# aukeschaap/ttcross

Hardware: AMD Instinct MI355X
Metric: fiber evals/s (neval / wall time of dtt_dmrgg), Ising C_64 n=51 r=32 piv=2 (d=63) (higher is better)
Workload: dtype f64; 1 GPU; Ising C_64 n=51 r=32 piv=2 (d=63); driver=test_crs_ising c 64 51 32 2, bond_groups=8, transport=none (single process), arith=exact, sweeps=16

## Files before the change

### profiles/trace_timeline.py

```python
import csv
import glob
import statistics
import sys

f = glob.glob(sys.argv[1] + '/**/*kernel_trace.csv', recursive=True)[0]
rows = list(csv.DictReader(open(f)))
rows.sort(key=lambda r: int(r['Start_Timestamp']))
start = sys.argv[2] if len(sys.argv) > 2 else "20"
count = int(sys.argv[3]) if len(sys.argv) > 3 else 40


def short(name):
    return name.split('(')[0].replace('void ', '')[:40]


if start == "tail":
    med = statistics.median
    sw = [i for i, r in enumerate(rows) if 'k_sweep_cluster' in r['Kernel_Name']]
    pairs = []
    for a, b in zip(sw, sw[1:]):
        mid = [r for r in rows[a + 1:b] if r['Queue_Id'] == rows[a]['Queue_Id']]
        if any(k in r['Kernel_Name'] for r in mid for k in ('k_reset', 'k_init', 'k_fin_')):
            continue
        t = int(rows[a]['End_Timestamp'])
        steps = []
        for r in mid:
            s, e = int(r['Start_Timestamp']), int(r['End_Timestamp'])
            steps.append((short(r['Kernel_Name']), (s - t) / 1e3, (e - s) / 1e3))
            t = max(t, e)
        last = (int(rows[b]['Start_Timestamp']) - t) / 1e3
        ktime = sum(x[2] for x in steps)
        e2s = (int(rows[b]['Start_Timestamp']) - int(rows[a]['End_Timestamp'])) / 1e3
        pairs.append((e2s, ktime, e2s - ktime, tuple(steps), last))
    shapes = {}
    for p in pairs:
        shapes.setdefault(tuple(x[0] for x in p[3]), []).append(p)
    sweeps = [(int(rows[i]['End_Timestamp']) - int(rows[i]['Start_Timestamp'])) / 1e3 for i in sw]
    real = [x for x in sweeps if x > 20.0]
    print(f"k_sweep_cluster: {len(real)} launches that sweep, median {med(real):.1f} us (min {min(real):.1f}, max {max(real):.1f}); "
          f"{len(sweeps) - len(real)} that exit on the stop flag")
    for names, ps in sorted(shapes.items(), key=lambda kv: -len(kv[1])):
        print(f"{len(ps)} pairs with {len(names)} launches in between: end-to-start median {med(p[0] for p in ps):.1f} us "
              f"(min {min(p[0] for p in ps):.1f}, max {max(p[0] for p in ps):.1f}) = kernels {med(p[1] for p in ps):.1f} + gaps {med(p[2] for p in ps):.1f}")
        for k, nm in enumerate(names):
            print(f"    gap {med(p[3][k][1] for p in ps):6.1f}  dur {med(p[3][k][2] for p in ps):6.1f}  {nm}")
        print(f"    gap {med(p[4] for p in ps):6.1f}  k_sweep_cluster (next)")
    sys.exit(0)
if start == "run":
    inits = [i for i, r in enumerate(rows) if 'k_init_samples' in r['Kernel_Name']]
    i0 = inits[2] - 8
else:
    idx = [i for i, r in enumerate(rows) if 'k_sweep_cluster' in r['Kernel_Name']]
    i0 = idx[int(start)]
t0 = int(rows[i0]['Start_Timestamp'])
prev_end = t0
for r in rows[i0:i0 + count]:
    s, e = int(r['Start_Timestamp']), int(r['End_Timestamp'])
    print(f"{(s - t0) / 1e3:9.1f} us  gap {(s - prev_end) / 1e3:6.1f}  dur {(e - s) / 1e3:7.1f}  {r['Kernel_Name'][:60]}")
    prev_end = max(prev_end, e)
```

### ttcross_amd/csrc/ttx_create_plan.h

```cpp
#pragma once
#include <algorithm>
#include <cmath>
#include <cstdarg>
#include <cstddef>
#include <cstdio>
#include <cstdlib>
#include <cstring>
#include <mutex>
#include <string>
#include <vector>

#include "../../include/ttx.h"
#include "ttx_dev.h"
#include "ttx_qr_plan.h"

#if defined(__HIPCC__)
#define TTX_PLAN_HD __host__ __device__ inline
#else
#define TTX_PLAN_HD inline
#endif

#define DE5_W 4
#define DE5_SEG 16
TTX_PLAN_HD size_t de5_lds_doubles(int m) { const int VS = ((m + 7) & ~7) + 8 + DE5_SEG; return (size_t)5 * VS + 128 + (size_t)DE5_W * 64; }
TTX_PLAN_HD bool de5_fits(int m) { return m >= 3; }
TTX_PLAN_HD int de_rows_stride(int m) { const int s = m + 56; return ((s + 31) & ~31) + 16; }
TTX_PLAN_HD size_t de_rows_lds_doubles(int m) { return (size_t)12 * de_rows_stride(m); }
TTX_PLAN_HD int det_vs(int m) { return ((m + 7) & ~7) + 8; }
TTX_PLAN_HD size_t det_lds_doubles(int m, int nbk) { return (size_t)4 * det_vs(m) + 256 + (det_vs(m) + 48) + (size_t)3 * nbk * 16 * 64; }

constexpr int TTX_PLAN_FB = 1024;
constexpr int TTX_PLAN_FNR = 24;
constexpr int TTX_PLAN_MVN_MAXQ = 8;

struct EnvText { bool set = false; std::string v; };
struct CreateEnv {
    EnvText arith;
    EnvText sweep;
    EnvText cl_pad;
    bool fullpiv_mfma = false;
    bool fast_persist_off = false;
    bool de_lane = false;
    bool de_tables_off = false, de_fastdiv_off = false, de_cut_off = false, de_v2_off = false, de_team_off = false;
    bool de_lot_point_set = false; int de_lot_point = 0;
    int de_team_units = 256, de_team6_units = 1024;
    int de_test_fault = 0;
    bool de_v5 = false;
    int cluster_nb = 8;
    bool cluster_coop = false;
    int cluster_test_abort = 0;
    bool dbg_waves = false;
    bool lottery_one_block = false;
    bool lottery_wave_off = false;
    bool lottery_rows2 = false;
    bool mvn_v2_off = false;
    bool tail_off = false;
    bool tail_side_off = false;
};
template <class Get>
CreateEnv create_env_from(Get get)
{
    auto text = [&](const char *name) { EnvText t; if (const char *e = get(name)) { t.set = true; t.v = e; } return t; };
    auto num = [&](const char *name, int dflt) { const char *e = get(name); return e ? atoi(e) : dflt; };
    auto off = [&](const char *name) { const char *e = get(name); return e && atoi(e) == 0; };
    CreateEnv v;
    v.arith = text("TTX_ARITH"); v.sweep = text("TTX_SWEEP"); v.cl_pad = text("TTX_CL_PAD");
    v.fullpiv_mfma = text("TTX_FULLPIV").v == "mfma";
    v.fast_persist_off = off("TTX_FAST_PERSIST");
    v.de_lane = num("TTX_DE_LANE", 0) == 1;
    v.de_tables_off = off("TTX_DE_TABLES"); v.de_fastdiv_off = off("TTX_DE_FASTDIV"); v.de_cut_off = off("TTX_DE_CUT");
    v.de_v2_off = off("TTX_DE_V2"); v.de_team_off = off("TTX_DE_TEAM");
    v.de_lot_point_set = get("TTX_DE_LOT_POINT") != nullptr; v.de_lot_point = num("TTX_DE_LOT_POINT", 0);
    v.de_team_units = num("TTX_DE_TEAM_UNITS", v.de_team_units); v.de_team6_units = num("TTX_DE_TEAM6_UNITS", v.de_team6_units);
    v.de_test_fault = num("TTX_DE_TEST_FAULT", 0);
    v.de_v5 = num("TTX_DE_V5", 0) == 1;
    v.cluster_nb = num("TTX_CLUSTER_NB", v.cluster_nb);
    v.cluster_coop = num("TTX_CLUSTER_COOP", 0) == 1;
    v.cluster_test_abort = num("TTX_CLUSTER_TEST_ABORT", 0);
    v.dbg_waves = get("TTX_DBG_WAVES") != nullptr;
    v.lottery_one_block = num("TTX_LOTTERY_NB", 0) == 1;
    v.lottery_wave_off = off("TTX_LOTTERY_WAVE");
    v.lottery_rows2 = num("TTX_LOTTERY_ROWS", 0) == 2;
    v.mvn_v2_off = off("TTX_MVN_V2");
    v.tail_off = off("TTX_TAIL"); v.tail_side_off = off("TTX_TAIL_SIDE");
    return v;
}
struct DevCaps { int ncu = 0; bool coop = false; };

enum SweepWant { SWEEP_AUTO, SWEEP_CHAIN, SWEEP_FUSED, SWEEP_CLUSTER };
enum SlotKind { SLOTS_NONE, SLOTS_HOST, SLOTS_DEVICE };

struct CdfTables { std::vector<ttx_cdfseg> tab; std::vector<int> ns; };

struct CreatePlan {
    int err = TTX_OK; std::string errtext;
    int d = 0, RM = 0, NM = 0, W = 1, wrank = 0, nproc = 1, g0 = 0, G = 0, nbmax = 0, NC = 0, mode = 0, H = 0;
    std::vector<int32_t> own;
    int ising_id = 0; bool isDE = false;
    double mvn_norm = 1.0;
    size_t SS = 0, SW = 0, CS = 0, XD = 0, IOFF = 0, MSZ = 0, QB = 0, SB = 0, VS = 0;
    int nfb = 0, nlotmax = 0;
    int nn = 0, snum = 0;
    SlotKind slots = SLOTS_NONE; size_t HS = 0;
    int cdf_kmax = -1;
    bool pfull = false, qscr = false;
    bool want_fast = false;
    bool unit_nodes = false;
    int arith = 0, FD = 0, fpersist = 0;
    bool fast_tables = false;
    int de_npair = 0;
    int de_unit = 0, de_cut = 0;
    int de_slots = 0;
    int de_v2 = 0;
    int de_team = 0, de_team_units = 256, de_team6_units = 1024;
    int de_v5 = 0;
    int de_test_fault = 0;
    int de_lot_point = 0;
    int lot_wave = 0, lot_rows = 0;
    size_t lds_de = 0, lds_det = 0, lds_det6 = 0, lds_de5 = 0, lds_der = 0;
    int mvn_v2 = 0; size_t lds_mvn = 0;
    int lot_nb = 1, bnd_wave = 0;
    bool lot_cand = false;
    int fp_mfma = 0, fp_tiles = 0;
    size_t lds_par = 0, lds_half = 0, lds_lot = 0;
    int half_vals = 0, lot_vals = 0, fast_cap = 0;
    size_t lds_fused = 0, lds_cluster = 0;
    bool fused_ok = false;
    int cluster_cand = 0;
    int cluster_var = 0;
    int cluster_ldsinv = 0, cluster_zkeep = 0, cluster_coop = 0;
    int cl_test_abort = 0; bool dbg_waves = false;
    bool sweep_tail = true;
    bool sweep_tail_side = true;
    SweepWant sweep_want = SWEEP_AUTO; int ncu = 0;
    int fused = 0;
    int cluster = 0;
};

inline void share(int first, int last, int nproc, std::vector<int32_t> &own)
{
    own.assign(nproc + 1, 0);
    own[0] = first;
    for (int p = 1; p < nproc; p++) own[p] = first + (int)((double)(last - first + 1) * (double)p / nproc);
    own[nproc] = last + 1;
}
inline double powi(double a, int b)
{
    double r = 1.0;
    for (;;) { if (b & 1) r *= a; b /= 2; if (b == 0) break; a *= a; }
    return r;
}
inline bool cdf_tables(int kmax, CdfTables &out)
{
    out.tab.assign((size_t)(kmax + 1) * TTX_TABSEG, ttx_cdfseg());
    out.ns.assign(kmax + 1, 0);
    std::vector<ttx_cdfseg> tmp(TTX_MAXSEG);
    for (int K = 1; K <= kmax; K++) {
        const int n_ = ttx_cdf_build(K, tmp.data());
        if (n_ > TTX_TABSEG) { out = CdfTables(); return false; }
        out.ns[K] = n_;
        memcpy(&out.tab[(size_t)K * TTX_TABSEG], tmp.data(), sizeof(ttx_cdfseg) * n_);
    }
    return true;
}
inline bool cdf_table_fits(int kmax)
{
    static std::mutex mu;
    static int looked = 0, first_over = -1;
    if (kmax > 16384) return false;
    std::lock_guard<std::mutex> lk(mu);
    std::vector<ttx_cdfseg> tmp(TTX_MAXSEG);
    while (looked < kmax && first_over < 0) { looked++; if (ttx_cdf_build(looked, tmp.data()) > TTX_TABSEG) first_over = looked; }
    return first_over < 0 || kmax < first_over;
}

#if defined(__GNUC__)
__attribute__((format(printf, 3, 4)))
#endif
inline CreatePlan &plan_refuse(CreatePlan &p, int code, const char *fmt, ...)
{
    char buf[512];
    va_list ap; va_start(ap, fmt); vsnprintf(buf, sizeof buf, fmt, ap); va_end(ap);
    p.err = code; p.errtext = buf;
    return p;
}

inline CreatePlan create_plan(const ttx_config &cfg, bool nofun, const CreateEnv &env, const DevCaps &caps)
{
    CreatePlan p;
    const int d = cfg.d, fun = cfg.fun_id, nproc = std::max(cfg.nproc, 1);
    p.d = d; p.RM = cfg.maxrank; p.nproc = nproc; p.ncu = caps.ncu;
    p.W = cfg.world_size < 1 ? 1 : cfg.world_size; p.wrank = cfg.world_rank;
    int NM = 1;
    for (int k = 0; k < d; k++) { if (cfg.n[k] < 1 || cfg.n[k] > 32000) return plan_refuse(p, TTX_EINVAL, "bad mode size"); NM = std::max(NM, cfg.n[k]); }
    p.NM = NM;
    if ((long long)p.RM * NM > (long long)TTX_MAXPART * TTX_BLK) return plan_refuse(p, TTX_EINVAL, "maxrank*n too large");
    if (cfg.mybonds) p.own.assign(cfg.mybonds, cfg.mybonds + nproc + 1);
    else share(1, d - 1, nproc, p.own);
    for (int g = 0; g < nproc; g++) if (p.own[g + 1] <= p.own[g]) return plan_refuse(p, TTX_EINVAL, "mybonds: empty group %d", g);
    if (p.own[0] != 1 || p.own[nproc] != d) return plan_refuse(p, TTX_EINVAL, "mybonds: must run from 1 to d = %d (got %d .. %d)", d, p.own[0], p.own[nproc]);
    p.g0 = (int)((long long)nproc * p.wrank / p.W);
    p.G = (int)((long long)nproc * (p.wrank + 1) / p.W) - p.g0;
    for (int g = 0; g < nproc; g++) p.nbmax = std::max(p.nbmax, p.own[g + 1] - p.own[g]);
    p.NC = p.nbmax + 1;
    p.mode = (cfg.pivoting == 0) ? 1 : (cfg.pivoting < 0) ? 2 : 0;
    p.H = (cfg.pivoting <= 0) ? 2 : 2 * cfg.pivoting;
    p.ising_id = (fun == TTX_FUN_ISING) ? (int)cfg.par[2 * cfg.n[0]] : 0;
    p.isDE = fun == TTX_FUN_ISING && p.ising_id != 1;
    if (fun == TTX_FUN_MVN) {
        if (cfg.naux < d + d * d + 1) return plan_refuse(p, TTX_EINVAL, "mvn: aux too short");
        p.mvn_norm = std::sqrt(powi(2.0 * 3.141592653589793, d) * cfg.aux[d + (size_t)d * d]);
        if (!(p.mvn_norm > 0.0) || !std::isfinite(p.mvn_norm))
            return plan_refuse(p, TTX_EINVAL, "ttx_create: mvn normalisation sqrt((2 pi)^d det) = %g is not a positive finite number (det = %g under- or overflows at d = %d)",
                               p.mvn_norm, cfg.aux[d + (size_t)d * d], d);
    }
    const size_t RM = p.RM;
    const size_t VS = ((d + 7) & ~7) + 8;
    const int nlotmax = 2 * p.RM + 2 * NM;
    p.VS = VS; p.nlotmax = nlotmax;
    p.SS = RM * NM; p.SW = (size_t)NM * RM; p.CS = RM * NM * RM;
    p.nfb = (int)((RM * NM + TTX_BLK - 1) / TTX_BLK);
    p.XD = RM * NM + RM * RM;
    p.IOFF = (sizeof(int) * (XH + d + 2) + 15) & ~(size_t)15;
    p.MSZ = (p.IOFF + sizeof(double) * p.XD + 15) & ~(size_t)15;
    p.QB = (size_t)nproc * RM * RM + 2 * nproc;
    p.SB = SUM_HDR + nproc + 5 * (size_t)(d + 1);
    p.qscr = 2 * sizeof(double) * (RM * RM + 2) > TTX_LDS_WORK;
    p.nn = cfg.n[0];
    for (int k = 1; k < d; k++) p.nn = std::min(p.nn, cfg.n[k]);
    p.snum = std::max(8, nproc);

    bool want = cfg.arith == TTX_ARITH_FAST;
    if (cfg.arith != TTX_ARITH_EXACT && cfg.arith != TTX_ARITH_FAST) return plan_refuse(p, TTX_EINVAL, "ttx_create: arith must be TTX_ARITH_EXACT or TTX_ARITH_FAST (got %d)", cfg.arith);
    if (env.arith.set) {
        if (env.arith.v == "fast") want = true;
        else if (env.arith.v != "exact") return plan_refuse(p, TTX_EINVAL, "TTX_ARITH must be exact or fast (got %s)", env.arith.v.c_str());
    }
    p.want_fast = want && !nofun;
    bool unit = fun == TTX_FUN_ISING;
    for (int j = 0; unit && j < std::min(NM, (int)cfg.npar); j++) unit = cfg.par[j] >= 0.0 && cfg.par[j] <= 1.0;
    p.unit_nodes = unit;
    p.arith = (p.want_fast && ((p.isDE && unit) || fun == TTX_FUN_MVN)) ? 1 : 0;
    if (p.arith) {
        p.fast_tables = true;
        p.FD = d + 1;
        p.fpersist = (fun == TTX_FUN_MVN && env.fast_persist_off) ? 0 : 1;
    }
    if (p.isDE && !p.arith && env.de_lane) p.de_unit = unit;
    if (p.isDE && !p.arith && !env.de_lane && !env.de_tables_off) {
        p.de_npair = d * (d + 1) / 2;
        p.de_unit = unit && !env.de_fastdiv_off;
        p.de_cut = (p.de_unit && !env.de_cut_off) ? 1 : 0;
        p.de_lot_point = (env.de_lot_point_set ? env.de_lot_point : (int)(d <= 160)) != 0;
        p.de_slots = (int)RM * ((NM + 63) / 64);
        p.lds_de = sizeof(double) * (5 * VS + 256) + (p.de_cut ? sizeof(int) * VS : 0);
        p.de_v2 = cfg.pivoting >= 0 && p.de_slots <= TTX_MAXPART && p.lds_de <= TTX_LDS_WORK && !env.de_v2_off;
        p.lds_det = sizeof(double) * det_lds_doubles(d, 3);
        p.lds_det6 = sizeof(double) * det_lds_doubles(d, 1);
        p.de_team = p.de_v2 && !p.de_cut && p.lds_det <= TTX_LDS_WORK && !env.de_team_off;
        p.de_team_units = env.de_team_units;
        p.de_team6_units = env.de_team6_units;
        p.de_test_fault = env.de_test_fault;
        p.lds_de5 = sizeof(double) * de5_lds_doubles(d);
        p.de_v5 = p.de_v2 && !p.de_cut && de5_fits(d) && p.lds_de5 <= TTX_LDS_WORK && env.de_v5;
    }
    p.pfull = cfg.pivoting < 0;
    if (cfg.pivoting < 0 && env.fullpiv_mfma && RM <= 64 && (long long)(RM * NM) * (long long)(RM * NM) < (1LL << 31)) {
        const size_t side = RM * NM;
        p.fp_mfma = 1; p.fp_tiles = (int)(((side + 63) / 64) * ((side + 63) / 64));
    }
    if (cdf_table_fits(p.RM * NM)) p.cdf_kmax = p.RM * NM;

    p.lds_par = sizeof(double) * (cfg.npar + 2);
    {
        const size_t base = sizeof(double) * (cfg.npar + RM + 4);
        const size_t idx_bytes = sizeof(short) * ((RM + 1) * VS + 16), val_bytes = sizeof(double) * ((RM + 1) * 2 * VS + 4);
        p.half_vals = (fun == TTX_FUN_ISING && p.ising_id == 1 && base + val_bytes <= TTX_LDS_VALUES) ? 1 : 0;
        p.lds_half = base + (p.half_vals ? val_bytes : idx_bytes);
        const size_t dif_bytes = sizeof(double) * ((RM + 1) * VS + 4);
        if (fun == TTX_FUN_MVN && base + dif_bytes <= TTX_LDS_HALF_DIFF) { p.half_vals = 1; p.lds_half = base + dif_bytes; }
        if (p.arith) p.lds_half = std::max(p.lds_half, base + sizeof(double) * ((size_t)std::max(p.FD, TTX_PLAN_FNR) + 4 + RM + 2));
    }
    const size_t lot_hdr = sizeof(double) * (cfg.npar + 4) + sizeof(int) * 4 * (nlotmax + 4);
    {
        p.lds_lot = lot_hdr + sizeof(short) * (2 * RM * VS + 16);
        const size_t lot_dif = lot_hdr + sizeof(double) * (2 * RM * VS + 4);
        if (fun == TTX_FUN_MVN && lot_dif <= TTX_LDS_LOTTERY) { p.lot_vals = 1; p.lds_lot = lot_dif; }
        if (p.arith && fun == TTX_FUN_ISING) {
            const size_t hdr = lot_hdr + 32;
            const size_t rowb = 2 * sizeof(double) * RM;
            p.fast_cap = (int)std::min<size_t>(std::min<size_t>(40, (size_t)d + 1), hdr < TTX_LDS_VALUES ? (TTX_LDS_VALUES - hdr) / rowb : 0);
            p.lds_lot = std::max(p.lds_lot, hdr + rowb * p.fast_cap);
        }
    }
    {
        const bool fastc = fun == TTX_FUN_ISING && p.ising_id == 1 && cfg.pivoting >= 0 && p.cdf_kmax >= 0;
        p.lds_fused = sizeof(double) * (cfg.npar + 4 + 4 * RM * VS + 2 * RM * NM + RM + 4) + sizeof(int) * 4 * (nlotmax + 4);
        p.fused_ok = fastc && p.RM <= 64 && nlotmax <= TTX_PLAN_FB && p.lds_fused <= TTX_LDS_WORK;
        int NB = std::max(1, std::min(env.cluster_nb, TTX_CLMAX));
        while (NB > 1 && p.G * NB > caps.ncu / 2) NB--;
        const size_t SL = RM * ((NM + NB - 1) / NB + 1);
        p.lds_cluster = sizeof(double) * (cfg.npar + 4 + 2 * RM * (2 * VS + 2) + 4 * SL + 2 * RM + 8) + sizeof(int) * 4 * (nlotmax + 4);
        if (p.lds_cluster + sizeof(double) * 2 * RM * RM <= TTX_LDS_WORK) { p.cluster_ldsinv = 1; p.lds_cluster += sizeof(double) * 2 * RM * RM; }
        const size_t zk = sizeof(int) * ((size_t)p.nbmax * 2 * RM + 2 * p.nbmax + 4);
        if (p.lds_cluster + zk <= TTX_LDS_WORK) { p.cluster_zkeep = 1; p.lds_cluster += zk; }
        const bool cfastc = p.want_fast && fun == TTX_FUN_ISING && p.ising_id == 1;
        if (env.cl_pad.set && env.cl_pad.v != "0" && env.cl_pad.v != "1") return plan_refuse(p, TTX_EINVAL, "TTX_CL_PAD must be 0 or 1 (got %s)", env.cl_pad.v.c_str());
        p.cluster_var = cfastc ? 2 : (unit && !(env.cl_pad.set && env.cl_pad.v == "0")) ? 1 : 0;
        if (fastc && p.RM <= 64 && NB >= 2 && p.G * NB <= caps.ncu && p.lds_cluster <= TTX_LDS_WORK) {
            p.cluster_cand = NB;
            p.cluster_coop = caps.coop && env.cluster_coop;
        }
        p.cl_test_abort = env.cluster_test_abort; p.dbg_waves = env.dbg_waves;
        p.sweep_tail = !env.tail_off; p.sweep_tail_side = !env.tail_side_off;
        const std::string want_sweep = env.sweep.set ? env.sweep.v : "auto";
        if (want_sweep == "cluster") p.sweep_want = SWEEP_CLUSTER;
        else if (want_sweep == "fused") p.sweep_want = SWEEP_FUSED;
        else if (want_sweep == "auto") p.sweep_want = SWEEP_AUTO;
        else if (want_sweep == "chain") p.sweep_want = SWEEP_CHAIN;
        else return plan_refuse(p, TTX_EINVAL, "TTX_SWEEP must be auto, chain, fused or cluster (got %s)", want_sweep.c_str());
    }
    if (!nofun && (p.lds_half > TTX_LDS_DEVICE || p.lds_lot > TTX_LDS_LOTTERY)) return plan_refuse(p, TTX_EINVAL, "problem too large for LDS staging (d*maxrank)");
    {
        const bool heavy = p.isDE || fun == TTX_FUN_MVN;
        if (heavy && !env.lottery_one_block) p.lot_nb = std::min((nlotmax + 63) / 64, 64);
        if (p.lot_nb > 1 && (nlotmax + p.lot_nb - 1) / p.lot_nb > 64) p.lot_nb = 1;
        if (fun == TTX_FUN_MVN && d <= 64 * TTX_PLAN_MVN_MAXQ && cfg.pivoting >= 0 && (int)RM * ((NM + 63) / 64) <= TTX_MAXPART && !env.mvn_v2_off) {
            p.lot_cand = true;
            p.mvn_v2 = 1; p.de_slots = (int)RM * ((NM + 63) / 64);
            p.bnd_wave = 1;
            p.lds_mvn = sizeof(double) * (3 * (size_t)d + 8);
        }
        if (p.isDE && p.arith) p.bnd_wave = 1;
        if (p.isDE && p.de_npair) {
            p.lot_cand = true;
            p.lds_der = sizeof(double) * de_rows_lds_doubles(d);
            p.lot_wave = p.de_v2 && !p.de_cut && p.lds_der <= TTX_LDS_WORK && !env.lottery_wave_off;
            p.bnd_wave = p.lot_wave || (p.de_cut && p.de_v2 && p.lds_der <= TTX_LDS_WORK);
            p.lot_rows = p.lot_wave ? (env.lottery_rows2 ? 2 : 1) : 0;
        }
    }
    if (fun == TTX_FUN_HOST || fun == TTX_FUN_COSCOEFF || fun == TTX_FUN_DEVICE || fun == TTX_FUN_TRAINS) {
        p.HS = std::max<size_t>({RM * NM, (size_t)p.nn * p.snum, (size_t)p.NC * NM, (size_t)nlotmax, (size_t)2 * NM, (size_t)256});
        p.slots = fun == TTX_FUN_HOST ? SLOTS_HOST : SLOTS_DEVICE;
    }
    return p;
}

inline void create_admit(CreatePlan &p, int occ)
{
    bool cluster_ok = p.cluster_cand != 0;
    if (cluster_ok) {
        const long long cap = (long long)occ * p.ncu;
        const long long grid = 8LL * p.cluster_cand * ((p.G + 7) / 8);
        if (grid * 2 > cap) cluster_ok = false;
    }
    if (p.sweep_want == SWEEP_CLUSTER) { if (cluster_ok) p.cluster = p.cluster_cand; }
    else if (p.sweep_want == SWEEP_FUSED) { if (p.fused_ok) p.fused = 1; }
    else if (p.sweep_want == SWEEP_AUTO) { if (cluster_ok) p.cluster = p.cluster_cand; else if (p.fused_ok && p.G == 1) p.fused = 1; }
    if (p.cluster && p.cluster_var == 2) p.arith = 1;
}
```

### ttcross_amd/csrc/ttx_engine.hip

```cpp
#include <hip/hip_runtime.h>

#include <chrono>
#include <cmath>
#include <cstdarg>
#include <cstdio>
#include <cstdlib>
#include <cstring>
#include <map>
#include <memory>
#include <string>
#include <thread>
#include <type_traits>
#include <vector>

#include <atomic>
#include <dlfcn.h>
#include <rccl/rccl.h>

#include "../../include/ttx.h"
#include "../../include/ttx_device_fun.h"
#include "ttx_lds.h"
#include "ttx_qr_plan.h"
#include "ttx_create_plan.h"
#include "ttx_loop_plan.h"
// ... 21 lines not shown
#include "ttx_roundsum.h"
#include "ttx_sample.h"
#include "ttx_sample_real.h"
#include "ttx_topk.h"
#include "ttx_sample_sq.h"
#include "ttx_trainfun.h"

static thread_local std::string g_err;
static int fail(int code, const char *fmt, ...)
{
    char buf[512];
    va_list ap; va_start(ap, fmt); vsnprintf(buf, sizeof buf, fmt, ap); va_end(ap);
    g_err = buf;
    return code;
}
#define HIPCHECK(x) do { hipError_t e_ = (x); if (e_ != hipSuccess) return fail(TTX_EHIP, "%s failed: %s (%s:%d)", #x, hipGetErrorString(e_), __FILE__, __LINE__); } while (0)


static int env_int(const char *name, int dflt) { const char *e = getenv(name); return e ? atoi(e) : dflt; }
static bool env_off(const char *name) { const char *e = getenv(name); return e && atoi(e) == 0; }

static int ensure_lds(int device, const void *fn, size_t need)
{
    return ttx_lds_raise(device, fn, need, [](const void *fn, size_t need) -> int {
        HIPCHECK(hipFuncSetAttribute(fn, hipFuncAttributeMaxDynamicSharedMemorySize, (int)need));
        return TTX_OK;
    });
}

extern "C" const char *ttx_last_error(void) { return g_err.c_str(); }
extern "C" int ttx_version(void) { return 3; }


struct RcclApi {
    void *lib = nullptr;
    ncclResult_t (*GetUniqueId)(ncclUniqueId *) = nullptr;
    ncclResult_t (*CommInitRank)(ncclComm_t *, int, ncclUniqueId, int) = nullptr;
    ncclResult_t (*CommDestroy)(ncclComm_t) = nullptr;
    ncclResult_t (*Send)(const void *, size_t, ncclDataType_t, int, ncclComm_t, hipStream_t) = nullptr;
    ncclResult_t (*Recv)(void *, size_t, ncclDataType_t, int, ncclComm_t, hipStream_t) = nullptr;
    ncclResult_t (*AllReduce)(const void *, void *, size_t, ncclDataType_t, ncclRedOp_t, ncclComm_t, hipStream_t) = nullptr;
    ncclResult_t (*GroupStart)() = nullptr;
    ncclResult_t (*GroupEnd)() = nullptr;
    const char *(*GetErrorString)(ncclResult_t) = nullptr;
};
static RcclApi g_rccl;
static int rccl_load()
{
    if (g_rccl.lib) return TTX_OK;
    void *L = dlopen("librccl.so", RTLD_NOW | RTLD_GLOBAL);
    if (!L) L = dlopen("/opt/rocm/lib/librccl.so", RTLD_NOW | RTLD_GLOBAL);
    if (!L) return fail(TTX_EHIP, "cannot load librccl.so: %s", dlerror());
#define SYM_(f, name) *(void **)(&g_rccl.f) = dlsym(L, name); if (!g_rccl.f) return fail(TTX_EHIP, "librccl.so lacks %s", name);
    SYM_(GetUniqueId, "ncclGetUniqueId") SYM_(CommInitRank, "ncclCommInitRank") SYM_(CommDestroy, "ncclCommDestroy")
    SYM_(Send, "ncclSend") SYM_(Recv, "ncclRecv") SYM_(AllReduce, "ncclAllReduce") SYM_(GroupStart, "ncclGroupStart")
    SYM_(GroupEnd, "ncclGroupEnd") SYM_(GetErrorString, "ncclGetErrorString")
#undef SYM_
    g_rccl.lib = L;
    return TTX_OK;
}
#define NCCLCHECK(x) do { ncclResult_t e_ = (x); if (e_ != ncclSuccess) return fail(TTX_EHIP, "%s failed: %s", #x, g_rccl.GetErrorString(e_)); } while (0)

enum {
    SC_TRAIN,
    SC_META,
    SC_IND, SC_OUT, SC_X,
    SC_FLAG, SC_LQ,
    SC_XA, SC_XB, SC_SORT,
    SC_W, SC_M, SC_P, SC_SCR, SC_VEC,
    SC_H, SC_ROW, SC_CNT,
    SC_SRX,
    SC_TFUN, SC_TVAL,
    SC_MAT,
    SC_KP, SC_KW, SC_KS, SC_KX,
    SC_KREC, SC_KSEL, SC_KOUT,
    SC_RSO, SC_RSW, SC_RSYA, SC_RSYB,
    SC_RSM, SC_RSTAB,
    SC_QH, SC_QF, SC_QS, SC_QX,
    SC_BTAB,
    SC_NBUF
};
struct EvBuf { void *p = nullptr; size_t bytes = 0; };
struct OpTimer {
    hipEvent_t ev[2] = {nullptr, nullptr};
    int start(hipStream_t s) { for (auto &e : ev) if (!e) HIPCHECK(hipEventCreate(&e)); HIPCHECK(hipEventRecord(ev[0], s)); return TTX_OK; }
    int stop(hipStream_t s) { HIPCHECK(hipEventRecord(ev[1], s)); return TTX_OK; }
    int ms(double *out) { float t = 0.f; HIPCHECK(hipEventElapsedTime(&t, ev[0], ev[1])); *out = t; return TTX_OK; }
};
enum { TM_MODESUM, TM_ALG, TM_HEAD, TM_DRAW, TM_APPLY,
       TM_GRAM, TM_SCORE, TM_SELECT,
       TM_RS_SKETCH, TM_N };

struct DevFun;
struct TrainFun;
struct ttx_engine {
    ttx_config cfg;
    std::vector<int32_t> n1;
    std::vector<double> par, aux, quadw;
    std::vector<int32_t> own;
    int d = 0, RM = 0, NM = 0, G = 0, NC = 0, nbmax = 0, H = 0, mode = 0;
    int g0 = 0;
    int W = 1, wrank = 0;
    DevProb P{};
    hipStream_t stream = nullptr;
    std::vector<void *> allocs;
    size_t SB = 0, QB = 0;
    double *h_sum = nullptr;
    char *h_msg = nullptr;
    double *h_tmp = nullptr;
    char *recvL = nullptr, *recvR = nullptr;
    ncclComm_t comm = nullptr;
    ttx_transport cb{};
    bool have_cb = false;
    int cb_error = 0;
    struct RedJob { ttx_engine *h; double *buf; size_t count; int op; };
    static const int NRED = 16;
    RedJob red[NRED];
    double *red_mem = nullptr; size_t red_cap = 0; int red_next = 0;
    RedJob *red_slot(size_t count, int op)
    {
        if (!red_mem || count > red_cap) return nullptr;
        RedJob *j = &red[red_next];
        j->h = this; j->buf = red_mem + (size_t)red_next * red_cap; j->count = count; j->op = op;
        red_next = (red_next + 1) % NRED;
        return j;
    }
    ShmTransport *shm = nullptr;
    std::vector<ttx_sweep_rec> recs;
    std::vector<int32_t> tapes;
    std::vector<int32_t> rfinal;
    std::vector<std::vector<uint8_t>> updhist;
    int64_t neval = 0;
    double seconds = 0.0;
    bool ran = false;
    bool profile = false;
    struct Ev { int kind, n; hipEvent_t a, b; };
    std::vector<Ev> evs;
    std::vector<hipEvent_t> evpool;
    int64_t k_launches[TTX_K_NKINDS] = {0};
    double k_ms[TTX_K_NKINDS] = {0}, k_bytes[TTX_K_NKINDS] = {0};
    double *Wa = nullptr, *Wb = nullptr, *Wc = nullptr, *Wd = nullptr, *Sm = nullptr, *bak = nullptr;
    int *Si = nullptr;
    CreatePlan sel;
    struct Retired { bool cluster = false, de_team = false, de_v5 = false; } retired;
    int cluster_nb() const { return retired.cluster ? 0 : sel.cluster; }
    bool de_team() const { return sel.de_team && !retired.de_team; }
    bool de_v5() const { return sel.de_v5 && !retired.de_v5; }
    int arith() const { return P.arith; }
    int cluster_fallbacks = 0;
    int det_fallbacks = 0, de5_fallbacks = 0;
    bool cluster_aborted = false;
    double *h_svd = nullptr; double svd_seq = 0.0;
    hipStream_t qstream = nullptr;
    hipEvent_t ev_sum[2] = {nullptr, nullptr}, ev_val[2] = {nullptr, nullptr}, ev_tail[2] = {nullptr, nullptr};
    double *h_sum_base = nullptr;
    double *h_val = nullptr;
    int *h_abort = nullptr;
    ttx_host_fun hfun = nullptr;
    const double *hfun_par = nullptr;
    std::shared_ptr<DevFun> dfun;
    std::shared_ptr<TrainFun> tfun;
    TfOps tf_ops{};
    std::vector<char> tf_host;
    std::vector<std::pair<hipEvent_t, hipEvent_t>> tf_evs;
    bool tf_figures = false;
    int64_t tf_launches = 0, tf_elements = 0;
    double tf_ms = 0.0;
    int64_t host_calls = 0;
    int64_t n_resid = 0;
    EvBuf scratch[SC_NBUF];
    std::vector<char> train_host, meta_host;
    OpTimer timer[TM_N];
    int ncu = 0;
    int ev_last_mode = -1;
    double ct_ms = 0.0, ct_bytes = 0.0;
    double alg_ms = 0.0, alg_rd = 0.0, alg_wr = 0.0;
    double sm_ms_head = 0.0, sm_bytes = 0.0, sm_ms_draw = 0.0;
    int64_t sm_failed = 0;
    double sr_ms_head = 0.0, sr_bytes = 0.0, sr_ms_draw = 0.0;
    int64_t sr_failed = 0;
    double ma_ms = 0.0, ma_rd = 0.0, ma_wr = 0.0, ma_flops = 0.0;
    int ma_mode = -1;
    double tk_ms_gram = 0.0, tk_ms_score = 0.0, tk_ms_select = 0.0, tk_flops = 0.0;
    int tk_mode = -1;
    double sq_ms_head = 0.0, sq_ms_rows = 0.0, sq_ms_pick = 0.0, sq_flops = 0.0;
    int64_t sq_failed = 0;
    int sq_mode = -1;
    double rs_ms[4] = {0.0, 0.0, 0.0, 0.0}, rs_flops = 0.0;
    std::vector<int32_t> rs_l;
    int rs_mode = -1;
    std::vector<hipEvent_t> rs_ev;
    double bs_ms_tab = 0.0, bs_ms_chain = 0.0, bs_flops = 0.0;
    int bs_mode = -1;
    std::vector<hipEvent_t> bs_ev;
};

static HostPool &host_pool()
{
    static HostPool p(host_pool_threads(getenv("TTX_HOST_THREADS"), getenv("OMP_NUM_THREADS"), std::thread::hardware_concurrency()));
    return p;
}

static int host_eval(ttx_engine *h)
{
    HIPCHECK(hipStreamSynchronize(h->stream));
    HIPCHECK(hipGetLastError());
    DevProb &P = h->P;
    const size_t nslot = (size_t)h->G * h->sel.HS;
    std::vector<uint32_t> todo;
    for (size_t s = 0; s < nslot; s++) if (P.hreq[s]) { todo.push_back((uint32_t)s); P.hreq[s] = 0; }
    const int32_t d = h->d;
    const int32_t *nn = h->n1.data() + 1;
    host_pool().run(todo.size(), [&](size_t i) {
        int32_t ind[2048];
        const short *row = P.hidx + (size_t)todo[i] * d;
        for (int k = 0; k < d; k++) ind[k] = row[k];
        P.hval[todo[i]] = h->hfun(&d, ind, nn, h->hfun_par);
    });
    h->host_calls += (int64_t)todo.size();
    return TTX_OK;
}

struct DevFun {
    int device = 0;
    hipModule_t mod = nullptr;
    hipFunction_t slots = nullptr, list = nullptr;
    ttx_devfun_info info{};
    double *par = nullptr;
    std::string name;
    std::vector<unsigned char> image;
    ~DevFun()
    {
        (void)hipSetDevice(device);
        if (par) (void)hipFree(par);
        else (void)hipDeviceSynchronize();
        if (mod) (void)hipModuleUnload(mod);
    }
};
#define DEVFUN_LAUNCHCHECK(x) do { hipError_t e_ = (x); if (e_ != hipSuccess) return fail(TTX_EHIP, "%s failed: %s (%s:%d)", #x, hipGetErrorString(e_), __FILE__, __LINE__); } while (0)
static int devfun_slots(ttx_engine *h)
{
    DevFun &f = *h->dfun;
    DevProb &P = h->P;
    int d = P.d;
    long long nslot = (long long)h->G * h->sel.HS;
    const int *n = P.n + 1;
    const double *par = f.par;
    const short *hidx = P.hidx; unsigned char *hreq = P.hreq; double *hval = P.hval;
    const int waves = f.info.block / 64;
    const long long want = f.info.kind == TTX_DEVFUN_KIND_WAVE ? (nslot + waves - 1) / waves : (nslot + f.info.block - 1) / f.info.block;
    const unsigned grid = (unsigned)std::max<long long>(1, std::min<long long>(want, 4096));
    void *args[] = {&d, &n, &par, &nslot, &hidx, &hreq, &hval};
    DEVFUN_LAUNCHCHECK(hipModuleLaunchKernel(f.slots, grid, 1, 1, (unsigned)f.info.block, 1, 1, (unsigned)(f.info.lds_per_wave * waves), h->stream, args, nullptr));
    return TTX_OK;
}

struct TrainFun {
    std::vector<ttx_engine *> x;
    int op = 0;
    std::shared_ptr<DevFun> comb;
};
static int tf_grid(ttx_engine *h, long long items);
static int tf_prepare(ttx_engine *h, const char *who, bool figures);
static int tf_finish(ttx_engine *h);
static int tf_eval_list(ttx_engine *h, int64_t npts, const int32_t *ind, double *out);
struct TfScope {
    ttx_engine *h; hipEvent_t a = nullptr, b = nullptr;
    bool on;
    explicit TfScope(ttx_engine *h_) : h(h_), on(h_->profile && h_->tf_figures) { if (on) { (void)hipEventCreate(&a); (void)hipEventCreate(&b); (void)hipEventRecord(a, h->stream); } }
    ~TfScope() { if (on) { (void)hipEventRecord(b, h->stream); h->tf_evs.push_back({a, b}); } }
};
static int tf_slots(ttx_engine *h)
{
    const TrainFun &f = *h->tfun;
    DevProb &P = h->P;
    long long nslot = (long long)h->G * h->sel.HS;
    const TfOps &O = h->tf_ops;
    const size_t lds = sizeof(double) * TTX_TF_WAVES * tf_lds_doubles(O.ldx, O.d);
    const dim3 grid(tf_grid(h, nslot)), block(64 * TTX_TF_WAVES);
    const short *hidx = P.hidx; unsigned char *hreq = P.hreq; double *hval = P.hval;
    double *tval = (double *)h->scratch[SC_TVAL].p;
    unsigned long long *cnt = (unsigned long long *)h->scratch[SC_CNT].p;
    if (h->tf_figures) h->tf_launches++;
    TfScope timed(h);
    switch (f.op) {
        case TTX_TOP_PRODUCT: hipLaunchKernelGGL(k_tf_slots<TF_PRODUCT>, grid, block, lds, h->stream, O, nslot, hidx, hreq, hval, tval, cnt); break;
        case TTX_TOP_RATIO: hipLaunchKernelGGL(k_tf_slots<TF_RATIO>, grid, block, lds, h->stream, O, nslot, hidx, hreq, hval, tval, cnt); break;
        case TTX_TOP_SQRTABS: hipLaunchKernelGGL(k_tf_slots<TF_SQRTABS>, grid, block, lds, h->stream, O, nslot, hidx, hreq, hval, tval, cnt); break;
        default: {
            hipLaunchKernelGGL(k_tf_slots<TF_DEVICE>, grid, block, lds, h->stream, O, nslot, hidx, hreq, hval, tval, cnt);
            DevFun &c = *f.comb;
            int m = O.m, d = O.d;
            const int *n = P.n + 1;
            const double *par = c.par, *tv = tval;
            const unsigned cg = (unsigned)std::max<long long>(1, std::min<long long>((nslot + c.info.block - 1) / c.info.block, 4096));
            void *args[] = {&m, &d, &n, &par, &nslot, &hidx, &hreq, &tv, &hval};
            DEVFUN_LAUNCHCHECK(hipModuleLaunchKernel(c.slots, cg, 1, 1, (unsigned)c.info.block, 1, 1, 0, h->stream, args, nullptr));
        }
    }
    return TTX_OK;
}

static int slot_eval(ttx_engine *h)
{
    DevProb &P = h->P;
    if (!P.slot_dev) return host_eval(h);
    if (h->cfg.fun_id == TTX_FUN_DEVICE) return devfun_slots(h);
// ... 66 lines not shown
    P.ising_id = s.ising_id;
    P.has_quad = cfg.quadw != nullptr;
    P.small_element = 10 * 2.220446049250313e-16; P.small_pivot = 1.e-5;
    P.mvn_norm = s.mvn_norm;
    P.SS = s.SS; P.SW = s.SW; P.CS = s.CS;
    P.arith = s.arith; P.FD = s.FD; P.fpersist = s.fpersist;
    P.de_npair = s.de_npair; P.de_unit = s.de_unit; P.de_cut = s.de_cut;
    P.nfb = s.nfb; P.fp_mfma = s.fp_mfma; P.fp_tiles = s.fp_tiles;
    P.XD = s.XD; P.IOFF = s.IOFF; P.MSZ = s.MSZ;
    P.accuracy = cfg.accuracy; P.maxrank = cfg.maxrank;
    P.lot_nb = s.lot_nb; P.lot_max = s.nlotmax; P.bnd_wave = s.bnd_wave;
    h->n1.assign(d + 2, 1);
    for (int k = 1; k <= d; k++) h->n1[k] = cfg.n[k - 1];
    if (cfg.npar > 0) h->par.assign(cfg.par, cfg.par + cfg.npar);
    if (cfg.aux && cfg.naux > 0) h->aux.assign(cfg.aux, cfg.aux + cfg.naux);
    int *dn; double *dpar, *daux = nullptr, *dq = nullptr;
    A_(dev_upload(h, &dn, h->n1.data(), (size_t)d + 2));
    A_(dev_alloc(h, &dpar, cfg.npar + 1));
    if (cfg.npar > 0) HIPCHECK(hipMemcpy(dpar, h->par.data(), sizeof(double) * cfg.npar, hipMemcpyHostToDevice));
    if (!h->aux.empty()) A_(dev_upload(h, &daux, h->aux.data(), h->aux.size()));
    if (cfg.quadw) {
        h->quadw.assign((size_t)(d + 1) * NM, 0.0);
        size_t off = 0;
        for (int k = 1; k <= d; k++) { for (int j = 0; j < h->n1[k]; j++) h->quadw[(size_t)k * NM + j] = cfg.quadw[off + j]; off += h->n1[k]; }
        A_(dev_upload(h, &dq, h->quadw.data(), h->quadw.size()));
    }
    P.n = dn; P.par = dpar; P.aux = daux; P.quadw = dq;
    return TTX_OK;
}
static int create_integrand_tables(ttx_engine *h)
{
    const CreatePlan &s = h->sel;
    DevProb &P = h->P;
    const int d = s.d;
    const size_t G = s.G, NC = s.NC, RM = s.RM;
    const bool mvn = h->cfg.fun_id == TTX_FUN_MVN;
    if (s.fast_tables) {
        const size_t slots = s.fpersist ? G * NC : G;
        for (int sd = 0; sd < 2; sd++) {
            A_(dev_alloc(h, &P.fNear[sd], slots * (size_t)s.FD * RM));
            A_(dev_alloc(h, &P.fPiv[sd], slots * (size_t)TTX_FS * RM));
            if (mvn) A_(dev_alloc(h, &P.fDv[sd], slots * (size_t)s.FD * RM));
        }
        if (mvn) {
            std::vector<double> sy((size_t)d * d);
            const double *ic = h->aux.data() + d;
            for (int i = 0; i < d; i++) for (int j = 0; j < d; j++) sy[i + (size_t)d * j] = 0.5 * (ic[i + (size_t)d * j] + ic[j + (size_t)d * i]);
            double *ds;
            A_(dev_upload(h, &ds, sy.data(), sy.size()));
            P.auxS = ds;
        }
    }
    if (s.de_npair) {
        A_(dev_alloc(h, &P.deTL, G * (size_t)s.de_npair * RM)); A_(dev_alloc(h, &P.deTR, G * (size_t)s.de_npair * RM));
        A_(dev_alloc(h, &P.deUL, G * (size_t)(d + 1) * RM));
        if (s.de_cut) { A_(dev_alloc(h, &P.deCL, G * (size_t)(d + 1) * RM)); A_(dev_alloc(h, &P.deCR, G * (size_t)(d + 1) * RM)); }
    }
    if (mvn) {
        std::vector<double> t((size_t)d * d);
        for (int i = 0; i < d; i++) for (int j = 0; j < d; j++) t[j + (size_t)d * i] = h->aux[d + i + (size_t)d * j];
        double *dt;
        A_(dev_upload(h, &dt, t.data(), t.size()));
        P.auxT = dt;
    }
    return TTX_OK;
}
static int create_cores(ttx_engine *h)
{
    const CreatePlan &s = h->sel;
    DevProb &P = h->P;
    const size_t d = s.d, G = s.G, NC = s.NC, RM = s.RM, NM = s.NM;
    A_(dev_alloc(h, &P.arg, G * NC * P.CS)); A_(dev_alloc(h, &P.col, G * NC * P.CS)); A_(dev_alloc(h, &P.row, G * NC * P.CS));
    A_(dev_alloc(h, &P.inv, G * NC * RM * RM)); A_(dev_alloc(h, &P.vip, G * NC * 4 * RM));
    A_(dev_alloc(h, &P.L, G * NC * d * RM)); A_(dev_alloc(h, &P.R, G * NC * d * RM));
    A_(dev_alloc(h, &P.r, G * (d + 2))); A_(dev_alloc(h, &P.rr, G * (d + 2))); A_(dev_alloc(h, &P.upd, G * (d + 2))); A_(dev_alloc(h, &P.tape, G * (d + 2) * 4));
    A_(dev_alloc(h, &P.acol, G * RM * NM)); A_(dev_alloc(h, &P.arow, G * RM * NM));
    A_(dev_alloc(h, &P.Tq, G * NC * RM * RM));
    A_(dev_alloc(h, &P.ind0, d + 2)); A_(dev_alloc(h, &P.gs, G));
    for (size_t g = 0; g < G; g++) {
        GroupState g0s{};
        g0s.first = h->own[h->g0 + g]; g0s.last = h->own[h->g0 + g + 1] - 1; g0s.gglobal = h->g0 + (int)g;
        const hipError_t e = hipMemcpy(P.gs + g, &g0s, offsetof(GroupState, S), hipMemcpyHostToDevice);
        if (e != hipSuccess) return fail(TTX_EHIP, "ttx_create: %s", hipGetErrorString(e));
    }
    if (s.pfull) A_(dev_alloc(h, &P.pfull, G * NM * RM * (size_t)s.nfb));
    if (s.fp_mfma) { A_(dev_alloc(h, &P.sb, G * (RM * NM) * (RM * NM))); A_(dev_alloc(h, &P.pfull2, G * (size_t)s.fp_tiles)); }
    if (s.cdf_kmax >= 0) {
        CdfTables t;
        if (!cdf_tables(s.cdf_kmax, t)) return fail(TTX_EINVAL, "ttx_create: no CDF tables up to K = %d", s.cdf_kmax);
        ttx_cdfseg *dt; int *dn_;
        A_(dev_upload(h, &dt, t.tab.data(), t.tab.size()));
        A_(dev_upload(h, &dn_, t.ns.data(), t.ns.size()));
        P.cdf_tab = dt; P.cdf_ns = dn_; P.cdf_kmax = s.cdf_kmax;
    }
    LotPart *lp; unsigned *lc;
    A_(dev_alloc(h, &lp, G * s.lot_nb));
    A_(dev_alloc(h, &lc, G));
    P.lotp = lp; P.lot_ctr = lc;
    if (s.lot_cand) { A_(dev_alloc(h, &P.lotc, G * s.nlotmax * 4)); A_(dev_alloc(h, &P.lotf, G * s.nlotmax)); }
    if (s.cluster) {
        unsigned *ctr; ClPart *cp;
        A_(dev_alloc(h, &ctr, G));
        A_(dev_alloc(h, &cp, 2 * G * TTX_CLREC));
        P.cl_ctr = ctr; P.cl_part = cp;
#ifdef TTX_STAMPS
        if (s.dbg_waves) { long long *dbg; A_(dev_alloc(h, &dbg, (size_t)8 * 64 * 8)); P.dbg = dbg; }
#endif
        HIPCHECK(hipHostMalloc((void **)&h->h_abort, sizeof(int)));
        *h->h_abort = 0;
        P.cl_abort = h->h_abort;
        P.cl_test_abort = s.cl_test_abort;
    }
    return TTX_OK;
}
static int create_exchange(ttx_engine *h)
{
    const CreatePlan &s = h->sel;
    DevProb &P = h->P;
    const size_t G = s.G, RM = s.RM, d = s.d;
    const int nproc = s.nproc;
    A_(dev_alloc(h, &P.msgR, G * P.MSZ)); A_(dev_alloc(h, &P.msgL, G * P.MSZ));
    A_(dev_alloc(h, &h->recvL, P.MSZ)); A_(dev_alloc(h, &h->recvR, P.MSZ));
    A_(dev_alloc(h, &P.inL, G)); A_(dev_alloc(h, &P.inR, G));
    A_(dev_alloc(h, &P.red, G * 4)); A_(dev_alloc(h, &P.redsend, 4));
    A_(dev_alloc(h, &P.qsend, h->QB)); A_(dev_alloc(h, &P.qwork, ((size_t)nproc + 2) * RM * RM)); A_(dev_alloc(h, &P.sumsend, h->SB));
    P.qscr = nullptr;
    if (s.qscr) A_(dev_alloc(h, &P.qscr, G * 2 * RM * RM));
    if (s.W > 1) { A_(dev_alloc(h, &P.redrecv, 4)); A_(dev_alloc(h, &P.qall, h->QB)); A_(dev_alloc(h, &P.sumrecv, h->SB)); }
    else { P.redrecv = P.redsend; P.qall = P.qsend; P.sumrecv = P.sumsend; }
    {
        std::vector<char *> il(G, nullptr), ir(G, nullptr);
        for (size_t g = 0; g < G; g++) {
            if (g > 0) il[g] = P.msgR + (g - 1) * P.MSZ; else if (h->g0 > 0) il[g] = h->recvL;
            if (g + 1 < G) ir[g] = P.msgL + (g + 1) * P.MSZ; else if (h->g0 + (int)G < nproc) ir[g] = h->recvR;
        }
        HIPCHECK(hipMemcpy(P.inL, il.data(), sizeof(char *) * G, hipMemcpyHostToDevice));
        HIPCHECK(hipMemcpy(P.inR, ir.data(), sizeof(char *) * G, hipMemcpyHostToDevice));
    }
    int *ctl, *rq;
    A_(dev_alloc(h, &ctl, (size_t)4));
    A_(dev_alloc(h, &rq, G * (d + 2)));
    P.ctl = ctl; P.rq = rq;
    P.tail_side = 0;
    A_(dev_alloc(h, &P.tailrec, 2 * G)); A_(dev_alloc(h, &P.tail_tape, 2 * G * (d + 2) * 4)); A_(dev_alloc(h, &P.strk, (size_t)2));
    return TTX_OK;
}
static int create_staging(ttx_engine *h)
{
    HIPCHECK(hipHostMalloc((void **)&h->h_sum_base, sizeof(double) * 2 * h->SB));
    h->h_sum = h->h_sum_base;
    memset(h->h_sum_base, 0, sizeof(double) * 2 * h->SB);
    HIPCHECK(hipHostMalloc((void **)&h->h_val, sizeof(double) * 2));
    HIPCHECK(hipStreamCreateWithFlags(&h->qstream, hipStreamNonBlocking));
    for (int x = 0; x < 2; x++) { HIPCHECK(hipEventCreateWithFlags(&h->ev_sum[x], hipEventDisableTiming)); HIPCHECK(hipEventCreateWithFlags(&h->ev_val[x], hipEventDisableTiming)); HIPCHECK(hipEventCreateWithFlags(&h->ev_tail[x], hipEventDisableTiming)); }
    HIPCHECK(hipHostMalloc((void **)&h->h_msg, 4 * h->P.MSZ));
    HIPCHECK(hipHostMalloc((void **)&h->h_tmp, sizeof(double) * std::max(h->QB, h->SB)));
    if (h->W > 1) {
        h->red_cap = std::max<size_t>(std::max(h->QB, h->SB), 8);
        HIPCHECK(hipHostMalloc((void **)&h->red_mem, sizeof(double) * h->red_cap * ttx_engine::NRED));
    }
    return TTX_OK;
}
static int create_slots(ttx_engine *h)
{
    const CreatePlan &s = h->sel;
    DevProb &P = h->P;
    if (s.slots == SLOTS_NONE) return TTX_OK;
    const size_t nslot = (size_t)s.G * s.HS, d = s.d;
    if (s.slots == SLOTS_DEVICE) {
        P.slot_dev = 1;
        A_(dev_alloc(h, &P.hidx, nslot * d)); A_(dev_alloc(h, &P.hval, nslot)); A_(dev_alloc(h, &P.hreq, nslot));
    } else {
        HIPCHECK(hipHostMalloc((void **)&P.hidx, sizeof(short) * nslot * d));
        HIPCHECK(hipHostMalloc((void **)&P.hval, sizeof(double) * nslot));
        HIPCHECK(hipHostMalloc((void **)&P.hreq, nslot));
        memset(P.hreq, 0, nslot); memset(P.hval, 0, sizeof(double) * nslot);
    }
    P.HS = (int)s.HS; P.hostpass = 0;
    return TTX_OK;
}
#undef A_

static int create_impl(ttx_engine **out, const ttx_config *cfg, bool nofun)
{
    if (!out || !cfg) return fail(TTX_EINVAL, "ttx_create: null argument");
    *out = nullptr;
    if (!cfg->n) return fail(TTX_EINVAL, "ttx_create: mode sizes missing");
    if (cfg->d < 2) return fail(TTX_EINVAL, "dtt_dmrgg: l,m: 1 %d", cfg->d);
    if (cfg->maxrank < 1 || cfg->maxrank > 128) return fail(TTX_EINVAL, "ttx_create: maxrank must be in 1..128 (got %d)", cfg->maxrank);
    if (cfg->pivoting < -1) return fail(TTX_EINVAL, "dtt_dmrgg: unknown pivoting: %d", cfg->pivoting);
    if (2 * cfg->pivoting + 2 > TTX_MAXH) return fail(TTX_EINVAL, "dtt_dmrgg: pivoting %d too large", cfg->pivoting);
    if (!(nofun && cfg->fun_id == 0) && (cfg->fun_id < 1 || cfg->fun_id > TTX_FUN_TRAINS)) return fail(TTX_EINVAL, "ttx_create: unknown fun_id %d", cfg->fun_id);
    if (cfg->npar < 0 || (cfg->npar > 0 && !cfg->par)) return fail(TTX_EINVAL, "ttx_create: par missing");
    if (cfg->fun_id == TTX_FUN_ISING && (cfg->npar < 2 * cfg->n[0] + 1)) return fail(TTX_EINVAL, "ttx_create: the Ising integrand needs par(1:2n+1) (nodes, weights, id)");
    if ((cfg->fun_id == TTX_FUN_STDNORM || cfg->fun_id == TTX_FUN_MVN) && cfg->npar < cfg->n[0]) return fail(TTX_EINVAL, "ttx_create: the integrand needs the nodes par(1:n)");
    if (cfg->fun_id != TTX_FUN_HOST && cfg->fun_id != TTX_FUN_COSCOEFF && cfg->fun_id != TTX_FUN_DEVICE && cfg->fun_id != TTX_FUN_TRAINS && cfg->fun_id != 0)
        for (int k = 1; k < cfg->d; k++)
            if (cfg->n[k] > cfg->n[0]) return fail(TTX_EINVAL, "ttx_create: mode %d has %d points, more than the first mode (%d): the built-in integrands index par by n(1)", k + 1, cfg->n[k], cfg->n[0]);
    if (cfg->fun_id == TTX_FUN_HOST && cfg->d > 2048) return fail(TTX_EINVAL, "ttx_create: host integrand: at most 2048 dimensions (tt_size)");
    if (cfg->fun_id == TTX_FUN_DEVICE && cfg->d > 2048) return fail(TTX_EINVAL, "ttx_create: device integrand: at most 2048 dimensions (tt_size)");
    if (cfg->fun_id == TTX_FUN_TRAINS && cfg->d > 2048) return fail(TTX_EINVAL, "ttx_create: integrand of trains: at most 2048 dimensions (tt_size)");
    if (cfg->fun_id == TTX_FUN_COSCOEFF) { if (int rc0 = coscoeff_check("ttx_create", cfg->d, cfg->n, cfg->aux, cfg->naux)) return rc0; }
    const int W = cfg->world_size < 1 ? 1 : cfg->world_size;
    if (cfg->fun_id == TTX_FUN_TRAINS && W > 1) return fail(TTX_EINVAL, "ttx_create: an integrand of trains (TTX_FUN_TRAINS) runs in one process: bond groups (nproc) work, world_size %d does not", W);
    const int nproc = std::max(cfg->nproc < 1 ? 1 : cfg->nproc, 1);
    if (nproc >= cfg->d) return fail(TTX_EINVAL, "nproc exceeds or equal dimension, cannot proceed");
    if (nproc < W) return fail(TTX_EINVAL, "ttx_create: %d bond groups cannot be spread over %d GPUs", nproc, W);
    if (nproc > 256) return fail(TTX_EINVAL, "ttx_create: at most 256 bond groups");
    if (cfg->world_rank < 0 || cfg->world_rank >= W) return fail(TTX_EINVAL, "ttx_create: world_rank out of range");
    int ndev = 0;
    if (hipGetDeviceCount(&ndev) != hipSuccess || ndev <= 0) return fail(TTX_ENODEV, "ttx_create: no HIP device (the engine has no CPU path)");
    if (cfg->device < 0 || cfg->device >= ndev) return fail(TTX_ENODEV, "ttx_create: device %d not present", cfg->device);
    HIPCHECK(hipSetDevice(cfg->device));
    DevCaps caps;
    {
        hipDeviceProp_t prop;
        HIPCHECK(hipGetDeviceProperties(&prop, cfg->device));
        int coop = 0;
        HIPCHECK(hipDeviceGetAttribute(&coop, hipDeviceAttributeCooperativeLaunch, cfg->device));
        caps.ncu = prop.multiProcessorCount; caps.coop = coop != 0;
    }

    ttx_config c = *cfg;
    c.nproc = nproc;
    CreatePlan plan = create_plan(c, nofun, create_env(), caps);
    if (plan.err) return fail(plan.err, "%s", plan.errtext.c_str());
    if (plan.cluster_cand) {
        const void *fn = reinterpret_cast<const void *>(cluster_kernel(plan.cluster_var));
        if (int rc = ensure_lds(cfg->device, fn, plan.lds_cluster)) return rc;
        int occ = 0;
        HIPCHECK(hipOccupancyMaxActiveBlocksPerMultiprocessor(&occ, cluster_kernel(plan.cluster_var), CB, plan.lds_cluster));
        create_admit(plan, occ);
    } else create_admit(plan, 0);

    ttx_engine *h = new ttx_engine();
    struct Guard { ttx_engine *h; ~Guard() { if (h) destroy_keep_error(h); } } guard{h};
    h->cfg = c;
    h->sel = std::move(plan);
    const CreatePlan &s = h->sel;
    h->W = s.W; h->wrank = s.wrank; h->d = s.d; h->RM = s.RM; h->NM = s.NM; h->own = s.own;
    h->g0 = s.g0; h->G = s.G; h->nbmax = s.nbmax; h->NC = s.NC; h->mode = s.mode; h->H = s.H;
    h->QB = s.QB; h->SB = s.SB;
    HIPCHECK(hipStreamCreateWithFlags(&h->stream, hipStreamNonBlocking));
    int rc;
    if ((rc = create_problem(h)) || (rc = create_integrand_tables(h)) || (rc = create_cores(h)) || (rc = create_exchange(h)) ||
        (rc = create_staging(h)) || (rc = create_slots(h))) return rc;
    guard.h = nullptr;
    *out = h;
    return TTX_OK;
}
extern "C" int ttx_create(ttx_engine **out, const ttx_config *cfg) { return create_impl(out, cfg, false); }

extern "C" void ttx_destroy(ttx_engine *h)
{
    if (!h) return;
    if (h->dfun) { (void)hipSetDevice(h->cfg.device); if (h->stream) (void)hipStreamSynchronize(h->stream); h->dfun.reset(); }
    if (h->tfun) { (void)hipSetDevice(h->cfg.device); if (h->stream) (void)hipStreamSynchronize(h->stream); h->tfun.reset(); }
    if (h->comm && g_rccl.CommDestroy) (void)g_rccl.CommDestroy(h->comm);
    for (void *p : h->allocs) (void)hipFree(p);
    for (auto &b : h->scratch) if (b.p) (void)hipFree(b.p);
    for (auto &t : h->timer) for (auto &e : t.ev) if (e) (void)hipEventDestroy(e);
    for (auto &e : h->tf_evs) { (void)hipEventDestroy(e.first); (void)hipEventDestroy(e.second); }
    if (h->h_sum_base) (void)hipHostFree(h->h_sum_base);
    if (h->h_val) (void)hipHostFree(h->h_val);
    if (h->h_svd) (void)hipHostFree(h->h_svd);
    if (h->qstream) (void)hipStreamDestroy(h->qstream);
    for (int x = 0; x < 2; x++) { if (h->ev_sum[x]) (void)hipEventDestroy(h->ev_sum[x]); if (h->ev_val[x]) (void)hipEventDestroy(h->ev_val[x]); if (h->ev_tail[x]) (void)hipEventDestroy(h->ev_tail[x]); }
    if (h->h_msg) (void)hipHostFree(h->h_msg);
    if (h->h_tmp) (void)hipHostFree(h->h_tmp);
    if (h->red_mem) (void)hipHostFree(h->red_mem);
    if (h->shm) { shm_close(h->shm); delete h->shm; }
    if (h->h_abort) (void)hipHostFree(h->h_abort);
    if (!h->P.slot_dev) {
        if (h->P.hidx) (void)hipHostFree(h->P.hidx);
        if (h->P.hval) (void)hipHostFree(h->P.hval);
        if (h->P.hreq) (void)hipHostFree(h->P.hreq);
    }
    for (auto &e : h->evpool) (void)hipEventDestroy(e);
    for (auto &e : h->rs_ev) (void)hipEventDestroy(e);
    for (auto &e : h->bs_ev) (void)hipEventDestroy(e);
    if (h->stream) (void)hipStreamDestroy(h->stream);
    delete h;
}

extern "C" int ttx_comm_unique_id(uint8_t id[128])
{
    int rc = rccl_load();
    if (rc) return rc;
    ncclUniqueId u;
    NCCLCHECK(g_rccl.GetUniqueId(&u));
    memcpy(id, u.internal, 128);
    return TTX_OK;
}
extern "C" int ttx_comm_init(ttx_engine *h, const uint8_t id[128])
{
    if (!h) return fail(TTX_EINVAL, "ttx_comm_init: null handle");
    if (h->cfg.fun_id == TTX_FUN_TRAINS) return fail(TTX_ESTATE, "ttx_comm_init: an engine with an integrand of trains (TTX_FUN_TRAINS) runs in one process");
    if (h->W == 1) return TTX_OK;
    int rc = rccl_load();
    if (rc) return rc;
    HIPCHECK(hipSetDevice(h->cfg.device));
    ncclUniqueId u;
    memcpy(u.internal, id, 128);
    NCCLCHECK(g_rccl.CommInitRank(&h->comm, h->W, u, h->wrank));
    return TTX_OK;
}
extern "C" int ttx_k_rccl_selftest(int32_t device, int64_t msg_bytes, int32_t nsum)
{
    if (msg_bytes < 1 || nsum < 1) return fail(TTX_EINVAL, "ttx_k_rccl_selftest: bad sizes");
    int ndev = 0;
    if (hipGetDeviceCount(&ndev) != hipSuccess || ndev <= 0) return fail(TTX_ENODEV, "no HIP device");
    HIPCHECK(hipSetDevice(device));
    int rc = rccl_load();
    if (rc) return rc;
    ncclUniqueId u;
    NCCLCHECK(g_rccl.GetUniqueId(&u));
    ncclComm_t comm = nullptr;
    NCCLCHECK(g_rccl.CommInitRank(&comm, 1, u, 0));
    hipStream_t st = nullptr;
    char *dsend = nullptr, *drecv = nullptr; double *dred = nullptr, *dout = nullptr;
    std::vector<char> hs((size_t)msg_bytes), hr((size_t)msg_bytes);
    std::vector<double> hd((size_t)nsum + 4), ho((size_t)nsum + 4);
    for (int64_t i = 0; i < msg_bytes; i++) hs[(size_t)i] = (char)((i * 131 + 7) & 0xff);
    for (size_t i = 0; i < hd.size(); i++) hd[i] = 1.0 / (double)(i + 3) - 0.25 * (double)(i % 5);
    int bad = 0;
    auto body = [&]() -> int {
        HIPCHECK(hipStreamCreateWithFlags(&st, hipStreamNonBlocking));
        HIPCHECK(hipMalloc((void **)&dsend, (size_t)msg_bytes)); HIPCHECK(hipMalloc((void **)&drecv, (size_t)msg_bytes));
        HIPCHECK(hipMalloc((void **)&dred, sizeof(double) * hd.size())); HIPCHECK(hipMalloc((void **)&dout, sizeof(double) * hd.size()));
        HIPCHECK(hipMemcpyAsync(dsend, hs.data(), (size_t)msg_bytes, hipMemcpyHostToDevice, st));
        HIPCHECK(hipMemsetAsync(drecv, 0, (size_t)msg_bytes, st));
        HIPCHECK(hipMemcpyAsync(dred, hd.data(), sizeof(double) * hd.size(), hipMemcpyHostToDevice, st));
        HIPCHECK(hipMemsetAsync(dout, 0, sizeof(double) * hd.size(), st));
        NCCLCHECK(g_rccl.GroupStart());
        NCCLCHECK(g_rccl.Send(dsend, (size_t)msg_bytes, ncclChar, 0, comm, st));
        NCCLCHECK(g_rccl.Recv(drecv, (size_t)msg_bytes, ncclChar, 0, comm, st));
        NCCLCHECK(g_rccl.GroupEnd());
        NCCLCHECK(g_rccl.AllReduce(dred, dout, 4, ncclDouble, ncclMax, comm, st));
        NCCLCHECK(g_rccl.AllReduce(dred + 4, dout + 4, (size_t)nsum, ncclDouble, ncclSum, comm, st));
        HIPCHECK(hipMemcpyAsync(hr.data(), drecv, (size_t)msg_bytes, hipMemcpyDeviceToHost, st));
        HIPCHECK(hipMemcpyAsync(ho.data(), dout, sizeof(double) * ho.size(), hipMemcpyDeviceToHost, st));
        HIPCHECK(hipStreamSynchronize(st));
        if (memcmp(hs.data(), hr.data(), (size_t)msg_bytes) != 0) bad |= 1;
        if (memcmp(hd.data(), ho.data(), sizeof(double) * hd.size()) != 0) bad |= 2;
        return TTX_OK;
    };
    rc = body();
    if (dsend) (void)hipFree(dsend); if (drecv) (void)hipFree(drecv); if (dred) (void)hipFree(dred); if (dout) (void)hipFree(dout);
    if (st) (void)hipStreamDestroy(st);
    (void)g_rccl.CommDestroy(comm);
    if (rc) return rc;
    if (bad) return fail(TTX_EHIP, "ttx_k_rccl_selftest: %s came back different", bad == 1 ? "the point-to-point message" : bad == 2 ? "an all-reduce" : "message and all-reduce");
    return TTX_OK;
}

extern "C" int ttx_comm_init_shm(ttx_engine *h, const char *name)
{
    if (!h || !name || !*name) return fail(TTX_EINVAL, "ttx_comm_init_shm: null argument");
    if (h->cfg.fun_id == TTX_FUN_TRAINS) return fail(TTX_ESTATE, "ttx_comm_init_shm: an engine with an integrand of trains (TTX_FUN_TRAINS) runs in one process");
    if (h->W == 1) return TTX_OK;
    if (h->shm) return fail(TTX_ESTATE, "ttx_comm_init_shm: already initialised");
    ShmTransport *T = new ShmTransport();
    std::string text;
    if (int rc = shm_attach(name, h->wrank, h->W, (h->P.MSZ + 63) & ~(size_t)63, std::max<size_t>(std::max(h->QB, h->SB), 8), T, &text)) {
        delete T;
        return fail(rc, "%s", text.c_str());
    }
    h->shm = T;
    h->cb.ctx = T; h->cb.sendrecv = shm_sendrecv; h->cb.allreduce = shm_allreduce; h->have_cb = true;
    if (shm_barrier(T)) return fail(TTX_EHIP, "ttx_comm_init_shm: not all %d ranks attached", T->W);
    return TTX_OK;
}

extern "C" int ttx_set_transport(ttx_engine *h, const ttx_transport *t)
{
    if (!h || !t || !t->sendrecv || !t->allreduce) return fail(TTX_EINVAL, "ttx_set_transport: null argument");
    if (h->cfg.fun_id == TTX_FUN_TRAINS) return fail(TTX_ESTATE, "ttx_set_transport: an engine with an integrand of trains (TTX_FUN_TRAINS) runs in one process");
    h->cb = *t; h->have_cb = true;
    return TTX_OK;
}

extern "C" int ttx_set_integrand_host(ttx_engine *h, ttx_host_fun fun, const double *par)
{
    if (!h || !fun) return fail(TTX_EINVAL, "ttx_set_integrand_host: null argument");
    if (h->cfg.fun_id != TTX_FUN_HOST) return fail(TTX_ESTATE, "ttx_set_integrand_host: the engine was not created with fun_id = TTX_FUN_HOST");
    h->hfun = fun; h->hfun_par = par;
    return TTX_OK;
}
extern "C" int64_t ttx_host_calls(const ttx_engine *h) { return h ? h->host_calls : 0; }

static int devfun_load(const char *who, const char *prefix, const char *macro, const char *what, ttx_engine *h, const void *image, int64_t nbytes, const char *name,
                       const double *par, int32_t npar, std::shared_ptr<DevFun> *out)
{
    if (!image || nbytes <= 0) return fail(TTX_EINVAL, "%s: empty code object image", who);
    if (!name || !*name || strlen(name) > 200) return fail(TTX_EINVAL, "%s: integrand name missing (or longer than 200 characters)", who);
    if (npar < 0 || (npar > 0 && !par)) return fail(TTX_EINVAL, "%s: par missing (npar = %d)", who, npar);
    if (!devfun_image_plausible((const unsigned char *)image, (size_t)nbytes))
        return fail(TTX_EINVAL, "%s: the image is neither a complete code object (ELF) nor a complete offload bundle of hipcc --genco", who);
    HIPCHECK(hipSetDevice(h->cfg.device));
    auto f = std::make_shared<DevFun>();
    f->device = h->cfg.device; f->name = name;
    f->image.assign((const unsigned char *)image, (const unsigned char *)image + nbytes);
    f->image.push_back(0);
    hipError_t e = hipModuleLoadData(&f->mod, f->image.data());
    if (e != hipSuccess) {
        (void)hipGetLastError(); f->mod = nullptr;
        return fail(TTX_EINVAL, "%s: the runtime refused the code object (%s): is it built for this GPU (--offload-arch=gfx950)?", who, hipGetErrorString(e));
    }
    const std::string sn = std::string(prefix) + "slots_" + name, ln = std::string(prefix) + "list_" + name, in = std::string(prefix) + "info_" + name;
    hipDeviceptr_t ip = nullptr; size_t ib = 0;
    if ((e = hipModuleGetGlobal(&ip, &ib, f->mod, in.c_str())) != hipSuccess || hipModuleGetFunction(&f->slots, f->mod, sn.c_str()) != hipSuccess ||
        hipModuleGetFunction(&f->list, f->mod, ln.c_str()) != hipSuccess) {
        (void)hipGetLastError();
        return fail(TTX_EINVAL, "%s: the code object has no %s '%s' (symbols %s, %s, %s: see %s in ttx_device_fun.h)",
                    who, what, name, in.c_str(), sn.c_str(), ln.c_str(), macro);
    }
    if (ib < sizeof(int)) return fail(TTX_EINVAL, "%s: %s is not a ttx_devfun_info", who, in.c_str());
    HIPCHECK(hipMemcpy(&f->info, (const void *)ip, std::min(ib, sizeof(f->info)), hipMemcpyDeviceToHost));
    if (f->info.abi != TTX_DEVFUN_ABI || ib != sizeof(f->info))
        return fail(TTX_EINVAL, "%s: integrand '%s' was compiled against slot ABI version %d, this engine speaks version %d: recompile it with this engine's ttx_device_fun.h",
// ... 31 lines not shown
{
    if (!h) return fail(TTX_EINVAL, "ttx_eval_device: null handle");
    if (h->cfg.fun_id == TTX_FUN_TRAINS) return tf_eval_list(h, npts, ind, out);
    if (h->cfg.fun_id != TTX_FUN_DEVICE) return fail(TTX_ESTATE, "ttx_eval_device: the engine was not created with fun_id = TTX_FUN_DEVICE");
    if (!h->dfun) return fail(TTX_ESTATE, "ttx_eval_device: call ttx_set_integrand_device first");
    if (npts < 0 || (npts > 0 && (!ind || !out))) return fail(TTX_EINVAL, "ttx_eval_device: null argument");
    if (npts == 0) return TTX_OK;
    int d = h->d;
    for (int64_t p = 0; p < npts; p++)
        for (int k = 0; k < d; k++)
            if (ind[p * d + k] < 1 || ind[p * d + k] > h->n1[k + 1])
                return fail(TTX_EINVAL, "ttx_eval_device: point %lld: index %d of mode %d is outside 1..%d", (long long)p, ind[p * d + k], k + 1, h->n1[k + 1]);
    HIPCHECK(hipSetDevice(h->cfg.device));
    DevFun &f = *h->dfun;
    int *dind = nullptr; double *dout = nullptr;
    HIPCHECK(hipMalloc((void **)&dind, sizeof(int) * (size_t)npts * d));
    if (hipMalloc((void **)&dout, sizeof(double) * (size_t)npts) != hipSuccess) { (void)hipFree(dind); return fail(TTX_EHIP, "ttx_eval_device: out of device memory"); }
    int rc = TTX_OK;
    long long np = npts;
    const int *n = h->P.n + 1;
    const double *par = f.par;
    const int waves = f.info.block / 64;
    const long long want = f.info.kind == TTX_DEVFUN_KIND_WAVE ? (np + waves - 1) / waves : (np + f.info.block - 1) / f.info.block;
    const unsigned grid = (unsigned)std::max<long long>(1, std::min<long long>(want, 4096));
    void *args[] = {&d, &n, &par, &np, &dind, &dout};
    hipError_t e = hipMemcpyAsync(dind, ind, sizeof(int) * (size_t)npts * d, hipMemcpyHostToDevice, h->stream);
    if (e == hipSuccess) e = hipModuleLaunchKernel(f.list, grid, 1, 1, (unsigned)f.info.block, 1, 1, (unsigned)(f.info.lds_per_wave * waves), h->stream, args, nullptr);
    if (e == hipSuccess) e = hipMemcpyAsync(out, dout, sizeof(double) * (size_t)npts, hipMemcpyDeviceToHost, h->stream);
    if (e == hipSuccess) e = hipStreamSynchronize(h->stream);
    if (e != hipSuccess) rc = fail(TTX_EHIP, "ttx_eval_device: %s", hipGetErrorString(e));
    (void)hipFree(dind); (void)hipFree(dout);
    return rc;
}

static void hostfn_xfer(void *ud)
{
    ttx_engine *h = (ttx_engine *)ud;
    const DevProb &P = h->P;
    const int left = (h->g0 > 0) ? h->wrank - 1 : -1, right = (h->g0 + h->G < h->cfg.nproc) ? h->wrank + 1 : -1;
    char *sR = h->h_msg, *sL = h->h_msg + P.MSZ, *rL = h->h_msg + 2 * P.MSZ, *rR = h->h_msg + 3 * P.MSZ;
    if (h->cb.sendrecv(h->cb.ctx, right, sR, (int64_t)P.MSZ, left, rL, (int64_t)P.MSZ)) h->cb_error = 1;
    if (h->cb.sendrecv(h->cb.ctx, left, sL, (int64_t)P.MSZ, right, rR, (int64_t)P.MSZ)) h->cb_error = 1;
}
static void hostfn_allreduce(void *ud)
{
    ttx_engine::RedJob *j = (ttx_engine::RedJob *)ud;
    if (j->h->cb.allreduce(j->h->cb.ctx, j->buf, (int64_t)j->count, j->op)) j->h->cb_error = 1;
}

static int xfer_neighbours(ttx_engine *h)
{
    if (h->W == 1) return TTX_OK;
    DevProb &P = h->P;
    const int left = (h->g0 > 0) ? h->wrank - 1 : -1, right = (h->g0 + h->G < h->cfg.nproc) ? h->wrank + 1 : -1;
    char *outR = P.msgR + (size_t)(h->G - 1) * P.MSZ, *outL = P.msgL;
    if (h->comm) {
        NCCLCHECK(g_rccl.GroupStart());
        if (right >= 0) { NCCLCHECK(g_rccl.Send(outR, P.MSZ, ncclChar, right, h->comm, h->stream)); NCCLCHECK(g_rccl.Recv(h->recvR, P.MSZ, ncclChar, right, h->comm, h->stream)); }
        if (left >= 0) { NCCLCHECK(g_rccl.Send(outL, P.MSZ, ncclChar, left, h->comm, h->stream)); NCCLCHECK(g_rccl.Recv(h->recvL, P.MSZ, ncclChar, left, h->comm, h->stream)); }
        NCCLCHECK(g_rccl.GroupEnd());
        return TTX_OK;
    }
    if (!h->have_cb) return fail(TTX_ESTATE, "world_size > 1 but neither ttx_comm_init nor ttx_set_transport was called");
    char *sR = h->h_msg, *sL = h->h_msg + P.MSZ;
    if (right >= 0) HIPCHECK(hipMemcpyAsync(sR, outR, P.MSZ, hipMemcpyDeviceToHost, h->stream));
    if (left >= 0) HIPCHECK(hipMemcpyAsync(sL, outL, P.MSZ, hipMemcpyDeviceToHost, h->stream));
    HIPCHECK(hipLaunchHostFunc(h->stream, hostfn_xfer, h));
    if (left >= 0) HIPCHECK(hipMemcpyAsync(h->recvL, h->h_msg + 2 * P.MSZ, P.MSZ, hipMemcpyHostToDevice, h->stream));
    if (right >= 0) HIPCHECK(hipMemcpyAsync(h->recvR, h->h_msg + 3 * P.MSZ, P.MSZ, hipMemcpyHostToDevice, h->stream));
    return TTX_OK;
}
static int allreduce_dev(ttx_engine *h, const double *src, double *dst, size_t count, int op)
{
    if (h->W == 1) return TTX_OK;
    if (h->comm) { NCCLCHECK(g_rccl.AllReduce(src, dst, count, ncclDouble, op ? ncclMax : ncclSum, h->comm, h->stream)); return TTX_OK; }
    if (!h->have_cb) return fail(TTX_ESTATE, "world_size > 1 but neither ttx_comm_init nor ttx_set_transport was called");
    ttx_engine::RedJob *job = h->red_slot(count, op);
    if (!job) return fail(TTX_EHIP, "allreduce staging exhausted");
    HIPCHECK(hipMemcpyAsync(job->buf, src, sizeof(double) * count, hipMemcpyDeviceToHost, h->stream));
    HIPCHECK(hipLaunchHostFunc(h->stream, hostfn_allreduce, job));
    HIPCHECK(hipMemcpyAsync(dst, job->buf, sizeof(double) * count, hipMemcpyHostToDevice, h->stream));
    return TTX_OK;
}

static hipEvent_t ev_get(ttx_engine *h)
{
    if (!h->evpool.empty()) { hipEvent_t e = h->evpool.back(); h->evpool.pop_back(); return e; }
    hipEvent_t e; (void)hipEventCreate(&e); return e;
}
struct KScope {
    ttx_engine *h; int kind, n; hipEvent_t a = nullptr, b = nullptr;
    KScope(ttx_engine *h_, int kind_, int n_ = 1) : h(h_), kind(kind_), n(n_) { if (h->profile) { a = ev_get(h); b = ev_get(h); (void)hipEventRecord(a, h->stream); } }
    ~KScope() { if (h->profile) { (void)hipEventRecord(b, h->stream); h->evs.push_back({kind, n, a, b}); } else h->k_launches[kind] += n; }
};
static void ev_collect(ttx_engine *h)
{
    for (auto &e : h->evs) {
        float ms = 0.f;
        (void)hipEventElapsedTime(&ms, e.a, e.b);
        h->k_ms[e.kind] += ms; h->k_launches[e.kind] += e.n;
        h->evpool.push_back(e.a); h->evpool.push_back(e.b);
    }
    h->evs.clear();
}

static double erank_host(const ttx_engine *h, const int32_t *r)
{
    const int l = 1, m = h->d, d = m;
    if (d == 1) return 0.0;
    double s = 0.0;
    for (int i = l; i <= m; i++) s = s + r[i - 1] * h->n1[i] * r[i];
    if (s == 0.0) return s;
    int b = r[l - 1] * h->n1[l] + h->n1[m] * r[m];
    if (d == 2) return s / b;
    int a = 0;
    for (int i = l + 1; i <= m - 1; i++) a += h->n1[i];
    return (std::sqrt(b * b + 4.0 * a * s) - b) / (2.0 * a);
}

static std::string fmt_e(int w, int dgt, double v)
{
    char tmp[64], body[64];
    if (v != 0.0 && std::isfinite(v)) {
        snprintf(tmp, sizeof tmp, "%.*e", dgt - 1, v);
        char *e = strchr(tmp, 'e');
        int ex = atoi(e + 1) + 1;
        *e = 0;
        std::string digs;
        for (char *c = tmp; *c; c++) if (*c >= '0' && *c <= '9') digs.push_back(*c);
        snprintf(body, sizeof body, ".%sE%c%02d", digs.c_str(), ex < 0 ? '-' : '+', abs(ex));
    } else snprintf(body, sizeof body, ".%sE+00", std::string(dgt, '0').c_str());
    std::string s = body;
    const bool neg = std::signbit(v) && v != 0.0;
    if ((int)s.size() + 1 + (neg ? 1 : 0) <= w) s = "0" + s;
    if (neg) s = "-" + s;
    if ((int)s.size() < w) s = std::string(w - s.size(), ' ') + s;
    return s;
}

static void print_line(const ttx_engine *h, const ttx_sweep_rec &r, double val_prev)
{
    if (h->wrank != 0) return;
    const char *sd = r.dir == 0 ? "::" : r.dir == 1 ? ">>" : "<<";
    printf("%3d%2s rank%5.1f time: %s n_evals: %10lld", r.it, sd, r.erank, fmt_e(9, 3, r.seconds).c_str(), (long long)r.neval);
    if (h->P.has_quad) {
        if (r.it == 0) printf(" val %s", fmt_e(20, 14, r.val).c_str());
        else if (h->cfg.has_tru) printf(" err %s val %s", fmt_e(8, 3, std::fabs(1.0 - r.val / h->cfg.tru)).c_str(), fmt_e(20, 14, r.val).c_str());
        else printf(" cnv %s val %s", fmt_e(8, 3, std::fabs(1.0 - r.val / val_prev)).c_str(), fmt_e(20, 14, r.val).c_str());
    }
    printf("\n");
    fflush(stdout);
}

static int readback(ttx_engine *h)
{
    hipLaunchKernelGGL(k_collect, dim3(1), dim3(256), 0, h->stream, h->P);
    {
        int rc = allreduce_dev(h, h->P.sumsend, h->P.sumrecv, h->SB, 0);
        if (rc) return rc;
        HIPCHECK(hipMemcpyAsync(h->h_sum, h->P.sumrecv, sizeof(double) * h->SB, hipMemcpyDeviceToHost, h->stream));
        HIPCHECK(hipStreamSynchronize(h->stream));
        if (h->cb_error) return fail(TTX_EHIP, "host transport: a sendrecv / allreduce callback failed");
    }
    if (h->profile) ev_collect(h);
    return TTX_OK;
}
static inline const double *sum_bond(const ttx_engine *h, int p) { return h->h_sum + SUM_HDR + h->cfg.nproc + 5 * (size_t)p; }

static std::vector<int32_t> global_ranks(const ttx_engine *h)
{
    std::vector<int32_t> r(h->d + 1, 1);
    for (int p = 1; p < h->d; p++) r[p] = (int32_t)sum_bond(h, p)[0];
    return r;
}
static std::vector<int32_t> rank0_view(ttx_engine *h, int it)
{
    const int d = h->d;
    if (it == 0) { h->updhist.clear(); return std::vector<int32_t>(d + 1, 1); }
    std::vector<uint8_t> u(d + 1, 0);
    for (int p = 1; p < d; p++) u[p] = sum_bond(h, p)[1] > 0.0;
    h->updhist.push_back(u);
    std::vector<int32_t> r(d + 1, 1);
    for (int g = 0; g < h->cfg.nproc; g++) {
        int lag = std::max(0, g - 1), upto = it - lag;
        for (int p = h->own[g]; p < h->own[g + 1]; p++)
            for (int t = 1; t <= upto; t++) r[p] += h->updhist[t - 1][p];
    }
    return r;
}

static inline size_t lds_fpersist(const DevProb &P) { return (P.arith && P.fpersist) ? sizeof(double) * 4 * (P.d + 8) : 0; }

static int launch_quad(ttx_engine *h, hipStream_t sq, const DevProb &Q, int mode, const double *w)
{
    const size_t lds_q = sizeof(double) * ((size_t)h->RM * h->RM + 2);
    hipLaunchKernelGGL(k_quad_build, dim3(h->NC, h->G), dim3(256), lds_q, sq, Q, mode, w);
    hipLaunchKernelGGL(k_quad_chain, dim3(h->G), dim3(256), Q.qscr ? 0 : 2 * lds_q, sq, Q);
    if (h->cfg.nproc > 1) {
        int rc = allreduce_dev(h, Q.qsend, Q.qall, h->QB, 0);
        if (rc) return rc;
        hipLaunchKernelGGL(k_quad_tree, dim3(1), dim3(256), 0, sq, Q);
    }
    return TTX_OK;
}

struct KLaunch {
    const void *fn = nullptr; const char *name = "-"; dim3 grid, block; size_t lds = 0; bool raise = false;
    explicit operator bool() const { return fn != nullptr; }
};
template <class F>
static KLaunch kl(F *fn, const char *name, dim3 grid, dim3 block, size_t lds, bool raise = false)
{
    KLaunch k; k.fn = reinterpret_cast<const void *>(fn); k.name = name; k.grid = grid; k.block = block; k.lds = lds; k.raise = raise;
    return k;
}
template <class... A>
static void launch(hipStream_t st, const KLaunch &k, const A &...a)
{
    static_assert(((std::is_same<A, DevProb>::value || std::is_same<A, int>::value) && ...), "the chain kernels take a DevProb and ints");
    void *args[] = {(void *)&a...};
    (void)hipLaunchKernel(k.fn, k.grid, k.block, args, k.lds, st);
}
struct ChainPlan {
    KLaunch tables;
    KLaunch lottery, lot_eval;
    int lot_vals = 0;
    struct Tier { KLaunch k; int upto = 0; };
    Tier half[3]; int ntier = 0;
    int half_vals = -1;
    KLaunch base; int base_vals = 0;
    enum { FP_PLAIN, FP_MFMA, FP_COLUMNS } fullpiv = FP_PLAIN;
    KLaunch accept, init_samples, init_fibers, exch_boundary, fin_luar, fin_lual;
    KLaunch exch_tail;
    int nfb = 0, srows = 0, fl = 0;
    std::vector<const KLaunch *> all() const
    {
        std::vector<const KLaunch *> v = {&tables, &lottery, &lot_eval, &base, &accept, &init_samples, &init_fibers, &exch_boundary, &exch_tail, &fin_luar, &fin_lual};
        for (int t = 0; t < ntier; t++) v.push_back(&half[t].k);
        return v;
    }
};
#define KFUN_(k) (FUN == FUN_ISING ? #k "<ISING>" : FUN == FUN_STDNORM ? #k "<STDNORM>" : FUN == FUN_MVN ? #k "<MVN>" : #k "<HOST>")
#define KUNIT_(k, ...) (P.de_unit ? kl(k<true>, #k "<true>", __VA_ARGS__) : kl(k<false>, #k "<false>", __VA_ARGS__))
#define KUNIT2_(k, x, ...) (P.de_unit ? kl(k<true, x>, #k "<true," #x ">", __VA_ARGS__) : kl(k<false, x>, #k "<false," #x ">", __VA_ARGS__))
template <int FUN>
static ChainPlan chain_plan(const ttx_engine *h)
{
    const DevProb &P = h->P;
    const CreatePlan &s = h->sel;
    const int d = h->d, G = h->G, RM = h->RM, NM = h->NM, nproc = h->cfg.nproc;
    const bool fastk = P.arith && (FUN == FUN_MVN || s.isDE);
    const size_t VS = s.VS;
    ChainPlan p;
    p.nfb = s.nfb;
    p.base = kl(k_halfstep<FUN>, KFUN_(k_halfstep), dim3(p.nfb, G), dim3(TTX_BLK), s.lds_half, true);
    p.base_vals = fastk ? 0 : s.half_vals;
    p.lottery = kl(k_lottery<FUN>, "k_lottery", dim3(P.lot_nb, G), dim3(P.lot_nb == 1 ? 512 : 256), s.lds_lot, true);
    p.lot_vals = fastk ? s.fast_cap : s.lot_vals;
    const dim3 slots(s.de_slots, G), cand(P.lot_max, G), cand4((P.lot_max + 3) / 4, G);
    const KLaunch de = KUNIT_(k_halfstep_de, slots, dim3(64), s.lds_de, true);
    const KLaunch det3 = KUNIT2_(k_halfstep_det, 3, dim3(1, G), dim3(64 * 14), s.lds_det, true);
    const KLaunch det1 = KUNIT2_(k_halfstep_det, 1, dim3(1, G), dim3(64 * 6), s.lds_det6, true);
    const KLaunch de5 = KUNIT_(k_halfstep_de5, slots, dim3(64 * DE5_W), s.lds_de5, true);
    const KLaunch rows = KUNIT2_(k_lottery_eval_de_rows, false, cand4, dim3(64), s.lds_der, true);
    const KLaunch rows_tab = KUNIT2_(k_lottery_eval_de_rows, true, cand4, dim3(64), s.lds_der, true);
    if (fastk) p.lot_eval = KLaunch();
    else if (FUN == FUN_MVN && s.mvn_v2) p.lot_eval = kl(k_lottery_eval_mvn, "k_lottery_eval_mvn", cand, dim3(64), s.lds_mvn);
    else if (FUN == FUN_ISING && P.de_cut && s.de_v2 && s.lot_cand)
        p.lot_eval = s.de_lot_point ? kl(k_lottery_eval_decp, "k_lottery_eval_decp", cand, dim3(64), sizeof(double) * (2 * (size_t)(d + 64) + 2048), true)
                                    : kl(k_lottery_eval_dec, "k_lottery_eval_dec", cand, dim3(64), s.lds_de, true);
    else if (FUN == FUN_ISING && s.lot_wave) p.lot_eval = s.lot_rows == 2 ? rows_tab : rows;
    if (p.lot_eval) { p.lottery.grid = dim3(1, G); p.lottery.block = dim3(512); }
    if (fastk) { p.half[p.ntier++].k = p.base; p.half_vals = 0; }
    else if (FUN == FUN_MVN && s.mvn_v2) p.half[p.ntier++].k = kl(k_halfstep_mvn, "k_halfstep_mvn", slots, dim3(64), s.lds_mvn);
    else if (FUN == FUN_ISING && s.de_v2) {
        if (h->de_team() && !h->de_v5()) { p.half[p.ntier++] = {det3, s.de_team_units}; p.half[p.ntier++] = {det1, s.de_team6_units}; }
        p.half[p.ntier++].k = h->de_v5() ? de5 : P.de_cut ? kl(k_halfstep_dec, "k_halfstep_dec", slots, dim3(64), s.lds_de, true) : de;
    } else { p.half[p.ntier++].k = p.base; p.half_vals = s.half_vals; }
    p.fullpiv = FUN == FUN_HOST ? ChainPlan::FP_COLUMNS : P.fp_mfma ? ChainPlan::FP_MFMA : ChainPlan::FP_PLAIN;
    p.accept = kl(k_accept, "k_accept", dim3(2 * p.nfb + 2 * NM + 1, G), dim3(TTX_BLK), sizeof(double) * std::max<size_t>(RM + 2, (size_t)std::min<int>(RM, 64) * std::min<int>(RM, 64)));
    {
        const size_t lds_s = s.lds_par + 16 + sizeof(short) * 256 * VS;
        p.srows = lds_s <= TTX_LDS_WORK ? 1 : 0;
        p.init_samples = kl(k_init_samples<FUN>, KFUN_(k_init_samples), dim3(G), dim3(256), p.srows ? lds_s : s.lds_par, p.srows != 0);
        p.init_fibers = kl(k_init_fibers<FUN>, KFUN_(k_init_fibers), dim3(h->NC, G), dim3(256), s.lds_par);
    }
    if (s.de_npair) p.tables = P.de_cut ? kl(k_de_ctables, "k_de_ctables", dim3(2 * RM, G), dim3(256), sizeof(double) * (size_t)(d + 2))
                                    : kl(k_de_tables, "k_de_tables", dim3((2 * (d + 1) * RM + 255) / 256, G), dim3(256), 0);
    else if (fastk && !P.fpersist) p.tables = kl(k_fast_tables<FUN>, KFUN_(k_fast_tables), dim3(2 * RM, G), dim3(64), sizeof(double) * 2 * (d + 8));
    if (nproc > 1) {
        const size_t lds_b = s.lds_par + 16 + sizeof(short) * 2 * VS + sizeof(double) * (64 * 64 + 4) +
                             (P.bnd_wave ? sizeof(double) * (std::max<size_t>(2 * (size_t)de_rows_stride(d), 3 * (size_t)d + 2) + 8 + (P.de_cut ? 64 * 32 : 0)) : 0);
        p.exch_boundary = kl(k_exch_boundary<FUN>, KFUN_(k_exch_boundary), dim3(2 * NM, G), dim3(TTX_BLK), lds_b, true);
        if constexpr (FUN != FUN_HOST) p.exch_tail = kl(k_exch_tail<FUN>, KFUN_(k_exch_tail), dim3(2 * NM + 1, G), dim3(TTX_BLK), std::max(lds_b, lds_fpersist(P)), true);
    }
    {
        int ft = 256;
        while (ft > 64 && sizeof(double) * ((size_t)RM * RM + (size_t)ft * RM) > TTX_LDS_FIN) ft >>= 1;
        const size_t lds_f = sizeof(double) * ((size_t)RM * RM + (size_t)ft * RM);
        p.fl = lds_f <= TTX_LDS_WORK ? 1 : 0;
        const dim3 gr(h->NC, G, std::max(1, std::min(64, (NM * RM + ft - 1) / ft)));
        p.fin_luar = kl(k_fin_luar, "k_fin_luar", gr, dim3(ft), p.fl ? lds_f : 0, p.fl != 0);
        p.fin_lual = kl(k_fin_lual, "k_fin_lual", gr, dim3(ft), p.fl ? lds_f : 0, p.fl != 0);
    }
    return p;
}
#undef KFUN_
#undef KUNIT_
#undef KUNIT2_

#ifdef TTX_STAMPS
static int dump_stamps(ttx_engine *h)
{
    const DevProb &P = h->P;
    if (P.dbg) {
        std::vector<long long> hb(8 * 64 * 8);
        HIPCHECK(hipMemcpy(hb.data(), P.dbg, sizeof(long long) * hb.size(), hipMemcpyDeviceToHost));
        long long t0 = 0;
        for (long long v : hb) if (v && (!t0 || v < t0)) t0 = v;
        for (int hh = 0; hh < 8; hh++) {
            bool any = false;
            for (int w = 0; w < 64; w++) if (hb[((size_t)hh * 64 + w) * 8]) any = true;
            if (!any) continue;
            fprintf(stderr, "half-step %d (cycles since the first stamp; per wave: start eval-done reduced published polled reduced2)\n", hh);
            for (int w = 0; w < 64; w++) {
                const long long *e = &hb[((size_t)hh * 64 + w) * 8];
                if (!e[0]) continue;
                fprintf(stderr, "  blk %d wave %d: %7lld %7lld %7lld %7lld %7lld %7lld\n", w / 4, w % 4, e[0] - t0, e[1] - t0, e[2] - t0, e[3] - t0, e[4] - t0, e[5] - t0);
            }
        }
    }
    GroupState g0s;
    HIPCHECK(hipMemcpy(&g0s, P.gs, sizeof(GroupState), hipMemcpyDeviceToHost));
    for (int k = 0; k < 2; k++) {
        fprintf(stderr, "stamps kernel %d (n=%lld):", k, g0s.nstamp[k]);
        for (int x = 0; x < 16; x++) fprintf(stderr, " %.2fus", g0s.nstamp[k] ? 0.01 * (double)g0s.stamp[k][x] / (double)g0s.nstamp[k] : 0.0);
        fprintf(stderr, "\n");
    }
    return TTX_OK;
}
#endif

template <int FUN>
struct SweepRun {
    using clk = std::chrono::steady_clock;
    ttx_engine *const h; DevProb &P; const hipStream_t st;
    const int d, G, nproc, cluster, fused;
    const clk::time_point t0 = clk::now();
    LoopPlan L; ChainPlan plan;
    DevProb Pq;
    double val = 1.0, val_prev = 1.0;
    int strike = 0; bool ready = false, fin_enqueued = false;
    explicit SweepRun(ttx_engine *h_) : h(h_), P(h_->P), st(h_->stream), d(h_->d), G(h_->G), nproc(h_->cfg.nproc), cluster(h_->cluster_nb()), fused(h_->sel.fused) {}
    double since() const { return std::chrono::duration<double>(clk::now() - t0).count(); }
    template <class... A>
    int EV(const KLaunch &k, A... a)
    {
        if (FUN != FUN_HOST) { launch(st, k, P, a...); return TTX_OK; }
        DevProb Q = P;
        Q.hostpass = 1; launch(st, k, Q, a...);
        if (int rc = slot_eval(h)) return rc;
        Q.hostpass = 2; launch(st, k, Q, a...);
        return TTX_OK;
    }
    int prepare()
    {
        LoopIn in;
        in.whole = cluster || fused; in.cluster = cluster != 0; in.profile = h->profile; in.pipeline_off = env_off("TTX_PIPELINE");
        in.W = h->W; in.nproc = nproc; in.has_quad = P.has_quad; in.host_pass = FUN == FUN_HOST;
        in.sweep_tail = h->sel.sweep_tail; in.sweep_tail_side = h->sel.sweep_tail_side; in.maxrank = h->cfg.maxrank;
        L = loop_plan(in);
        P.tail_side = L.side ? 1 : 0;
        h->recs.clear(); h->tapes.clear();
        plan = chain_plan<FUN>(h);
        for (const KLaunch *k : plan.all()) if (k->raise) if (int rc = ensure_lds(h, k->fn, k->lds)) return rc;
        if (fused) if (int rc = ensure_lds(h, reinterpret_cast<const void *>(k_sweep_fused), h->sel.lds_fused)) return rc;
        if (cluster) { if (int rc = ensure_lds_cluster(h)) return rc; *h->h_abort = 0; }
        Pq = P;
        if (L.pipe) Pq.r = P.rq;
        hipLaunchKernelGGL(k_reset, dim3(64), dim3(256), 0, st, P, h->SB, h->QB);
        {
            KScope ks(h, TTX_K_OTHER, 4);
            if (int rc = EV(plan.init_samples, h->sel.snum, h->sel.nn, FUN == FUN_HOST ? 0 : plan.srows, 0)) return rc;
            if (int rc = EV(plan.init_fibers)) return rc;
            hipLaunchKernelGGL(k_init_factors, dim3(h->NC, G), dim3(256), lds_fpersist(P), st, P);
            hipLaunchKernelGGL(k_init_final, dim3(G), dim3(256), 0, st, P);
        }
        if (L.head) {
            hipLaunchKernelGGL(k_collect, dim3(1), dim3(256), 0, st, P);
            h->h_sum = h->h_sum_base;
            HIPCHECK(hipMemcpyAsync(h->h_sum, P.sumrecv, sizeof(double) * h->SB, hipMemcpyDeviceToHost, st));
            HIPCHECK(hipEventRecord(h->ev_sum[0], st));
            if (int rc = launch_sweep_kernel(1)) return rc;
            HIPCHECK(hipEventSynchronize(h->ev_sum[0]));
        } else if (int rc = readback(h)) return rc;
        HIPCHECK(hipGetLastError());
        for (int g = 0; g < nproc; g++) val = (g == 0) ? h->h_sum[SUM_HDR + g] : val * h->h_sum[SUM_HDR + g];
        if (!P.has_quad) val = 0.0;
        val_prev = val;
        record(0, 0);
        ready = (1 >= h->cfg.maxrank);
        return TTX_OK;
    }
    int launch_sweep_kernel(int it_)
    {
        const CreatePlan &s = h->sel;
        int dir = 2 - it_ % 2, epoch = it_, nsteps = h->nbmax, NB = s.cluster, ldsinv = s.cluster_ldsinv, zkeep = s.cluster_zkeep;
        const dim3 grid(8 * NB * ((G + 7) / 8)), block(CB);
        KScope ks(h, TTX_K_HALFSTEP, 1);
        if (!cluster) hipLaunchKernelGGL(k_sweep_fused, dim3(G), dim3(FB), s.lds_fused, st, P, dir, nsteps);
        else if (s.cluster_coop) {
            void *args[] = {&P, &dir, &nsteps, &NB, &ldsinv, &epoch, &zkeep};
            HIPCHECK(hipLaunchCooperativeKernel(reinterpret_cast<const void *>(cluster_kernel(s.cluster_var)), grid, block, args, (unsigned)s.lds_cluster, st));
        } else hipLaunchKernelGGL(cluster_kernel(s.cluster_var), grid, block, s.lds_cluster, st, P, dir, nsteps, NB, ldsinv, epoch, zkeep);
        return TTX_OK;
    }
    int enqueue_chain_sweep(int it_)
    {
        const int dir = 2 - it_ % 2;
        const int rb = std::min((int)h->RM, it_ + 1);
        const int units = (h->sel.de_test_fault && it_ == h->sel.de_test_fault) ? 1 : rb * ((h->NM + 63) / 64);
        KLaunch half = plan.half[plan.ntier - 1].k;
        for (int t = plan.ntier - 2; t >= 0; t--) if (units * G <= plan.half[t].upto) { half = plan.half[t].k; half.grid.x = units; }
        for (int pp = 1; pp <= h->nbmax; pp++) {
            if (plan.tables) { KScope ks(h, TTX_K_OTHER); launch(st, plan.tables, P, dir, pp); }
            if (h->cfg.pivoting < 0) { if (int rc = enqueue_full_pivoting(dir, pp, rb)) return rc; }
            else {
                if (plan.lot_eval) {
                    KScope ks(h, TTX_K_LOTTERY, 3);
                    launch(st, plan.lottery, P, dir, pp, plan.lot_vals, 1);
                    launch(st, plan.lot_eval, P);
                    launch(st, plan.lottery, P, dir, pp, plan.lot_vals, 2);
                } else { KScope ks(h, TTX_K_LOTTERY); if (int rc = EV(plan.lottery, dir, pp, plan.lot_vals, 0)) return rc; }
                KScope ks(h, TTX_K_HALFSTEP, h->H);
                for (int hh = 0; hh < h->H; hh++) {
                    if (plan.half_vals < 0) launch(st, half, P, hh, dir, h->mode);
                    else if (int rc = EV(half, hh, dir, h->mode, plan.half_vals)) return rc;
                }
            }
            { KScope ks(h, TTX_K_ACCEPT); launch(st, plan.accept, P, h->H, plan.nfb); }
        }
        return TTX_OK;
    }
    int enqueue_full_pivoting(int dir, int pp, int rb)
    {
        KScope ks(h, TTX_K_HALFSTEP, 5);
        KLaunch cols = plan.base;
        cols.grid.z = h->NM * h->RM;
        hipLaunchKernelGGL(k_bond_begin, dim3(G), dim3(64), 0, st, P, dir, pp);
        if (plan.fullpiv == ChainPlan::FP_MFMA) {
            const int side = h->RM * h->NM, gx = (side + 63) / 64;
            launch(st, cols, P, 0, dir, 4, plan.base_vals);
            hipLaunchKernelGGL(k_full_gemm_argmax, dim3(gx, gx, G), dim3(256), 0, st, P);
            hipLaunchKernelGGL(k_full_resolve2, dim3(G), dim3(256), 0, st, P, gx, gx);
        } else if (plan.fullpiv == ChainPlan::FP_COLUMNS) {
            for (int z = 0; z < h->NM * rb; z++) {
                DevProb Q = P;
                Q.zbase = z;
                Q.hostpass = 1; launch(st, plan.base, Q, 0, dir, 3, 0);
                if (int rc = slot_eval(h)) return rc;
                Q.hostpass = 2; launch(st, plan.base, Q, 0, dir, 3, 0);
            }
            hipLaunchKernelGGL(k_full_resolve, dim3(G), dim3(256), 0, st, P);
        } else {
            launch(st, cols, P, 0, dir, 3, plan.base_vals);
            hipLaunchKernelGGL(k_full_resolve, dim3(G), dim3(256), 0, st, P);
        }
        if (int rc = EV(plan.base, 0, dir, 2, plan.base_vals)) return rc;
        return EV(plan.base, 1, dir, 2, plan.base_vals);
    }
    int enqueue_sweep_end(int it_)
    {
        const int slot = it_ & 1;
        if (L.side) return end_side(it_);
        if (L.forkq) HIPCHECK(hipStreamWaitEvent(st, h->ev_val[slot ^ 1], 0));
        if (int rc = L.tail ? end_tail(it_) : end_classic(it_)) return rc;
        if (L.pipe) HIPCHECK(hipEventRecord(h->ev_sum[slot], st));
        if (!P.has_quad) return TTX_OK;
        if (L.forkq) HIPCHECK(hipStreamWaitEvent(h->qstream, h->ev_sum[slot], 0));
        return enqueue_quadrature(it_, L.forkq ? h->qstream : st);
    }
    int end_side(int it_)
    {
        const int slot = it_ & 1;
        HIPCHECK(hipStreamWaitEvent(st, h->ev_val[slot ^ 1], 0));
        KScope ks(h, TTX_K_EXCHANGE, 1);
        launch(st, plan.exch_tail, P, it_);
        HIPCHECK(hipEventRecord(h->ev_tail[slot], st));
        return TTX_OK;
    }
    int end_tail(int it_)
    {
        { KScope ks(h, TTX_K_EXCHANGE, 1); launch(st, plan.exch_tail, P, it_); }
        hipLaunchKernelGGL(k_sweep_end, dim3(1), dim3(256), 0, st, P, it_, h->h_sum_base + (size_t)(it_ & 1) * h->SB, 1);
        return TTX_OK;
    }
    int end_classic(int it_)
    {
        {
            KScope ks(h, TTX_K_EXCHANGE, (h->W > 1 ? 4 : 2) + (nproc > 1 ? 1 : 0));
            if (!cluster) hipLaunchKernelGGL(k_exch_pack, dim3(G), dim3(256), 0, st, P);
            if (h->W > 1) {
                hipLaunchKernelGGL(k_exch_localmax, dim3(1), dim3(64), 0, st, P);
                if (int rc = xfer_neighbours(h)) return rc;
                if (int rc = allreduce_dev(h, P.redsend, P.redrecv, 4, 1)) return rc;
            }
            hipLaunchKernelGGL(k_exch_max_apply, dim3(G), dim3(256), lds_fpersist(P), st, P, h->W > 1 ? 1 : 0, nproc > 1 ? 1 : 0);
            if (nproc > 1) { if (int rc = EV(plan.exch_boundary)) return rc; }
        }
        double *const pinned = h->h_sum_base + (size_t)(it_ & 1) * h->SB;
        if (L.pipe) hipLaunchKernelGGL(k_sweep_end, dim3(1), dim3(256), 0, st, P, it_, h->W > 1 ? P.sumsend : pinned, 0);
        if (L.pipe && h->W > 1) {
            if (int rc = allreduce_dev(h, P.sumsend, P.sumrecv, h->SB, 0)) return rc;
            HIPCHECK(hipMemcpyAsync(pinned, P.sumrecv, sizeof(double) * h->SB, hipMemcpyDeviceToHost, st));
        }
        return TTX_OK;
    }
    int enqueue_quadrature(int it_, hipStream_t sq)
    {
        const int slot = it_ & 1;
        KScope ks(h, TTX_K_QUAD, nproc > 1 ? 3 : 2);
        if (int rc = launch_quad(h, sq, L.pipe ? Pq : P, 0, P.quadw)) return rc;
        if (L.pipe) {
            HIPCHECK(hipMemcpyAsync(h->h_val + slot, &P.gs[0].val, sizeof(double), hipMemcpyDeviceToHost, sq));
            HIPCHECK(hipEventRecord(h->ev_val[slot], sq));
        }
        return h->cb_error ? fail(TTX_EHIP, "host transport: a sendrecv / allreduce callback failed") : TTX_OK;
    }
    int enqueue_side(int it_)
    {
        const int slot = it_ & 1;
        hipStream_t sq = h->qstream;
        HIPCHECK(hipStreamWaitEvent(sq, h->ev_tail[slot], 0));
        hipLaunchKernelGGL(k_sweep_summary, dim3(1), dim3(256), 0, sq, P, it_, h->h_sum_base + (size_t)slot * h->SB);
        HIPCHECK(hipEventRecord(h->ev_sum[slot], sq));
        return enqueue_quadrature(it_, sq);
    }
    int enqueue_final(int after_val)
    {
        if (fin_enqueued) return TTX_OK;
        fin_enqueued = true;
        if (after_val >= 0) HIPCHECK(hipStreamWaitEvent(st, h->ev_val[after_val], 0));
        HIPCHECK(hipMemsetAsync(P.ctl, 0, sizeof(int) * 3, st));
        KScope ks(h, TTX_K_OTHER, 2);
        if (nproc > 1) {
            hipLaunchKernelGGL(k_exch_pack, dim3(G), dim3(256), 0, st, P);
            if (int rc = xfer_neighbours(h)) return rc;
            hipLaunchKernelGGL(k_exch_apply, dim3(G), dim3(256), lds_fpersist(P), st, P);
        }
        launch(st, plan.fin_luar, P, plan.fl);
        launch(st, plan.fin_lual, P, plan.fl);
        return TTX_OK;
    }
    void record(int it_, int dir)
    {
        ttx_sweep_rec r{};
        r.it = it_; r.dir = dir; r.erank = erank_host(h, rank0_view(h, it_).data()); r.neval = (int64_t)h->h_sum[SUM_NEVAL]; r.val = val;
        r.amax = h->h_sum[SUM_AMAX]; r.pivotmax = it_ ? h->h_sum[SUM_PMAX] : -1; r.pivotmin = it_ ? h->h_sum[SUM_PMIN] : -1; r.seconds = since();
        h->recs.push_back(r);
        if (h->cfg.verbose) print_line(h, r, val_prev);
    }
    int process_sweep(int it_)
    {
        const int slot = it_ & 1;
        if (L.pipe) {
            HIPCHECK(hipEventSynchronize(h->ev_sum[slot]));
            h->h_sum = h->h_sum_base + (size_t)slot * h->SB;
        } else if (int rc = readback(h)) return rc;
        const StopRule sr = stop_rule(it_, h->cfg.maxrank, h->cfg.accuracy, h->h_sum[SUM_PMAX], h->h_sum[SUM_AMAX], strike);
        if (L.pipe && sr.ready) if (int rc = enqueue_final(P.has_quad ? slot : -1)) return rc;
        if (P.has_quad) {
            if (L.pipe) { HIPCHECK(hipEventSynchronize(h->ev_val[slot])); val = h->h_val[slot]; }
            else val = h->h_sum[SUM_VAL];
        }
        HIPCHECK(hipGetLastError());
        if (cluster && *(volatile int *)h->h_abort) { h->cluster_aborted = true; return fail(TTX_EHIP, "cluster sweep kernel: barrier timed out (workgroups of a bond group were not co-resident)"); }
        record(it_, 2 - it_ % 2);
        const size_t o = h->tapes.size();
        h->tapes.resize(o + (size_t)(d + 1) * 4, -1);
        for (int p = 1; p < d; p++) for (int x = 0; x < 4; x++) h->tapes[o + (size_t)p * 4 + x] = (int32_t)sum_bond(h, p)[1 + x];
        val_prev = val;
        strike = sr.strikes;
        ready = ready || sr.ready;
        return TTX_OK;
    }
    int run()
    {
        if (int rc = prepare()) return rc;
        if (!L.pipe) {
            for (int it = 1; !ready; it++) {
                if (int rc = (cluster || fused) ? launch_sweep_kernel(it) : enqueue_chain_sweep(it)) return rc;
                if (int rc = enqueue_sweep_end(it)) return rc;
                if (int rc = process_sweep(it)) return rc;
            }
        } else if (!ready) {
            if (L.forkq) { HIPCHECK(hipEventRecord(h->ev_val[0], h->qstream)); HIPCHECK(hipEventRecord(h->ev_val[1], h->qstream)); }
            if (!L.head) if (int rc = launch_sweep_kernel(1)) return rc;
            for (int it = 1; !ready; it++) {
                if (int rc = enqueue_sweep_end(it)) return rc;
                if (it + 1 < h->cfg.maxrank) if (int rc = launch_sweep_kernel(it + 1)) return rc;
                if (L.side) if (int rc = enqueue_side(it)) return rc;
                if (int rc = process_sweep(it)) return rc;
            }
        }
        if (int rc = enqueue_final(-1)) return rc;
        if (int rc = readback(h)) return rc;
        HIPCHECK(hipGetLastError());
#ifdef TTX_STAMPS
        if (int rc = dump_stamps(h)) return rc;
#endif
        h->neval = (int64_t)h->h_sum[SUM_NEVAL];
        h->k_bytes[TTX_K_HALFSTEP] += h->h_sum[SUM_BYTES];
        h->n_resid = (int64_t)h->h_sum[SUM_NRESID];
        h->rfinal = global_ranks(h);
        h->seconds = since();
        h->ran = true;
        return TTX_OK;
    }
};
template <int FUN>
static int run_impl(ttx_engine *h) { return SweepRun<FUN>(h).run(); }

template <class F>
static int with_fun(const ttx_engine *h, const char *who, F f)
{
    switch (h->cfg.fun_id) {
        case TTX_FUN_ISING: return f(std::integral_constant<int, FUN_ISING>());
        case TTX_FUN_STDNORM: return f(std::integral_constant<int, FUN_STDNORM>());
        case TTX_FUN_HOST:
            if (who && !h->hfun) return fail(TTX_ESTATE, "%s: call ttx_set_integrand_host first", who);
            return f(std::integral_constant<int, FUN_HOST>());
        case TTX_FUN_COSCOEFF: return f(std::integral_constant<int, FUN_HOST>());
        case TTX_FUN_DEVICE:
            if (who && !h->dfun) return fail(TTX_ESTATE, "%s: call ttx_set_integrand_device first", who);
            return f(std::integral_constant<int, FUN_HOST>());
        case TTX_FUN_TRAINS:
            if (who && !h->tfun) return fail(TTX_ESTATE, "%s: call ttx_set_integrand_trains first", who);
            return f(std::integral_constant<int, FUN_HOST>());
        default: return f(std::integral_constant<int, FUN_MVN>());
    }
}

static void reset_kernel_stats(ttx_engine *h)
{
    for (int k = 0; k < TTX_K_NKINDS; k++) { h->k_launches[k] = 0; h->k_ms[k] = 0; h->k_bytes[k] = 0; }
}
static void drain(ttx_engine *h) { (void)hipStreamSynchronize(h->stream); (void)hipStreamSynchronize(h->qstream); }
static int read_fault_counter(ttx_engine *h)
{
    int faults = 0;
    drain(h);
    if (hipMemcpy(&faults, h->P.ctl + 3, sizeof(int), hipMemcpyDeviceToHost) != hipSuccess) faults = 0;
    return faults;
}
static int replay(ttx_engine *h, void (*retire)(ttx_engine *))
{
    drain(h);
    (void)hipGetLastError();
    retire(h);
    reset_kernel_stats(h);
    return run_impl<FUN_ISING>(h);
}

extern "C" int ttx_run(ttx_engine *h)
{
    if (!h) return fail(TTX_EINVAL, "ttx_run: null handle");
    HIPCHECK(hipSetDevice(h->cfg.device));
    if (h->cfg.fun_id == 0) return fail(TTX_ESTATE, "ttx_run: this engine holds a loaded tensor train and has no integrand");
    reset_kernel_stats(h);
    if (h->cfg.fun_id == TTX_FUN_TRAINS) {
        if (int rc = tf_prepare(h, "ttx_run", true)) return rc;
        if (int rc = run_impl<FUN_HOST>(h)) return rc;
        return tf_finish(h);
    }
    if (h->cfg.fun_id != TTX_FUN_ISING)
        return with_fun(h, "ttx_run", [&](auto fun) { h->host_calls = 0; return run_impl<decltype(fun)::value>(h); });
    h->cluster_aborted = false;
    int rc = run_impl<FUN_ISING>(h);
    if (rc && h->cluster_aborted)
        rc = replay(h, [](ttx_engine *e) {
            *e->h_abort = 0;
            e->retired.cluster = true; e->cluster_aborted = false; e->cluster_fallbacks++;
            if (e->P.ising_id == 1) e->P.arith = 0;
        });
    if (h->de_team() && !h->de_v5() && read_fault_counter(h)) {
        (void)hipGetLastError();
        if (h->W > 1) return fail(TTX_EHIP, "ttx_run: k_halfstep_det met a rank above the host's bound; set TTX_DE_TEAM=0");
        rc = replay(h, [](ttx_engine *e) { e->retired.de_team = true; e->det_fallbacks++; });
    }
    if (h->de_v5()) if (const int faults = read_fault_counter(h)) {
        (void)hipGetLastError();
        if (h->W > 1) return fail(TTX_EHIP, "ttx_run: the wave relay of k_halfstep_de5 broke (%d hand-overs); set TTX_DE_V5=0", faults);
        rc = replay(h, [](ttx_engine *e) { e->retired.de_v5 = true; e->de5_fallbacks++; });
    }
    return rc;
}

extern "C" int ttx_plan_describe(const ttx_engine *h, char *buf, int64_t cap)
{
    if (!h || !buf || cap < 1) return fail(TTX_EINVAL, "ttx_plan_describe: null argument");
    if (h->cfg.fun_id == 0) return fail(TTX_ESTATE, "ttx_plan_describe: this engine holds a loaded tensor train and has no integrand");
    return with_fun(h, nullptr, [&](auto fun) {
        const ChainPlan p = chain_plan<decltype(fun)::value>(h);
        std::string s = std::string("path: ") + (h->cluster_nb() ? "cluster" : h->sel.fused ? "fused" : "chain") + "\ntables: " + p.tables.name + "\nlottery: ";
        if (h->cfg.pivoting < 0) s += "-";
        else s += p.lot_eval ? std::string(p.lottery.name) + " + " + p.lot_eval.name + " + " + p.lottery.name : std::string(p.lottery.name);
        s += "\nhalfstep: ";
        for (int t = 0; t < p.ntier; t++) s += std::string(t ? ", " : "") + p.half[t].k.name + (t + 1 < p.ntier ? "[<=" + std::to_string(p.half[t].upto) + "]" : "");
        if (h->cfg.pivoting < 0) s += std::string("\nfullpiv: ") + (p.fullpiv == ChainPlan::FP_MFMA ? "mfma" : p.fullpiv == ChainPlan::FP_COLUMNS ? "columns" : "plain");
        s += "\n";
        if ((int64_t)s.size() + 1 > cap) return fail(TTX_EINVAL, "ttx_plan_describe: the text needs %zu bytes", s.size() + 1);
        memcpy(buf, s.c_str(), s.size() + 1);
        return (int)TTX_OK;
    });
}

extern "C" int ttx_num_sweeps(const ttx_engine *h) { return h ? (int)h->recs.size() : 0; }
extern "C" int ttx_get_sweeps(const ttx_engine *h, ttx_sweep_rec *out, int cap)
{
    if (!h || !out) return fail(TTX_EINVAL, "ttx_get_sweeps: null argument");
    int n = std::min(cap, (int)h->recs.size());
    memcpy(out, h->recs.data(), sizeof(ttx_sweep_rec) * n);
    return TTX_OK;
}
extern "C" int ttx_get_tapes(const ttx_engine *h, int32_t *out, int64_t cap)
{
    if (!h || !out) return fail(TTX_EINVAL, "ttx_get_tapes: null argument");
    int64_t n = std::min<int64_t>(cap, (int64_t)h->tapes.size());
    memcpy(out, h->tapes.data(), sizeof(int32_t) * n);
    return TTX_OK;
}
extern "C" int64_t ttx_neval(const ttx_engine *h) { return h ? h->neval : 0; }
extern "C" double ttx_seconds(const ttx_engine *h) { return h ? h->seconds : 0.0; }
extern "C" int ttx_get_ranks(const ttx_engine *h, int32_t *r)
{
    if (!h || !r || !h->ran) return fail(TTX_ESTATE, "ttx_get_ranks: run first");
    memcpy(r, h->rfinal.data(), sizeof(int32_t) * (h->d + 1));
    return TTX_OK;
}
static int owner_of_core(const ttx_engine *h, int k)
{
    for (int g = 0; g < h->G; g++) {
        int first = h->own[h->g0 + g], last = h->own[h->g0 + g + 1] - 1;
        bool lastg = (h->g0 + g == h->cfg.nproc - 1);
        if (k >= first && (k <= last || (lastg && k == h->d))) return g;
    }
    return -1;
}
static double *core_dev(const ttx_engine *h, int k)
{
    const int g = owner_of_core(h, k), first = h->own[h->g0 + g];
    return h->P.arg + ((size_t)g * h->NC + (k - first)) * h->P.CS;
}
static void push_ranks(ttx_engine *h)
{
    std::vector<int32_t> rr((size_t)h->G * (h->d + 2), 1);
    for (int g = 0; g < h->G; g++) for (int p = 0; p <= h->d; p++) rr[(size_t)g * (h->d + 2) + p] = h->rfinal[p];
    (void)hipMemcpyAsync(h->P.r, rr.data(), sizeof(int32_t) * rr.size(), hipMemcpyHostToDevice, h->stream);
    (void)hipStreamSynchronize(h->stream);
// ... 2889 lines not shown
```

### ttcross_amd/csrc/ttx_kernels.h

```cpp
#pragma once
#include <hip/hip_runtime.h>
#include <limits.h>
#include <math.h>
#include "ttx_cdf.h"
#include "ttx_dev.h"
#include "ttx_exp.h"

#ifdef TTX_STAMPS
#define STAMP_DECL const bool t_me = (threadIdx.x == 0 && blockIdx.x == 0 && blockIdx.y == 0); long long t_prev = wall_clock64(); int t_slot = 0
#define STAMP(gs, k) do { __syncthreads(); if (t_me) { long long t_now = wall_clock64(); (gs).stamp[k][t_slot++] += t_now - t_prev; t_prev = t_now; } } while (0)
#define STAMP_END(gs, k) do { if (t_me) (gs).nstamp[k]++; } while (0)
#else
#define STAMP_DECL
#define STAMP(gs, k)
#define STAMP_END(gs, k)
#endif
#define FUN_ISING 1
#define FUN_STDNORM 2
#define FUN_MVN 3
#define FUN_HOST 4

__device__ __forceinline__ double *core_ptr(const DevProb &P, double *base, int g, int p, int first)
{ return base + ((size_t)g * P.NC + (p - first)) * P.CS; }
__device__ __forceinline__ double *inv_ptr(const DevProb &P, int g, int s, int first)
// ... 533 lines not shown
    if (ch < nfull) {
        if (!DESC && rem) ld8d(p + 8 * nfull, x);
#pragma unroll
        for (int k = 0; k < 8; k++) step(y[DESC ? 7 - k : k]);
        if (!DESC && rem) {
#pragma unroll
            for (int k = 0; k < 8; k++) if (k < rem) step(x[k]);
        }
    } else if (!DESC && rem) {
        if (nfull == 0) ld8d(p, y);
#pragma unroll
        for (int k = 0; k < 8; k++) if (k < rem) step(y[k]);
    }
}
__device__ __forceinline__ double f_ising_c3v(int m, int A, const double *an, const double *aw, double sn, double sw,
                                              const double *bn, const double *bw)
{
    const int nb = m - A - 1;
    double v = 1.0, w = 1.0, vk = 1.0, wk = 1.0;
    auto vstep = [&](double xv) { vk = vk * xv; v = v + vk; };
    auto wstep = [&](double xv) { wk = wk * xv; w = w + wk; };
    chain8v<true>(bn, nb, vstep);
    vstep(sn);
    chain8v<true>(an, A, vstep);
    chain8v<false>(an, A, wstep);
    wstep(sn);
    chain8v<false>(bn, nb, wstep);
    double b = 1.0 / (v * w);
    double f = 2 * b;
    auto fstep = [&](double xv) { f = f * xv; };
    chain8v<false>(aw, A, fstep);
    fstep(sw);
    chain8v<false>(bw, nb, fstep);
    return f;
}

template <int FUN, bool ALIGNED>
__device__ __forceinline__ double eval_src3(const DevProb &P, const double *par, const Src3 &S, long slot = -1)
{
    if (ALIGNED && FUN == FUN_ISING && P.ising_id == 1) return f_ising_c3(P.d, P.n[1], par, S);
    if (ALIGNED && FUN == FUN_ISING && P.arith) return f_ising_fast(P.ising_id, P.d, P.n[1], par, S);
    if (ALIGNED && FUN == FUN_ISING) return f_ising_de<1>(P.ising_id, P.d, P.n[1], par, S.pa, S.A, S.self, 0, S.pb, P.de_unit != 0);
    return eval_fun<FUN>(P, par, S, slot);
}

template <int CTRL, int ROWMASK>
__device__ __forceinline__ int dpp_i(int x) { return __builtin_amdgcn_update_dpp(x, x, CTRL, ROWMASK, 0xf, false); }
template <int CTRL, int ROWMASK>
__device__ __forceinline__ double dpp_d(double x)
{
    const long long b = __double_as_longlong(x);
    const int lo = dpp_i<CTRL, ROWMASK>((int)b), hi = dpp_i<CTRL, ROWMASK>((int)(b >> 32));
    return __longlong_as_double(((long long)hi << 32) | (unsigned int)lo);
}
__device__ __forceinline__ double readlane63(double x)
{
    const long long b = __double_as_longlong(x);
    const int lo = __builtin_amdgcn_readlane((int)b, 63), hi = __builtin_amdgcn_readlane((int)(b >> 32), 63);
    return __longlong_as_double(((long long)hi << 32) | (unsigned int)lo);
}
__device__ __forceinline__ double wave_max(double v)
{
    v = fmax(v, dpp_d<0xb1, 0xf>(v));
    v = fmax(v, dpp_d<0x4e, 0xf>(v));
    v = fmax(v, dpp_d<0x124, 0xf>(v));
    v = fmax(v, dpp_d<0x128, 0xf>(v));
    v = fmax(v, dpp_d<0x142, 0xa>(v));
    v = fmax(v, dpp_d<0x143, 0xc>(v));
    return readlane63(v);
}
template <int CTRL, int ROWMASK>
__device__ __forceinline__ void argmax_step(double &a, double &v, int &idx)
{
    const double a2 = dpp_d<CTRL, ROWMASK>(a), v2 = dpp_d<CTRL, ROWMASK>(v);
    const int i2 = dpp_i<CTRL, ROWMASK>(idx);
    if (a2 > a || (a2 == a && i2 < idx)) { a = a2; v = v2; idx = i2; }
}
__device__ __forceinline__ void wave_argmax(double &a, double &v, int &idx)
{
    argmax_step<0xb1, 0xf>(a, v, idx);
    argmax_step<0x4e, 0xf>(a, v, idx);
    argmax_step<0x124, 0xf>(a, v, idx);
    argmax_step<0x128, 0xf>(a, v, idx);
    argmax_step<0x142, 0xa>(a, v, idx);
    argmax_step<0x143, 0xc>(a, v, idx);
    a = readlane63(a); v = readlane63(v); idx = __builtin_amdgcn_readlane(idx, 63);
}
__device__ __forceinline__ double block_max(double v, double *sh)
{
    v = wave_max(v);
    int w = threadIdx.x >> 6, nw = (blockDim.x + 63) >> 6;
    __syncthreads();
    if ((threadIdx.x & 63) == 0) sh[w] = v;
    __syncthreads();
    double r = sh[0];
    for (int x = 1; x < nw; x++) r = fmax(r, sh[x]);
    return r;
}
__device__ __forceinline__ void block_argmax(double &a, double &v, int &idx, double *sha, double *shv, int *shi)
{
    wave_argmax(a, v, idx);
    int w = threadIdx.x >> 6, nw = (blockDim.x + 63) >> 6;
    __syncthreads();
    if ((threadIdx.x & 63) == 0) { sha[w] = a; shv[w] = v; shi[w] = idx; }
    __syncthreads();
    if (threadIdx.x == 0)
        for (int x = 1; x < nw; x++)
            if (sha[x] > a || (sha[x] == a && shi[x] < idx)) { a = sha[x]; v = shv[x]; idx = shi[x]; }
}

__device__ __forceinline__ void atomic_max_pos(double *addr, double v)
{
    atomicMax((unsigned long long *)addr, (unsigned long long)__double_as_longlong(v));
}
__device__ __forceinline__ double max_pos(double a, double b)
{ return ((unsigned long long)__double_as_longlong(b) > (unsigned long long)__double_as_longlong(a)) ? b : a; }

__device__ inline void resolve_state(StepState &c, const Partial *pt)
{
    if (!c.active || !c.pending) return;
    const int nb = c.npart;
    double ba = -1.0, bv = 0.0; int bi = INT_MAX;
    for (int b = 0; b < nb; b++) {
        double a = pt[b].absmax; int ix = pt[b].idx;
        if (a > ba || (a == ba && ix < bi)) { ba = a; bv = pt[b].val; bi = ix; }
    }
    c.done = take_pivot(c.pending == 1, bi, c.r0, c.n2, c.havecol, c.haverow, c.ii, c.jj, c.kk, c.qq);
    c.pivot = bv;
    c.pending = 0;
}

__device__ inline void resolve_state_wave(StepState &c, const StepState &src, const Partial *pt, int lane)
{
    double ba = -1.0, bv = 0.0; int bi = INT_MAX;
    const bool pend = src.active && src.pending;
    if (pend)
        for (int b = lane; b < src.npart; b += 64) {
            const double a = pt[b].absmax; const int ix = pt[b].idx;
            if (a > ba || (a == ba && ix < bi)) { ba = a; bv = pt[b].val; bi = ix; }
        }
    wave_argmax(ba, bv, bi);
    if (lane != 0) return;
    c = src;
    if (!pend) return;
    c.done = take_pivot(c.pending == 1, bi, c.r0, c.n2, c.havecol, c.haverow, c.ii, c.jj, c.kk, c.qq);
    c.pivot = bv;
    c.pending = 0;
}

struct DiagIdx { const int *n; int k, s; __device__ __forceinline__ int operator()(int p) const { return (k - 1 + s * (p - 1)) % n[p] + 1; } };
struct FixIdx { const int *ind; int self, selfval; __device__ __forceinline__ int operator()(int s) const { return s == self ? selfval : ind[s]; } };

template <int FUN>
__global__ __launch_bounds__(256) void k_init_samples(DevProb P, int snum, int nn, int ldsrows, int shift_hi)
{
    extern __shared__ __align__(16) double dyn[];
    double *par = dyn;
    __shared__ double sha[4], shv[4]; __shared__ int shi[4];
    const int g = blockIdx.x, tid = threadIdx.x;
    GroupState &gs = P.gs[g];
    for (int x = tid; x < P.npar; x += blockDim.x) par[x] = P.par[x];
    __syncthreads();
    double ba = -1.0, bv = 0.0; int bi = INT_MAX;
    const int m = P.d, VSr = ((m + 7) & ~7) + 8;
    short *rows = (short *)(((size_t)(dyn + P.npar) + 15) & ~(size_t)15);
    short *row = rows + (size_t)tid * VSr;
    if (FUN == FUN_ISING && P.arith && P.ising_id != 1 && ldsrows) {
        const int lane = tid & 63, wv = tid >> 6, nw = blockDim.x >> 6, n1m = P.n[1];
        double *xv = (double *)rows + (size_t)wv * 2 * (m + 64), *wvv = xv + (m + 64);
        int *nl = (int *)((double *)rows + (size_t)nw * 2 * (m + 64));
        for (int x = tid; x < m; x += blockDim.x) nl[x] = P.n[x + 1];
        __syncthreads();
        for (int il = wv; il < nn * snum; il += nw) {
            const int k = il % nn + 1, sft = il / nn;
            __builtin_amdgcn_wave_barrier();
            for (int x = lane; x < m; x += 64) { const int ix = (k - 1 + sft * x) % nl[x]; xv[x] = par[ix]; wvv[x] = par[n1m + ix]; }
            __builtin_amdgcn_wave_barrier();
            const double f = de_fast_point_wave(P.ising_id, m, xv, wvv, lane);
            const double a = fabs(f);
            if (lane == 0 && (a > ba || (a == ba && il < bi))) { ba = a; bv = f; bi = il; }
        }
    } else
    if (!ldsrows)
        for (int il = tid; il < nn * snum; il += blockDim.x) {
            DiagIdx ix{P.n, il % nn + 1, il / nn};
            double f = eval_fun<FUN>(P, par, ix, (long)g * P.HS + il);
            double a = fabs(f);
            if (a > ba || (a == ba && il < bi)) { ba = a; bv = f; bi = il; }
        }
    else
    for (int il = tid; il < nn * snum; il += blockDim.x) {
        const int k = il % nn + 1, sft = il / nn;
        for (int p = 1; p <= m; p++) row[p - 1] = (short)((k - 1 + sft * (p - 1)) % P.n[p] + 1);
        for (int x = m; x < VSr; x++) row[x] = 1;
        row[m - 1 + 0] = row[m - 1];
        const int self = row[m - 1];
        row[m - 1] = 1;
        Src3 sx{row, m - 1, self, row + m};
        double f = eval_src3<FUN, true>(P, par, sx, (long)g * P.HS + il);
        double a = fabs(f);
        if (a > ba || (a == ba && il < bi)) { ba = a; bv = f; bi = il; }
    }
    if (HOST_PASS1(FUN, P)) return;
    block_argmax(ba, bv, bi, sha, shv, shi);
    if (tid == 0) {
        gs.amax = ba;
        int gg = gs.gglobal;
        int lo = (int)((double)snum * (double)gg / P.nprocs);
        int hi = (gg + 1 == P.nprocs) ? snum : (int)((double)snum * (double)(gg + 1) / P.nprocs);
        gs.neval = (long long)nn * (hi - lo);
        if (g == 0) {
            if (bi == INT_MAX) bi = 0;
            int s = bi / nn, k = bi % nn + 1;
            for (int p = 1; p <= P.d; p++) P.ind0[p] = (k - 1 + s * (p - 1)) % P.n[p] + 1;
            P.ind0[P.d + 1] = 1;
        }
    }
}

template <int FUN>
__global__ __launch_bounds__(256) void k_init_fibers(DevProb P)
{
    extern __shared__ __align__(16) double dyn[];
    double *par = dyn;
    __shared__ double shm[4];
    const int g = blockIdx.y, tid = threadIdx.x;
    GroupState &gs = P.gs[g];
    const int p = gs.first + blockIdx.x;
    if (p > gs.last + 1) return;
    for (int x = tid; x < P.npar; x += blockDim.x) par[x] = P.par[x];
    __syncthreads();
    double *A = core_ptr(P, P.arg, g, p, gs.first);
    double mx = 0.0;
    for (int j = tid; j < P.n[p]; j += blockDim.x) {
        FixIdx ix{P.ind0, p, j + 1};
        double f = eval_fun<FUN>(P, par, ix, (long)g * P.HS + (long)blockIdx.x * P.NM + j);
        A[(size_t)P.RM * j] = f;
        mx = fmax(mx, fabs(f));
    }
    if (HOST_PASS1(FUN, P)) return;
    mx = block_max(mx, shm);
    if (tid == 0) { atomic_max_pos(&gs.amax, mx); atomicAdd((unsigned long long *)&gs.neval, (unsigned long long)P.n[p]); }
}

__global__ __launch_bounds__(256) void k_init_factors(DevProb P)
{
    const int g = blockIdx.y, tid = threadIdx.x;
    GroupState &gs = P.gs[g];
    const int first = gs.first, p = first + blockIdx.x, m = P.d;
    if (p > gs.last + 1) return;
    const double *A = core_ptr(P, P.arg, g, p, first);
    if (p <= gs.last) {
        double piv = A[(size_t)P.RM * (P.ind0[p] - 1)];
        double rp = 1.0 / piv;
        double *C = core_ptr(P, P.col, g, p, first);
        for (int j = tid; j < P.n[p]; j += blockDim.x) C[(size_t)P.RM * j] = rp * A[(size_t)P.RM * j];
        if (tid == 0) {
            inv_ptr(P, g, p, first)[0] = piv;
            int *v = vip_ptr(P, g, p, first);
            v[0] = 1; v[1] = P.ind0[p]; v[2] = P.ind0[p + 1]; v[3] = 1;
        }
    }
    if (p >= first + 1) {
        double *W = core_ptr(P, P.row, g, p, first);
        for (int k = tid; k < P.n[p]; k += blockDim.x) W[k] = A[(size_t)P.RM * k];
    }
    {
        int s = first - 1 + blockIdx.x;
        short *Lt = L_ptr(P, g, s, first);
        for (int x = tid; x < s; x += blockDim.x) Lt[(size_t)x * P.RM] = (short)P.ind0[x + 1];
        int s2 = first + blockIdx.x;
        short *Rt = R_ptr(P, g, s2, first);
        for (int x = tid; x < m - s2; x += blockDim.x) Rt[(size_t)x * P.RM] = (short)P.ind0[s2 + 1 + x];
        if (tid == 0 && blockIdx.x == 0) inv_ptr(P, g, first - 1, first)[0] = 1.0;
        if (P.arith && P.fpersist) {
            extern __shared__ __align__(16) double dyn_i[];
            const int wv_ = tid >> 6, lane_ = tid & 63;
            if (wv_ < 2) {
                double *xs = dyn_i + (size_t)wv_ * 2 * (m + 8), *ws = xs + m + 8;
                const int len = wv_ == 0 ? s : m - s2, o0 = wv_ == 0 ? 1 : s2 + 1, bnd = wv_ == 0 ? s : s2;
                if (P.fun_id == FUN_MVN) {
                    for (int k = lane_; k < len; k += 64) xs[k] = P.par[P.ind0[o0 + k] - 1] - P.aux[o0 - 1 + k];
                    __builtin_amdgcn_wave_barrier();
                    mvn_entry_scratch(P, xs, len, o0 - 1, fast_dv(P, wv_, g, bnd, first), fast_near(P, wv_, g, bnd, first), fast_piv(P, wv_, g, bnd, first), lane_);
                } else {
                for (int k = lane_; k < len; k += 64) { const int ix = P.ind0[o0 + k]; xs[k] = P.par[ix - 1]; ws[k] = P.par[P.n[1] + ix - 1]; }
                __builtin_amdgcn_wave_barrier();
                fast_entry_scratch(xs, ws, len, wv_, fast_near(P, wv_, g, bnd, first), fast_piv(P, wv_, g, bnd, first), P.RM, lane_);
                }
            }
        }
    }
}

__global__ __launch_bounds__(256) void k_init_final(DevProb P)
{
    __shared__ double dots[256];
    const int g = blockIdx.x, tid = threadIdx.x;
    GroupState &gs = P.gs[g];
    const bool lastgroup = (gs.last + 1 == P.d && gs.gglobal == P.nprocs - 1);
    const int ncore = gs.last - gs.first + 1 + (lastgroup ? 1 : 0);
    double val = 1.0;
    if (P.has_quad) {
        for (int c0 = 0; c0 < ncore; c0 += 256) {
            const int c = c0 + tid;
            if (c < ncore) {
                const int p = gs.first + c;
                const double *A = core_ptr(P, P.arg, g, p, gs.first), *w = P.quadw + (size_t)p * P.NM;
                double t = 0.0;
                for (int j = 0; j < P.n[p]; j++) t = t + A[(size_t)P.RM * j] * w[j];
                dots[tid] = t;
            }
            __syncthreads();
            if (tid == 0)
                for (int c2 = c0; c2 < min(ncore, c0 + 256); c2++) {
                    const int p = gs.first + c2;
                    if (p <= gs.last) val = val * dots[c2 - c0] / inv_ptr(P, g, p, gs.first)[0];
                    else val = val * dots[c2 - c0];
                }
            __syncthreads();
        }
    }
    if (tid == 0) { gs.pivotmax_prev = gs.amax; gs.pivotmax = -1.0; gs.pivotmin = -1.0; gs.initval = val; }
}

__global__ __launch_bounds__(256) void k_reset(DevProb P, size_t SB, size_t QB)
{
    const size_t t0 = (size_t)blockIdx.x * blockDim.x + threadIdx.x, nt = (size_t)gridDim.x * blockDim.x;
    const size_t nr = (size_t)P.G * (P.d + 2);
    for (size_t x = t0; x < nr; x += nt) { P.r[x] = 1; P.rr[x] = 1; P.upd[x] = 0; }
    for (size_t x = t0; x < 4 * nr; x += nt) P.tape[x] = -1;
    for (size_t x = t0; x < SB; x += nt) P.sumsend[x] = 0.0;
    for (size_t x = t0; x < QB; x += nt) P.qsend[x] = 0.0;
    if (t0 < 4) P.ctl[t0] = 0;
    if (t0 < 2) P.strk[t0] = 0;
    if (P.lot_ctr) for (size_t x = t0; x < (size_t)P.G; x += nt) P.lot_ctr[x] = 0u;
    if (P.cl_ctr) {
        for (size_t x = t0; x < (size_t)P.G; x += nt) P.cl_ctr[x] = 0u;
        ClPart z; z.ab = 0.0; z.bb = 0.0; z.mx = 0.0; z.ix = 0; z.pad = 0;
        for (size_t x = t0; x < (size_t)2 * P.G * TTX_CLREC; x += nt) P.cl_part[x] = z;
    }
    for (size_t g = t0; g < (size_t)P.G; g += nt) {
        GroupState &gs = P.gs[g];
        gs.amax = 0.0; gs.pivotmax = -1.0; gs.pivotmin = -1.0; gs.pivotmax_prev = 0.0;
        gs.neval = 0; gs.rngpos = 0; gs.val = 0.0; gs.initval = 0.0; gs.bytes_half = 0.0; gs.n_resid = 0;
        gs.amax_bnd[0] = 0.0; gs.amax_bnd[1] = 0.0;
#ifdef TTX_STAMPS
        for (int a = 0; a < 2; a++) { gs.nstamp[a] = 0; for (int b = 0; b < 16; b++) gs.stamp[a][b] = 0; }
#endif
    }
}

__device__ inline void bond_state(const DevProb &P, int g, int dir, int pp, StepState &st)
{
    GroupState &gs = P.gs[g];
    const int m = P.d;
    int *r = P.r + (size_t)g * (m + 2);
    if (pp == 1) sweep_start(P, g);
    int nb = gs.last - gs.first + 1;
    st.active = (pp <= nb);
    st.done = 0; st.havecol = 0; st.haverow = 0; st.crs = 0; st.pending = 0; st.npart = 0; st.pivot = 0.0;
    st.ii = st.jj = st.kk = st.qq = 0;
    if (st.active) {
        int p = (dir == 1) ? gs.first + pp - 1 : gs.last + 1 - pp;
        st.p = p; st.r0 = r[p - 1]; st.r1 = r[p]; st.r2 = r[p + 1]; st.n1 = P.n[p]; st.n2 = P.n[p + 1];
    } else { st.p = 0; st.r0 = st.r1 = st.r2 = st.n1 = st.n2 = 0; st.done = 1; }
}

__global__ void k_bond_begin(DevProb P, int dir, int pp)
{
    if (threadIdx.x != 0) return;
    StepState st;
    bond_state(P, blockIdx.x, dir, pp, st);
    P.gs[blockIdx.x].S[0] = st;
}
__global__ __launch_bounds__(256) void k_full_resolve(DevProb P)
{
    __shared__ double sha[4], shv[4]; __shared__ int shi[4];
    const int g = blockIdx.x, tid = threadIdx.x;
    GroupState &gs = P.gs[g];
    StepState st = gs.S[0];
    if (!st.active) return;
    const int nf = st.r0 * st.n1, nb = (nf + TTX_BLK - 1) / TTX_BLK, ncol = st.n2 * st.r2;
    double ba = -1.0, bv = 0.0; int bi = INT_MAX;
    for (int x = tid; x < ncol * nb; x += blockDim.x) {
        const Partial pr = P.pfull[((size_t)g * P.NM * P.RM + x / nb) * P.nfb + x % nb];
        if (pr.absmax > ba || (pr.absmax == ba && pr.idx < bi)) { ba = pr.absmax; bv = pr.val; bi = pr.idx; }
    }
    block_argmax(ba, bv, bi, sha, shv, shi);
    if (tid == 0) {
        int x = (bi == INT_MAX) ? 0 : bi;
        st.qq = x / (nf * st.n2) + 1; x %= nf * st.n2;
        st.kk = x / nf + 1; x %= nf;
        st.jj = x / st.r0 + 1; st.ii = x % st.r0 + 1;
        st.pivot = bv;
        gs.S[0] = st;
    }
}

typedef double dbl4_ __attribute__((ext_vector_type(4)));
__global__ __launch_bounds__(256) void k_full_gemm_argmax(DevProb P)
{
    __shared__ double Bt[64 * 65];
    __shared__ double sha[4], shv[4]; __shared__ int shi[4];
    const int g = blockIdx.z, tid = threadIdx.x, wave = tid >> 6, l = tid & 63;
    const GroupState &gs = P.gs[g];
    const StepState &st = gs.S[0];
    if (!st.active) return;
    const int p = st.p, r0 = st.r0, r1 = st.r1, r2 = st.r2, n1 = st.n1, n2 = st.n2, first = gs.first;
    const int nf = r0 * n1, nc = n2 * r2;
    const int tm = blockIdx.x * 64, tn = blockIdx.y * 64;
    if (tm >= nf || tn >= nc) return;
    const double *Cp = core_ptr(P, P.col, g, p, first), *Wq = core_ptr(P, P.row, g, p + 1, first);
    const double *sb = P.sb + (size_t)g * ((size_t)P.RM * P.NM) * ((size_t)P.RM * P.NM);
    for (int x = tid; x < r1 * 64; x += 256) {
        const int k = x >> 6, c = x & 63, col = tn + c;
        double v = 0.0;
        if (col < nc) { const int kk = col % n2, qq = col / n2; v = Wq[kk + (size_t)P.NM * qq + P.SW * k]; }
        Bt[k * 65 + c] = v;
    }
    __syncthreads();
    const int ar = tm + 16 * wave + (l & 15), kq = l >> 4;
    const bool arok = ar < nf;
    const size_t aoff = arok ? (size_t)(ar % r0) + (size_t)P.RM * (ar / r0) : 0;
    dbl4_ acc[4];
#pragma unroll
    for (int nt = 0; nt < 4; nt++) acc[nt] = dbl4_{0.0, 0.0, 0.0, 0.0};
    for (int k0 = 0; k0 < r1; k0 += 4) {
        const int k = k0 + kq;
        const double a = (arok && k < r1) ? Cp[aoff + P.SS * k] : 0.0;
#pragma unroll
        for (int nt = 0; nt < 4; nt++) {
            const double b = (k < r1) ? Bt[k * 65 + 16 * nt + (l & 15)] : 0.0;
            acc[nt] = __builtin_amdgcn_mfma_f64_16x16x4f64(a, b, acc[nt], 0, 0, 0);
        }
    }
    double ab = -1.0, bv = 0.0; int bi = INT_MAX;
#pragma unroll
    for (int nt = 0; nt < 4; nt++)
#pragma unroll
        for (int reg = 0; reg < 4; reg++) {
            const int row = tm + 16 * wave + (l >> 4) + 4 * reg, col = tn + 16 * nt + (l & 15);
            if (row < nf && col < nc) {
                const size_t ix = (size_t)row + (size_t)nf * col;
                const double b = sb[ix] - acc[nt][reg];
                const double a_ = fabs(b);
                if (a_ > ab || (a_ == ab && (int)ix < bi)) { ab = a_; bv = b; bi = (int)ix; }
            }
        }
    block_argmax(ab, bv, bi, sha, shv, shi);
    if (tid == 0) { Partial pr; pr.absmax = ab; pr.val = bv; pr.idx = bi; pr.pad = 0; P.pfull2[(size_t)g * P.fp_tiles + blockIdx.y * gridDim.x + blockIdx.x] = pr; }
}
__global__ __launch_bounds__(256) void k_full_resolve2(DevProb P, int gx, int gy)
{
    __shared__ double sha[4], shv[4]; __shared__ int shi[4];
    const int g = blockIdx.x, tid = threadIdx.x;
    GroupState &gs = P.gs[g];
    StepState st = gs.S[0];
    if (!st.active) return;
    const int nf = st.r0 * st.n1, nc = st.n2 * st.r2;
    const int ux = (nf + 63) / 64, uy = (nc + 63) / 64;
    double ba = -1.0, bv = 0.0; int bi = INT_MAX;
    for (int x = tid; x < ux * uy; x += blockDim.x) {
        const Partial pr = P.pfull2[(size_t)g * P.fp_tiles + (x / ux) * gx + (x % ux)];
        if (pr.absmax > ba || (pr.absmax == ba && pr.idx < bi)) { ba = pr.absmax; bv = pr.val; bi = pr.idx; }
    }
    block_argmax(ba, bv, bi, sha, shv, shi);
    if (tid == 0) {
        int x = (bi == INT_MAX) ? 0 : bi;
        st.qq = x / (nf * st.n2) + 1; x %= nf * st.n2;
        st.kk = x / nf + 1; x %= nf;
        st.jj = x / st.r0 + 1; st.ii = x % st.r0 + 1;
        st.pivot = bv;
        gs.S[0] = st;
    }
}
// ... 732 lines not shown
    }
}

struct ListIdx { const int *ind; __device__ __forceinline__ int operator()(int s) const { return ind[s - 1]; } };
template <int FUN>
__global__ void k_eval_list(DevProb P, long long npts, const int *ind, double *out)
{
    extern __shared__ __align__(16) double dyn[];
    for (int x = threadIdx.x; x < P.npar; x += blockDim.x) dyn[x] = P.par[x];
    __syncthreads();
    long long t = (long long)blockIdx.x * blockDim.x + threadIdx.x;
    if (t >= npts) return;
    ListIdx ix{ind + t * P.d};
    out[t] = eval_fun<FUN>(P, dyn, ix);
}

__global__ __launch_bounds__(TTX_BLK) void k_resid_argmax(int m, int r, size_t ld, const double *a, const double *F, const double *x,
                                                          double *b_out, Partial *parts)
{
    __shared__ double xs[256];
    __shared__ double sha[4], shv[4]; __shared__ int shi[4];
    for (int s = threadIdx.x; s < r; s += TTX_BLK) xs[s] = x[s];
    __syncthreads();
    int t = blockIdx.x * TTX_BLK + threadIdx.x;
    double b = 0.0, ab = -1.0; int bi = INT_MAX;
    if (t < m) {
        b = a[t];
#pragma unroll 8
        for (int s = 0; s < r; s++) b = b + (-xs[s]) * F[t + ld * s];
        b_out[t] = b; ab = fabs(b); bi = t;
    }
    block_argmax(ab, b, bi, sha, shv, shi);
    if (threadIdx.x == 0) { Partial pr; pr.absmax = ab; pr.val = b; pr.idx = bi; pr.pad = 0; parts[blockIdx.x] = pr; }
}

__global__ void k_lottery_only(int npnt, int m, int n, int nz, const int *zcol, const int *zrow, unsigned long long rngpos, int *points)
{
    __shared__ ttx_cdfseg segc[TTX_MAXSEG], segr[TTX_MAXSEG];
    __shared__ int nsc, nsr;
    if (threadIdx.x == 0) nsc = ttx_cdf_build(m - nz, segc);
    if (threadIdx.x == 64) nsr = ttx_cdf_build(n - nz, segr);
    __syncthreads();
    for (int il = threadIdx.x; il < npnt; il += blockDim.x) {
        double d1 = ttx_flang_draw(rngpos + il), d2 = ttx_flang_draw(rngpos + npnt + il);
        points[il] = ttx_lottery_index(segc, nsc, m - nz, m, zcol, nz, d1);
        points[npnt + il] = ttx_lottery_index(segr, nsr, n - nz, n, zrow, nz, d2);
    }
}

__device__ __forceinline__ void exch_pack_group(const DevProb &P, int g)
{
    const int tid = threadIdx.x, m = P.d;
    GroupState &gs = P.gs[g];
    const int first = gs.first, last = gs.last;
    const int *r = P.r + (size_t)g * (m + 2), *rr = P.rr + (size_t)g * (m + 2), *upd = P.upd + (size_t)g * (m + 2);
    if (tid == 0) {
        double *red = P.red + (size_t)g * 4;
        red[0] = gs.amax; red[1] = gs.pivotmax; red[2] = (gs.pivotmin > 0.0) ? -gs.pivotmin : -999e9;
    }
    {
        const int q = last, u = upd[q];
        char *base = P.msgR + (size_t)g * P.MSZ;
        int *hh = (int *)base; int *ix = hh + XH; double *dd = (double *)(base + P.IOFF);
        if (tid == 0) { hh[0] = u; hh[1] = r[q]; }
        const int rq = r[q];
        const double *gI = inv_ptr(P, g, q, first);
        for (int x = tid; x < rq * rq; x += blockDim.x) dd[(size_t)P.RM * P.NM + x] = gI[x];
        if (u) {
            const short *Lt = L_ptr(P, g, q, first);
            for (int x = tid; x < q; x += blockDim.x) ix[x] = Lt[(size_t)x * P.RM + (rq - 1)];
            const double *A = core_ptr(P, P.arg, g, q + 1, first);
            const int n2 = P.n[q + 1], rrq1 = rr[q + 1];
            for (int x = tid; x < n2 * rrq1; x += blockDim.x) dd[x] = A[(rq - 1) + (size_t)P.RM * (x % n2) + P.SS * (x / n2)];
        }
    }
    {
        const int q = first, u = upd[q];
        char *base = P.msgL + (size_t)g * P.MSZ;
        int *hh = (int *)base; int *ix = hh + XH; double *dd = (double *)(base + P.IOFF);
        if (tid == 0) { hh[0] = u; hh[1] = r[q]; }
        if (u) {
            const int rq = r[q];
            const short *Rt = R_ptr(P, g, q, first);
            for (int x = tid; x < m - q; x += blockDim.x) ix[x] = Rt[(size_t)x * P.RM + (rq - 1)];
            const double *A = core_ptr(P, P.arg, g, q, first);
            const int n1 = P.n[q], rr0 = rr[q - 1];
            for (int x = tid; x < rr0 * n1; x += blockDim.x) dd[x] = A[(x % rr0) + (size_t)P.RM * (x / rr0) + P.SS * (rq - 1)];
        }
    }
}

__device__ __forceinline__ void exch_pack_group(const DevProb &P, int g);
__device__ __forceinline__ void exch_apply_group(const DevProb &P, int g);

__global__ void k_exch_localmax(DevProb P)
{
    if (P.ctl[0]) return;
    if (threadIdx.x != 0 || blockIdx.x != 0) return;
    double a = -1e300, b = -1e300, c = -1e300;
    for (int g = 0; g < P.G; g++) { a = fmax(a, P.red[4 * g]); b = fmax(b, P.red[4 * g + 1]); c = fmax(c, P.red[4 * g + 2]); }
    P.redsend[0] = a; P.redsend[1] = b; P.redsend[2] = c; P.redsend[3] = 0.0;
}
__device__ __forceinline__ void exch_apply_group(const DevProb &P, int g)
{
    const int tid = threadIdx.x, m = P.d;
    GroupState &gs = P.gs[g];
    const int first = gs.first, last = gs.last;
    int *r = P.r + (size_t)g * (m + 2), *upd = P.upd + (size_t)g * (m + 2);
    if (P.inL[g]) {
        const int bl = first - 1;
        const int *hh = (const int *)P.inL[g], *ix = hh + XH; const double *dd = (const double *)(P.inL[g] + P.IOFF);
        const int u = hh[0], rnew = hh[1];
        if (u) { short *Lt = L_ptr(P, g, bl, first); for (int x = tid; x < bl; x += blockDim.x) Lt[(size_t)x * P.RM + (rnew - 1)] = (short)ix[x]; }
        double *gI = inv_ptr(P, g, bl, first);
        for (int x = tid; x < rnew * rnew; x += blockDim.x) gI[x] = dd[(size_t)P.RM * P.NM + x];
        if (tid == 0) { upd[bl] = u; r[bl] = rnew; }
        if (u && P.arith && P.fpersist && tid < 64) {
            extern __shared__ __align__(16) double dyn_x[];
            double *xs = dyn_x, *ws = xs + m + 8;
            if (P.fun_id == FUN_MVN) {
                for (int k = tid; k < bl; k += 64) xs[k] = P.par[ix[k] - 1] - P.aux[k];
                __builtin_amdgcn_wave_barrier();
                mvn_entry_scratch(P, xs, bl, 0, fast_dv(P, 0, g, bl, first) + (rnew - 1), fast_near(P, 0, g, bl, first) + (rnew - 1), fast_piv(P, 0, g, bl, first) + (rnew - 1), tid);
            } else {
            for (int k = tid; k < bl; k += 64) { xs[k] = P.par[ix[k] - 1]; ws[k] = P.par[P.n[1] + ix[k] - 1]; }
            __builtin_amdgcn_wave_barrier();
            fast_entry_scratch(xs, ws, bl, 0, fast_near(P, 0, g, bl, first) + (rnew - 1), fast_piv(P, 0, g, bl, first) + (rnew - 1), P.RM, tid);
            }
        }
    }
    if (P.inR[g]) {
        const int br = last + 1;
        const int *hh = (const int *)P.inR[g], *ix = hh + XH;
        const int u = hh[0], rnew = hh[1];
        if (u) { short *Rt = R_ptr(P, g, br, first); for (int x = tid; x < m - br; x += blockDim.x) Rt[(size_t)x * P.RM + (rnew - 1)] = (short)ix[x]; }
        if (tid == 0) { upd[br] = u; r[br] = rnew; }
        if (u && P.arith && P.fpersist && tid >= 64 && tid < 128) {
            extern __shared__ __align__(16) double dyn_x[];
            double *xs = dyn_x + 2 * (m + 8), *ws = xs + m + 8;
            const int lane_ = tid - 64;
            if (P.fun_id == FUN_MVN) {
                for (int k = lane_; k < m - br; k += 64) xs[k] = P.par[ix[k] - 1] - P.aux[br + k];
                __builtin_amdgcn_wave_barrier();
                mvn_entry_scratch(P, xs, m - br, br, fast_dv(P, 1, g, br, first) + (rnew - 1), fast_near(P, 1, g, br, first) + (rnew - 1), fast_piv(P, 1, g, br, first) + (rnew - 1), lane_);
            } else {
            for (int k = lane_; k < m - br; k += 64) { xs[k] = P.par[ix[k] - 1]; ws[k] = P.par[P.n[1] + ix[k] - 1]; }
            __builtin_amdgcn_wave_barrier();
            fast_entry_scratch(xs, ws, m - br, 1, fast_near(P, 1, g, br, first) + (rnew - 1), fast_piv(P, 1, g, br, first) + (rnew - 1), P.RM, lane_);
            }
        }
    }
}

__global__ __launch_bounds__(256) void k_exch_pack(DevProb P) { if (P.ctl[0]) return; exch_pack_group(P, blockIdx.x); }
__global__ __launch_bounds__(256) void k_exch_apply(DevProb P) { exch_apply_group(P, blockIdx.x); }

__device__ __forceinline__ void exch_max_group(const DevProb &P, int g, int from_recv)
{
    double a = -1e300, b = -1e300, c = -1e300;
    if (from_recv) { a = P.redrecv[0]; b = P.redrecv[1]; c = P.redrecv[2]; }
    else for (int x = 0; x < P.G; x++) { a = fmax(a, P.red[4 * x]); b = fmax(b, P.red[4 * x + 1]); c = fmax(c, P.red[4 * x + 2]); }
    GroupState &gs = P.gs[g];
    gs.amax = a; gs.pivotmax = b; gs.pivotmin = (-c == 999e9) ? -1.0 : -c;
    gs.pivotmax_prev = b;
}
__global__ __launch_bounds__(256) void k_exch_max_apply(DevProb P, int from_recv, int do_apply)
{
    if (P.ctl[0]) return;
    const int g = blockIdx.x;
    if (threadIdx.x == 0) exch_max_group(P, g, from_recv);
    if (do_apply) exch_apply_group(P, g);
}

template <bool FAST> __device__ __forceinline__ double rows_span(double a, double u0, const double *xs, int L, bool neutral0, int n);
__host__ __device__ inline int de_rows_stride(int m);
__device__ __forceinline__ double de_finish_vals(int id, double a, int m, const double *xv, const double *wv);
__device__ __forceinline__ double de_pairs_point_wave_cut(int m, const double *xv, double *sf, int lane)
{
        double a = 1.0;
        for (int base = 0; base < m; base += 64) {
            const int row = base + lane;
            double u = 1.0, fr[32];
            int L = 0; bool on = row < m;
#pragma unroll
            for (int c = 0; c < 32; c++) {
                fr[c] = 1.0;
                if (on && row + c < m) { u = u * xv[row + c]; if (u > 0x1p-54) { fr[c] = de_t2<true>(u); L = c + 1; } else on = false; }
                else on = false;
            }
            const bool lng = (L == 32) && (row + 32 < m) && (u > 0x1p-54);
            if (__builtin_amdgcn_ballot_w64(lng) != 0ull) {
                const int rend = (base + 64 < m) ? base + 64 : m;
                for (int r = base; r < rend; r++) {
                    double uu = 1.0;
                    for (int j = r; j < m; j++) { uu = uu * xv[j]; if (uu <= 0x1p-54) break; a = a * de_t2<true>(uu); }
                }
                continue;
            }
            int inc = L;
#pragma unroll
            for (int o = 1; o < 64; o <<= 1) { const int y = __shfl_up(inc, o, 64); if (lane >= o) inc += y; }
            const int off = inc - L, total = __shfl(inc, 63, 64);
            __builtin_amdgcn_wave_barrier();
#pragma unroll
            for (int c = 0; c < 32; c++) if (c < L) sf[off + c] = fr[c];
            __builtin_amdgcn_wave_barrier();
            int t = 0;
            for (; t + 16 <= total; t += 16) {
                double f16[16];
#pragma unroll
                for (int k = 0; k < 8; k++) { const Double2 q2 = *reinterpret_cast<const Double2 *>(sf + t + 2 * k); f16[2 * k] = q2.a; f16[2 * k + 1] = q2.b; }
#pragma unroll
                for (int k = 0; k < 16; k++) a = a * f16[k];
            }
            for (; t < total; t++) a = a * sf[t];
        }
        return a;
}
__device__ __forceinline__ double de_corner_wave(const DevProb &P, const double *par, const short *rowA, int p, int self, const short *rowB,
                                                 double *scratch, int lane)
{
    const int m = P.d, RSW = de_rows_stride(m), n1m = P.n[1], n = lane & 15;
    double *xv = scratch, *wv = xv + RSW;
    for (int x = lane; x < m; x += 64) {
        const int ix = ((x < p - 1) ? (int)rowA[x] : (x == p - 1) ? self : (int)rowB[x - p]) - 1;
        xv[x] = par[ix]; wv[x] = par[n1m + ix];
    }
    if (lane < 56) xv[m + lane] = 1.0;
    __builtin_amdgcn_wave_barrier();
    if (P.arith) return de_fast_point_wave(P.ising_id, m, xv, wv, lane);
    if (P.de_cut) return de_finish_vals(P.ising_id, de_pairs_point_wave_cut(m, xv, (double *)(((size_t)(wv + RSW) + 15) & ~(size_t)15), lane), m, xv, wv);
    double a = 1.0;
    if (P.de_unit) for (int i = 0; i < m; i++) a = rows_span<true>(a, 1.0, xv + i, m - i, false, n);
    else for (int i = 0; i < m; i++) a = rows_span<false>(a, 1.0, xv + i, m - i, false, n);
    return de_finish_vals(P.ising_id, a, m, xv, wv);
}

__device__ __forceinline__ double mvn_quadform_wave(int m, const double *dv, int L, double dL, const double *icT, double *tb, int lane);
__device__ __forceinline__ double mvn_corner_wave(const DevProb &P, const double *par, const short *rowA, int p, int self, const short *rowB,
                                                  double *scratch, int lane)
{
    const int m = P.d;
    double *dv = scratch, *tb = scratch + ((m + 1) & ~1);
    for (int x = lane; x < m; x += 64) {
        const int ix = ((x < p - 1) ? (int)rowA[x] : (x == p - 1) ? self : (int)rowB[x - p]) - 1;
        dv[x] = par[ix] - P.aux[x];
    }
    __builtin_amdgcn_wave_barrier();
    if (P.arith) return mvn_fast_point_wave(P, dv, lane);
    const double ex = mvn_quadform_wave(m, dv, -1, 0.0, P.auxT, tb, lane);
    return ttx_exp(-0.5 * ex) / P.mvn_norm;
}

template <int FUN, bool MSG>
__device__ __forceinline__ void exch_boundary_block(const DevProb &P, int bx, int g, int par_)
{
    extern __shared__ __align__(16) double dyn[];
    __shared__ double s_bc;
    const int tid = threadIdx.x, m = P.d;
    GroupState &gs = P.gs[g];
    double *amax_to = MSG ? &gs.amax_bnd[par_] : &gs.amax;
    const int first = gs.first, last = gs.last;
    const int *r = P.r + (size_t)g * (m + 2), *rr = P.rr + (size_t)g * (m + 2), *upd = P.upd + (size_t)g * (m + 2);
    double *par = dyn;
    const int VSr = ((m + 7) & ~7) + 8;
    short *rowA = (short *)(((size_t)(dyn + P.npar) + 15) & ~(size_t)15), *rowB = rowA + VSr;
    double *lu = (double *)(rowB + VSr);
    double *wscr = lu + 64 * 64 + 4;
    __shared__ double s_corner;
    const bool dewave = (FUN == FUN_ISING) && P.ising_id != 1 && P.bnd_wave;
    const bool mvwave = (FUN == FUN_MVN) && P.bnd_wave;
    if (bx < P.NM) {
        const int k = bx, p = last, br = last + 1;
        if (!P.inR[g]) return;
        const int *hh = (const int *)P.inR[g], *ix = hh + XH;
        if (!(MSG ? hh[0] : upd[br]) || k >= P.n[br]) return;
        const int rp = r[p], rrp = rr[p], snew = (MSG ? hh[1] : r[br]) - 1, n2 = P.n[br];
        const double *msg = (const double *)(P.inR[g] + P.IOFF);
        double *A = core_ptr(P, P.arg, g, br, first), *W = core_ptr(P, P.row, g, br, first);
        double a = 0.0;
        if (tid < rrp) a = msg[tid + (size_t)rrp * k];
        if (upd[p]) {
            for (int x = tid; x < P.npar; x += TTX_BLK) par[x] = P.par[x];
            const int *vp = vip_ptr(P, g, p, first) + 4 * (rp - 1);
            const short *Lt = L_ptr(P, g, p - 1, first), *Rt = R_ptr(P, g, br, first);
            auto dimv = [&](int s) -> short { return (s < p) ? Lt[(size_t)(s - 1) * P.RM + (vp[0] - 1)] : (s == p) ? (short)vp[1] : (s == p + 1) ? (short)(k + 1) : MSG ? (short)ix[s - p - 2] : Rt[(size_t)(s - p - 2) * P.RM + snew]; };
            for (int x = tid; x < VSr; x += TTX_BLK) { rowA[x] = (x < p - 1) ? dimv(x + 1) : (short)1; rowB[x] = (x < m - p) ? dimv(p + 1 + x) : (short)1; }
            __syncthreads();
            if (dewave || mvwave) {
                if (tid < 64) {
                    const double c_ = dewave ? de_corner_wave(P, par, rowA, p, (int)vp[1], rowB, wscr, tid) : mvn_corner_wave(P, par, rowA, p, (int)vp[1], rowB, wscr, tid);
                    if (tid == 0) s_corner = c_;
                }
                __syncthreads();
            }
            if (tid == rrp) {
                Src3 sx{rowA, p - 1, (int)vp[1], rowB};
                a = (dewave || mvwave) ? s_corner : eval_src3<FUN, true>(P, par, sx, (long)g * P.HS + k);
                if (!HOST_PASS1(FUN, P)) {
                    atomic_max_pos(amax_to, fabs(a));
                    if (!MSG && k == 0) atomicAdd((unsigned long long *)&gs.neval, (unsigned long long)n2);
                }
            }
        }
        if (HOST_PASS1(FUN, P)) return;
        if (tid < rp) A[tid + (size_t)P.RM * k + P.SS * snew] = a;
        const double *gI = inv_ptr(P, g, p, first);
        double tmp = 0.0, xf = 0.0;
        if (rp <= 64) {
            __syncthreads();
            for (int x = tid; x < rp * rp; x += TTX_BLK) lu[x] = gI[x];
            __syncthreads();
            if (tid < 64) xf = wave_solve_L(lu, rp, a, tid, 64);
        } else
        for (int s = 0; s < rp; s++) {
            if (tid == s) { xf = (s == 0) ? a : a + (-1.0) * tmp; s_bc = xf; }
            __syncthreads();
            if (tid > s && tid < rp) tmp = tmp + s_bc * gI[tid * tid + s];
            __syncthreads();
        }
        if (tid < rp) W[k + (size_t)P.NM * snew + P.SW * tid] = xf;
    } else {
        const int j = bx - P.NM, p = first, bl = first - 1;
        if (!P.inL[g]) return;
        const int *hh = (const int *)P.inL[g], *ix = hh + XH;
        if (!(MSG ? hh[0] : upd[bl]) || j >= P.n[p]) return;
        const int rp = r[p], rrp = rr[p], inew = (MSG ? hh[1] : r[bl]) - 1, n1 = P.n[p];
        const double *msg = (const double *)(P.inL[g] + P.IOFF);
        double *A = core_ptr(P, P.arg, g, p, first), *C = core_ptr(P, P.col, g, p, first);
        double y = 0.0;
        if (tid < rrp) y = msg[j + (size_t)n1 * tid];
        if (upd[p]) {
            for (int x = tid; x < P.npar; x += TTX_BLK) par[x] = P.par[x];
            const int *vp = vip_ptr(P, g, p, first) + 4 * (rp - 1);
            const short *Lt = L_ptr(P, g, bl, first), *Rt = R_ptr(P, g, p + 1, first);
            auto dimv = [&](int s) -> short { return (s < p) ? (MSG ? (short)ix[s - 1] : Lt[(size_t)(s - 1) * P.RM + inew]) : (s == p) ? (short)(j + 1) : (s == p + 1) ? (short)vp[2] : Rt[(size_t)(s - p - 2) * P.RM + (vp[3] - 1)]; };
            for (int x = tid; x < VSr; x += TTX_BLK) { rowA[x] = (x < p - 1) ? dimv(x + 1) : (short)1; rowB[x] = (x < m - p) ? dimv(p + 1 + x) : (short)1; }
            __syncthreads();
            if (dewave || mvwave) {
                if (tid < 64) {
                    const double c_ = dewave ? de_corner_wave(P, par, rowA, p, j + 1, rowB, wscr, tid) : mvn_corner_wave(P, par, rowA, p, j + 1, rowB, wscr, tid);
                    if (tid == 0) s_corner = c_;
                }
                __syncthreads();
            }
            if (tid == rrp) {
                Src3 sx{rowA, p - 1, j + 1, rowB};
                y = (dewave || mvwave) ? s_corner : eval_src3<FUN, true>(P, par, sx, (long)g * P.HS + P.NM + j);
                if (!HOST_PASS1(FUN, P)) {
                    atomic_max_pos(amax_to, fabs(y));
                    if (!MSG && j == 0) atomicAdd((unsigned long long *)&gs.neval, (unsigned long long)n1);
                }
            }
        }
        if (HOST_PASS1(FUN, P)) return;
        if (tid < rp) A[inew + (size_t)P.RM * j + P.SS * tid] = y;
        const double *gI = inv_ptr(P, g, p, first);
        if (rp <= 64) {
            __syncthreads();
            for (int x = tid; x < rp * rp; x += TTX_BLK) lu[x] = gI[x];
            __syncthreads();
            if (tid < 64) y = wave_solve_U(lu, rp, y, wave_solve_rdg(lu, rp, tid), tid, 64);
        } else
        for (int s = 0; s < rp; s++) {
            if (tid == s) { y = (1.0 / gI[(s + 1) * (s + 1) - 1]) * y; s_bc = y; }
            __syncthreads();
            if (tid > s && tid < rp) y = y + (-gI[tid * tid + tid + s]) * s_bc;
            __syncthreads();
        }
        if (tid < rp) C[inew + (size_t)P.RM * j + P.SS * tid] = y;
    }
}
template <int FUN>
__global__ __launch_bounds__(TTX_BLK) void k_exch_boundary(DevProb P)
{
    if (P.ctl[0]) return;
    exch_boundary_block<FUN, false>(P, (int)blockIdx.x, (int)blockIdx.y, 0);
}
template <int FUN>
__global__ __launch_bounds__(TTX_BLK) void k_exch_tail(DevProb P, int it)
{
    if (P.ctl[0]) return;
    const int g = blockIdx.y;
    if ((int)blockIdx.x < 2 * P.NM) { exch_boundary_block<FUN, true>(P, (int)blockIdx.x, g, it & 1); return; }
    if (threadIdx.x == 0) {
        exch_max_group(P, g, 0);
        GroupState &gs = P.gs[g];
        const int *upd = P.upd + (size_t)g * (P.d + 2);
        const int u_r = P.inR[g] ? ((const int *)P.inR[g])[0] : 0, u_l = P.inL[g] ? ((const int *)P.inL[g])[0] : 0;
        gs.neval += boundary_neval(P.inR[g] != nullptr, u_r, upd[gs.last], P.n[gs.last + 1], P.inL[g] != nullptr, u_l, upd[gs.first], P.n[gs.first]);
    }
    exch_apply_group(P, g);
    if (!P.tail_side) return;
    __syncthreads();
    const int m = P.d, tid = threadIdx.x, par = it & 1;
    const GroupState &gs = P.gs[g];
    const int *r = P.r + (size_t)g * (m + 2), *tp = P.tape + (size_t)g * (m + 2) * 4;
    int *rq = P.rq + (size_t)g * (m + 2), *tq = P.tail_tape + ((size_t)par * P.G + g) * (m + 2) * 4;
    for (int x = tid; x < m + 2; x += blockDim.x) rq[x] = r[x];
    for (int x = 4 * gs.first + tid; x < 4 * (gs.last + 1); x += blockDim.x) tq[x] = tp[x];
    if (tid == 0) {
        TailRec t;
        t.amax = gs.amax; t.pivotmax = gs.pivotmax; t.pivotmin = gs.pivotmin; t.bytes_half = gs.bytes_half; t.initval = gs.initval;
        t.neval = gs.neval; t.n_resid = gs.n_resid;
        P.tailrec[(size_t)par * P.G + g] = t;
    }
}
__global__ __launch_bounds__(256) void k_sweep_summary(DevProb P, int it, double *out)
{
    const int m = P.d, tid = threadIdx.x, par = it & 1;
    if (tid == 0) P.ctl[2] = P.ctl[0];
    if (P.ctl[0]) return;
    const TailRec *rec = P.tailrec + (size_t)par * P.G;
    const int p_lo = P.gs[0].first, p_hi = P.gs[P.G - 1].last;
    for (int p = p_lo + tid; p <= p_hi; p += blockDim.x) {
        int g = 0;
        while (g + 1 < P.G && P.gs[g + 1].first <= p) g++;
        const int *r = P.rq + (size_t)g * (m + 2), *tp = P.tail_tape + ((size_t)par * P.G + g) * (m + 2) * 4;
        double *e = out + SUM_HDR + P.nprocs + 5 * p;
        e[0] = (double)r[p]; e[1] = (double)tp[4 * p]; e[2] = (double)tp[4 * p + 1]; e[3] = (double)tp[4 * p + 2]; e[4] = (double)tp[4 * p + 3];
    }
    if (tid < P.G) out[SUM_HDR + P.gs[tid].gglobal] = rec[tid].initval;
    if (tid != 0) return;
    double nev = 0.0, by = 0.0, nr = 0.0;
    for (int g = 0; g < P.G; g++) { nev += (double)rec[g].neval; by += rec[g].bytes_half; nr += (double)rec[g].n_resid; }
    const double amax = max_pos(rec[0].amax, P.gs[0].amax_bnd[par]), pmax = rec[0].pivotmax;
    out[SUM_NEVAL] = nev; out[SUM_BYTES] = by; out[SUM_NRESID] = nr;
    out[SUM_AMAX] = amax; out[SUM_PMAX] = pmax; out[SUM_PMIN] = rec[0].pivotmin;
    out[SUM_VAL] = 0.0;
    const StopRule s = stop_rule(it, P.maxrank, P.accuracy, pmax, amax, P.strk[(it - 1) & 1]);
    P.strk[par] = s.strikes;
    P.ctl[1] = s.strikes;
    if (s.ready) {
        for (int g = 0; g < P.G; g++) P.gs[g].amax = max_pos(P.gs[g].amax, P.gs[g].amax_bnd[par]);
        P.ctl[0] = 1;
    }
}

__global__ __launch_bounds__(256) void k_quad_tree(DevProb P)
{
    if (P.ctl[2]) return;
    const int tid = threadIdx.x, RM = P.RM, ng = P.nprocs;
    __shared__ int mym[256], myn[256];
    const double *part = P.qall, *dims = P.qall + (size_t)ng * RM * RM;
    double *work = P.qwork;
    for (int g = tid; g < ng; g += blockDim.x) { mym[g] = (int)dims[2 * g]; myn[g] = (int)dims[2 * g + 1]; }
    __syncthreads();
    for (int g = 0; g < ng; g++)
        for (int x = tid; x < mym[g] * myn[g]; x += blockDim.x) work[(size_t)g * RM * RM + (x % mym[g]) + RM * (x / mym[g])] = part[(size_t)g * RM * RM + (x % mym[g]) + RM * (x / mym[g])];
    __syncthreads();
    double *tmp = work + (size_t)ng * RM * RM;
    for (int q = 1; q < ng; q *= 2) {
        for (int me = 0; me + q < ng; me += 2 * q) {
            const int her = me + q;
            const double *Aa = work + (size_t)me * RM * RM, *Bb = work + (size_t)her * RM * RM;
            const int mm = mym[me], kk = myn[me], nn = myn[her];
            for (int x = tid; x < mm * nn; x += blockDim.x) {
                int i = x % mm, j = x / mm;
                double c = 0.0;
                for (int l = 0; l < kk; l++) c = c + Bb[l + RM * j] * Aa[i + RM * l];
                tmp[i + RM * j] = c;
            }
            __syncthreads();
            double *dst = work + (size_t)me * RM * RM;
            for (int x = tid; x < mm * nn; x += blockDim.x) dst[(x % mm) + RM * (x / mm)] = tmp[(x % mm) + RM * (x / mm)];
            __syncthreads();
            if (tid == 0) myn[me] = nn;
            __syncthreads();
        }
    }
    if (tid == 0) for (int g = 0; g < P.G; g++) P.gs[g].val = work[0];
}

__device__ __forceinline__ void collect_summary(const DevProb &P);
__global__ __launch_bounds__(256) void k_collect(DevProb P)
{
    if (blockIdx.x != 0 || P.ctl[0]) return;
    collect_summary(P);
}
__global__ __launch_bounds__(256) void k_sweep_end(DevProb P, int it, double *out, int fold)
{
    const int n = P.G * (P.d + 2), m = P.d, tid = threadIdx.x;
    for (int x = tid; x < n; x += blockDim.x) P.rq[x] = P.r[x];
    if (tid == 0) P.ctl[2] = P.ctl[0];
    if (P.ctl[0]) return;
    if (fold) {
        if (tid < P.G) {
            GroupState &gs = P.gs[tid];
            gs.amax = max_pos(gs.amax, gs.amax_bnd[it & 1]);
            gs.amax_bnd[it & 1] = 0.0;
        }
        __syncthreads();
    }
    const int p_lo = P.gs[0].first, p_hi = P.gs[P.G - 1].last;
    for (int p = p_lo + tid; p <= p_hi; p += blockDim.x) {
        int g = 0;
        while (g + 1 < P.G && P.gs[g + 1].first <= p) g++;
        const int *r = P.r + (size_t)g * (m + 2), *tp = P.tape + (size_t)g * (m + 2) * 4;
        double *e = out + SUM_HDR + P.nprocs + 5 * p;
        e[0] = (double)r[p]; e[1] = (double)tp[4 * p]; e[2] = (double)tp[4 * p + 1]; e[3] = (double)tp[4 * p + 2]; e[4] = (double)tp[4 * p + 3];
    }
    if (tid < P.G) out[SUM_HDR + P.gs[tid].gglobal] = P.gs[tid].initval;
    if (tid != 0) return;
    double nev = 0.0, by = 0.0, nr = 0.0;
    for (int g = 0; g < P.G; g++) { const GroupState &gs = P.gs[g]; nev += (double)gs.neval; by += gs.bytes_half; nr += (double)gs.n_resid; }
    const double amax = P.gs[0].amax, pmax = P.gs[0].pivotmax;
    out[SUM_NEVAL] = nev; out[SUM_BYTES] = by; out[SUM_NRESID] = nr;
    if (P.g0 == 0) { out[SUM_AMAX] = amax; out[SUM_PMAX] = pmax; out[SUM_PMIN] = P.gs[0].pivotmin; }
    out[SUM_VAL] = 0.0;
    const StopRule s = stop_rule(it, P.maxrank, P.accuracy, pmax, amax, P.ctl[1]);
    P.ctl[1] = s.strikes;
    P.ctl[0] = s.ready;
}
__device__ __forceinline__ void collect_summary(const DevProb &P)
{
    const int m = P.d, tid = threadIdx.x;
    double *o = P.sumsend;
    for (int g = 0; g < P.G; g++) {
        const GroupState &gs = P.gs[g];
        const int *r = P.r + (size_t)g * (m + 2), *tp = P.tape + (size_t)g * (m + 2) * 4;
        for (int p = gs.first + tid; p <= gs.last; p += blockDim.x) {
            double *e = o + SUM_HDR + P.nprocs + 5 * p;
            e[0] = (double)r[p]; e[1] = (double)tp[4 * p]; e[2] = (double)tp[4 * p + 1]; e[3] = (double)tp[4 * p + 2]; e[4] = (double)tp[4 * p + 3];
        }
    }
    if (tid != 0) return;
    double nev = 0.0, by = 0.0, nr = 0.0;
    for (int g = 0; g < P.G; g++) {
        const GroupState &gs = P.gs[g];
        nev += (double)gs.neval; by += gs.bytes_half; nr += (double)gs.n_resid;
        o[SUM_HDR + gs.gglobal] = gs.initval;
        if (gs.gglobal == 0) { o[SUM_AMAX] = gs.amax; o[SUM_PMAX] = gs.pivotmax; o[SUM_PMIN] = gs.pivotmin; }
    }
    o[SUM_NEVAL] = nev; o[SUM_BYTES] = by; o[SUM_NRESID] = nr;
    if (P.g0 == 0) o[SUM_VAL] = P.gs[0].val;
}

__global__ void k_fill_synth(double *p, size_t n, unsigned long long seed)
{
    for (size_t i = (size_t)blockIdx.x * blockDim.x + threadIdx.x; i < n; i += (size_t)gridDim.x * blockDim.x) {
        unsigned long long x = (i + 1) * 0x9E3779B97F4A7C15ull + seed; x ^= x >> 29; x *= 0xBF58476D1CE4E5B9ull; x ^= x >> 32;
        p[i] = (double)(x >> 11) * (1.0 / 9007199254740992.0) - 0.5;
    }
}
__global__ __launch_bounds__(TTX_BLK) void k_resid_argmax_stream(long long m, int r, size_t ld, const double *a, const double *F, const double *x,
                                                                 double *b_out, Partial *parts)
{
    __shared__ double xs[256];
    __shared__ double sha[4], shv[4]; __shared__ int shi[4];
    for (int s = threadIdx.x; s < r; s += TTX_BLK) xs[s] = x[s];
    __syncthreads();
    double ab = -1.0, bv = 0.0; int bi = INT_MAX;
    for (long long t = (long long)blockIdx.x * TTX_BLK + threadIdx.x; t < m; t += (long long)gridDim.x * TTX_BLK) {
        double b = a[t];
#pragma unroll 8
        for (int s = 0; s < r; s++) b = b + (-xs[s]) * F[t + ld * s];
        b_out[t] = b;
        double aa = fabs(b);
        if (aa > ab || (aa == ab && (int)t < bi)) { ab = aa; bv = b; bi = (int)t; }
    }
    block_argmax(ab, bv, bi, sha, shv, shi);
    if (threadIdx.x == 0) { Partial pr; pr.absmax = ab; pr.val = bv; pr.idx = bi; pr.pad = 0; parts[blockIdx.x] = pr; }
}

template <int FUN>
__global__ __launch_bounds__(64) void k_accchk(DevProb P, unsigned long long rngpos, int nlot, const int *owner, double *out, int *ind_out, int il0)
{
    extern __shared__ __align__(16) double dyn[];
    const int il = il0 + blockIdx.x, tid = threadIdx.x, m = P.d;
    double *par = dyn, *x = dyn + ((P.npar + 1) & ~1), *z = x + P.RM;
    int *ind = (int *)(z + P.RM);
    for (int s = tid; s < P.npar; s += 64) par[s] = P.par[s];
    for (int i = tid; i < m; i += 64) {
        double d = ttx_flang_draw(rngpos + (unsigned long long)il * m + i);
        ind[i] = (int)(d * P.n[i + 1]) + 1;
        ind_out[(size_t)il * m + i] = ind[i];
    }
    __syncthreads();
    double aval = 0.0;
    if (tid == 0) { ListIdx ix{ind}; aval = eval_fun<FUN>(P, par, ix, (long)blockIdx.x); }
    if (HOST_PASS1(FUN, P)) return;
    {
        const int g = owner[m], first = P.gs[g].first;
        const int *r = P.r + (size_t)g * (m + 2);
        const double *A = core_ptr(P, P.arg, g, m, first);
        if (tid < r[m - 1]) x[tid] = A[tid + (size_t)P.RM * (ind[m - 1] - 1)];
    }
    __syncthreads();
    for (int i = m - 1; i >= 1; i--) {
        const int g = owner[i], first = P.gs[g].first;
        const int *r = P.r + (size_t)g * (m + 2);
        const int q0 = r[i - 1], q1 = r[i];
        const double *A = core_ptr(P, P.arg, g, i, first) + (size_t)P.RM * (ind[i - 1] - 1);
        for (int t = tid; t < q0; t += 64) {
            double s = 0.0;
            for (int k = 0; k < q1; k++) s = s + A[t + P.SS * k] * x[k];
            z[t] = s;
        }
        __syncthreads();
        for (int t = tid; t < q0; t += 64) x[t] = z[t];
// ... 8 lines not shown
```

### ttcross_amd/csrc/ttx_loop_plan.h

```cpp
#pragma once

struct LoopIn {
    bool whole = false;
    bool cluster = false;
    bool profile = false;
    bool pipeline_off = false;
    int W = 1;
    int nproc = 1;
    bool has_quad = false;
    bool host_pass = false;
    bool sweep_tail = false;
    bool sweep_tail_side = false;
    int maxrank = 1;
};

struct LoopPlan {
    bool pipe = false;
    bool head = false;
    bool forkq = false;
    bool tail = false;
    bool side = false;
};

inline LoopPlan loop_plan(const LoopIn &in)
{
    LoopPlan p;
    p.pipe = in.whole && !in.profile && !in.pipeline_off;
    p.head = p.pipe && in.W == 1 && in.maxrank > 1;
    p.forkq = p.pipe && in.has_quad && in.W == 1;
    p.tail = p.pipe && in.cluster && in.W == 1 && in.nproc > 1 && !in.host_pass && in.sweep_tail;
    p.side = p.tail && p.forkq && in.sweep_tail_side;
    return p;
}
```

Measured before the change: 233.0 million evals/s.

## Trim run head and tail: direct init summary, early finish, LDS quad tree

Several head/tail optimizations land together. k_init_final now writes the summary straight to pinned host memory, which skips the collect kernel and memcpy before the first sweep. Its dot products are computed per wave. k_init_samples gets a wider block with LDS-cached dims. The final stage starts once the quad build finishes rather than after the value readback, and skips the final exchange when sweeps already ran. k_quad_tree runs its matrix product tree in LDS with double buffering. Each piece aims to cut fixed per-run latency at the start and end of dtt_dmrgg, but it adds more env-switchable paths and the risk of subtle ordering bugs.

Measured after the change: 236.4 million evals/s, median of 6. 1.5% higher.

```diff
diff --git a/profiles/trace_timeline.py b/profiles/trace_timeline.py
--- a/profiles/trace_timeline.py
+++ b/profiles/trace_timeline.py
@@ -46,6 +46,39 @@
             print(f"    gap {med(p[3][k][1] for p in ps):6.1f}  dur {med(p[3][k][2] for p in ps):6.1f}  {nm}")
         print(f"    gap {med(p[4] for p in ps):6.1f}  k_sweep_cluster (next)")
     sys.exit(0)
+if start == "ends":
+    med = statistics.median
+    resets = [i for i, r in enumerate(rows) if 'k_reset' in r['Kernel_Name']]
+    heads, tails = {}, {}
+    for a, b in zip(resets, resets[1:]):
+        run = rows[a:b]
+        sw = [i for i, r in enumerate(run) if 'k_sweep_cluster' in r['Kernel_Name']]
+        real = [i for i in sw if int(run[i]['End_Timestamp']) - int(run[i]['Start_Timestamp']) > 20000]
+        if not real:
+            continue
+        main = run[0]['Queue_Id']
+        q = lambda r: 'main' if r['Queue_Id'] == main else 'side'
+        t0 = int(run[0]['Start_Timestamp'])
+        seg = [(q(r), short(r['Kernel_Name']), (int(r['Start_Timestamp']) - t0) / 1e3, (int(r['End_Timestamp']) - t0) / 1e3) for r in run[:sw[0]]]
+        seg.append(('main', 'k_sweep_cluster (first) starts', (int(run[sw[0]]['Start_Timestamp']) - t0) / 1e3, (int(run[sw[0]]['Start_Timestamp']) - t0) / 1e3))
+        heads.setdefault(tuple(x[:2] for x in seg), []).append(seg)
+        t1 = int(run[real[-1]]['End_Timestamp'])
+        rest = [r for r in run[real[-1] + 1:] if int(r['End_Timestamp']) > t1]
+        seg = [(q(r), short(r['Kernel_Name']), (int(r['Start_Timestamp']) - t1) / 1e3, (int(r['End_Timestamp']) - t1) / 1e3) for r in rest]
+        seg.append(('main', 'k_reset (next run) starts', (int(rows[b]['Start_Timestamp']) - t1) / 1e3, (int(rows[b]['Start_Timestamp']) - t1) / 1e3))
+        tails.setdefault(tuple(x[:2] for x in seg), []).append(seg)
+    for title, shapes in (("head: start of k_reset -> start of the first k_sweep_cluster", heads),
+                          ("end: finish of the last sweeping k_sweep_cluster -> finish of the last kernel", tails)):
+        for names, segs in sorted(shapes.items(), key=lambda kv: -len(kv[1]))[:2]:
+            total = [max(x[3] for x in s[:-1]) if len(s) > 1 else 0.0 for s in segs] if title[0] == 'e' else [s[-1][3] for s in segs]
+            print(f"{title}: {len(segs)} runs, median {med(total):.1f} us (min {min(total):.1f}, max {max(total):.1f})")
+            busy = {'main': 0.0, 'side': 0.0}
+            for k, (qq, nm) in enumerate(names):
+                st_, en_ = med(s[k][2] for s in segs), med(s[k][3] for s in segs)
+                gap = st_ - busy[qq]
+                busy[qq] = max(busy[qq], en_)
+                print(f"    {qq}  start {st_:7.1f}  end {en_:7.1f}  dur {med(s[k][3] - s[k][2] for s in segs):6.1f}  gap on its queue {gap:6.1f}  {nm}")
+    sys.exit(0)
 if start == "run":
     inits = [i for i, r in enumerate(rows) if 'k_init_samples' in r['Kernel_Name']]
     i0 = inits[2] - 8
diff --git a/ttcross_amd/csrc/ttx_create_plan.h b/ttcross_amd/csrc/ttx_create_plan.h
--- a/ttcross_amd/csrc/ttx_create_plan.h
+++ b/ttcross_amd/csrc/ttx_create_plan.h
@@ -56,6 +56,12 @@
     bool mvn_v2_off = false;
     bool tail_off = false;
     bool tail_side_off = false;
+    bool head_direct_off = false;
+    bool init_wave_off = false;
+    bool fin_early_off = false;
+    bool fin_skip_exch_off = false;
+    bool init_wide_off = false;
+    bool quad_lds_off = false;
 };
 template <class Get>
 CreateEnv create_env_from(Get get)
@@ -83,6 +89,9 @@
     v.lottery_rows2 = num("TTX_LOTTERY_ROWS", 0) == 2;
     v.mvn_v2_off = off("TTX_MVN_V2");
     v.tail_off = off("TTX_TAIL"); v.tail_side_off = off("TTX_TAIL_SIDE");
+    v.head_direct_off = off("TTX_HEAD_DIRECT"); v.init_wave_off = off("TTX_INIT_WAVE");
+    v.fin_early_off = off("TTX_FIN_EARLY"); v.fin_skip_exch_off = off("TTX_FIN_SKIP_EXCH");
+    v.init_wide_off = off("TTX_INIT_WIDE"); v.quad_lds_off = off("TTX_QUAD_LDS");
     return v;
 }
 struct DevCaps { int ncu = 0; bool coop = false; };
@@ -132,10 +141,35 @@
     int cl_test_abort = 0; bool dbg_waves = false;
     bool sweep_tail = true;
     bool sweep_tail_side = true;
+    bool head_direct = true;
+    size_t lds_qtree = 0;
+    bool init_wide = true;
+    bool init_wave = true;
+    bool fin_early = true;
+    bool fin_skip_exch = true;
     SweepWant sweep_want = SWEEP_AUTO; int ncu = 0;
     int fused = 0;
     int cluster = 0;
 };
+
+inline size_t quad_tree_lds(int nproc, size_t RM, bool on)
+{
+    const size_t need = sizeof(double) * 2 * (size_t)nproc * RM * RM;
+    return on && nproc > 1 && need <= TTX_LDS_WORK ? need : 0;
+}
+struct InitSamplesPlan { int threads = 256, rows = 0; size_t lds = 0; };
+inline InitSamplesPlan init_samples_plan(size_t lds_par, size_t VS, int d, long nsamples, bool own_rows, bool wide)
+{
+    InitSamplesPlan p;
+    const size_t lds1 = lds_par + 16 + sizeof(short) * 256 * VS;
+    p.rows = lds1 <= TTX_LDS_WORK ? 1 : 0;
+    p.lds = p.rows ? lds1 : lds_par;
+    if (!p.rows || !wide || !own_rows) return p;
+    const int threads = (int)std::min<long>(512, std::max<long>(256, (nsamples + 63) / 64 * 64));
+    const size_t lds2 = lds_par + 16 + sizeof(short) * (size_t)threads * VS + 16 + sizeof(int) * (size_t)(d + 1);
+    if (lds2 <= TTX_LDS_WORK) { p.threads = threads; p.rows = 2; p.lds = lds2; }
+    return p;
+}
 
 inline void share(int first, int last, int nproc, std::vector<int32_t> &own)
 {
@@ -224,6 +258,7 @@
     p.IOFF = (sizeof(int) * (XH + d + 2) + 15) & ~(size_t)15;
     p.MSZ = (p.IOFF + sizeof(double) * p.XD + 15) & ~(size_t)15;
     p.QB = (size_t)nproc * RM * RM + 2 * nproc;
+    p.lds_qtree = quad_tree_lds(nproc, RM, !env.quad_lds_off);
     p.SB = SUM_HDR + nproc + 5 * (size_t)(d + 1);
     p.qscr = 2 * sizeof(double) * (RM * RM + 2) > TTX_LDS_WORK;
     p.nn = cfg.n[0];
@@ -313,6 +348,8 @@
         }
         p.cl_test_abort = env.cluster_test_abort; p.dbg_waves = env.dbg_waves;
         p.sweep_tail = !env.tail_off; p.sweep_tail_side = !env.tail_side_off;
+        p.head_direct = !env.head_direct_off; p.init_wave = !env.init_wave_off; p.init_wide = !env.init_wide_off;
+        p.fin_early = !env.fin_early_off; p.fin_skip_exch = !env.fin_skip_exch_off;
         const std::string want_sweep = env.sweep.set ? env.sweep.v : "auto";
         if (want_sweep == "cluster") p.sweep_want = SWEEP_CLUSTER;
         else if (want_sweep == "fused") p.sweep_want = SWEEP_FUSED;
diff --git a/ttcross_amd/csrc/ttx_engine.hip b/ttcross_amd/csrc/ttx_engine.hip
--- a/ttcross_amd/csrc/ttx_engine.hip
+++ b/ttcross_amd/csrc/ttx_engine.hip
@@ -197,7 +197,7 @@
     bool cluster_aborted = false;
     double *h_svd = nullptr; double svd_seq = 0.0;
     hipStream_t qstream = nullptr;
-    hipEvent_t ev_sum[2] = {nullptr, nullptr}, ev_val[2] = {nullptr, nullptr}, ev_tail[2] = {nullptr, nullptr};
+    hipEvent_t ev_sum[2] = {nullptr, nullptr}, ev_val[2] = {nullptr, nullptr}, ev_tail[2] = {nullptr, nullptr}, ev_qb[2] = {nullptr, nullptr}, ev_fin[2] = {nullptr, nullptr};
     double *h_sum_base = nullptr;
     double *h_val = nullptr;
     int *h_abort = nullptr;
@@ -570,7 +570,8 @@
     memset(h->h_sum_base, 0, sizeof(double) * 2 * h->SB);
     HIPCHECK(hipHostMalloc((void **)&h->h_val, sizeof(double) * 2));
     HIPCHECK(hipStreamCreateWithFlags(&h->qstream, hipStreamNonBlocking));
-    for (int x = 0; x < 2; x++) { HIPCHECK(hipEventCreateWithFlags(&h->ev_sum[x], hipEventDisableTiming)); HIPCHECK(hipEventCreateWithFlags(&h->ev_val[x], hipEventDisableTiming)); HIPCHECK(hipEventCreateWithFlags(&h->ev_tail[x], hipEventDisableTiming)); }
+    if (h->sel.lds_qtree) if (int rc = ensure_lds(h, reinterpret_cast<const void *>(k_quad_tree), h->sel.lds_qtree)) return rc;
+    for (int x = 0; x < 2; x++) { HIPCHECK(hipEventCreateWithFlags(&h->ev_sum[x], hipEventDisableTiming)); HIPCHECK(hipEventCreateWithFlags(&h->ev_val[x], hipEventDisableTiming)); HIPCHECK(hipEventCreateWithFlags(&h->ev_tail[x], hipEventDisableTiming)); HIPCHECK(hipEventCreateWithFlags(&h->ev_qb[x], hipEventDisableTiming)); HIPCHECK(hipEventCreateWithFlags(&h->ev_fin[x], hipEventDisableTiming)); }
     HIPCHECK(hipHostMalloc((void **)&h->h_msg, 4 * h->P.MSZ));
     HIPCHECK(hipHostMalloc((void **)&h->h_tmp, sizeof(double) * std::max(h->QB, h->SB)));
     if (h->W > 1) {
@@ -683,7 +684,7 @@
     if (h->h_val) (void)hipHostFree(h->h_val);
     if (h->h_svd) (void)hipHostFree(h->h_svd);
     if (h->qstream) (void)hipStreamDestroy(h->qstream);
-    for (int x = 0; x < 2; x++) { if (h->ev_sum[x]) (void)hipEventDestroy(h->ev_sum[x]); if (h->ev_val[x]) (void)hipEventDestroy(h->ev_val[x]); if (h->ev_tail[x]) (void)hipEventDestroy(h->ev_tail[x]); }
+    for (int x = 0; x < 2; x++) { if (h->ev_sum[x]) (void)hipEventDestroy(h->ev_sum[x]); if (h->ev_val[x]) (void)hipEventDestroy(h->ev_val[x]); if (h->ev_tail[x]) (void)hipEventDestroy(h->ev_tail[x]); if (h->ev_qb[x]) (void)hipEventDestroy(h->ev_qb[x]); if (h->ev_fin[x]) (void)hipEventDestroy(h->ev_fin[x]); }
     if (h->h_msg) (void)hipHostFree(h->h_msg);
     if (h->h_tmp) (void)hipHostFree(h->h_tmp);
     if (h->red_mem) (void)hipHostFree(h->red_mem);
@@ -1021,18 +1022,25 @@
     fflush(stdout);
 }
 
+static int readback_enqueue(ttx_engine *h, double *dst, hipStream_t sq)
+{
+    hipLaunchKernelGGL(k_collect, dim3(1), dim3(256), 0, sq, h->P);
+    int rc = allreduce_dev(h, h->P.sumsend, h->P.sumrecv, h->SB, 0);
+    if (rc) return rc;
+    HIPCHECK(hipMemcpyAsync(dst, h->P.sumrecv, sizeof(double) * h->SB, hipMemcpyDeviceToHost, sq));
+    return TTX_OK;
+}
+static int readback_wait(ttx_engine *h)
+{
+    HIPCHECK(hipStreamSynchronize(h->stream));
+    if (h->cb_error) return fail(TTX_EHIP, "host transport: a sendrecv / allreduce callback failed");
+    if (h->profile) ev_collect(h);
+    return TTX_OK;
+}
 static int readback(ttx_engine *h)
 {
-    hipLaunchKernelGGL(k_collect, dim3(1), dim3(256), 0, h->stream, h->P);
-    {
-        int rc = allreduce_dev(h, h->P.sumsend, h->P.sumrecv, h->SB, 0);
-        if (rc) return rc;
-        HIPCHECK(hipMemcpyAsync(h->h_sum, h->P.sumrecv, sizeof(double) * h->SB, hipMemcpyDeviceToHost, h->stream));
-        HIPCHECK(hipStreamSynchronize(h->stream));
-        if (h->cb_error) return fail(TTX_EHIP, "host transport: a sendrecv / allreduce callback failed");
-    }
-    if (h->profile) ev_collect(h);
-    return TTX_OK;
+    if (int rc = readback_enqueue(h, h->h_sum, h->stream)) return rc;
+    return readback_wait(h);
 }
 static inline const double *sum_bond(const ttx_engine *h, int p) { return h->h_sum + SUM_HDR + h->cfg.nproc + 5 * (size_t)p; }
 
@@ -1060,15 +1068,16 @@
 
 static inline size_t lds_fpersist(const DevProb &P) { return (P.arith && P.fpersist) ? sizeof(double) * 4 * (P.d + 8) : 0; }
 
-static int launch_quad(ttx_engine *h, hipStream_t sq, const DevProb &Q, int mode, const double *w)
+static int launch_quad(ttx_engine *h, hipStream_t sq, const DevProb &Q, int mode, const double *w, hipEvent_t built = nullptr)
 {
     const size_t lds_q = sizeof(double) * ((size_t)h->RM * h->RM + 2);
     hipLaunchKernelGGL(k_quad_build, dim3(h->NC, h->G), dim3(256), lds_q, sq, Q, mode, w);
+    if (built) HIPCHECK(hipEventRecord(built, sq));
     hipLaunchKernelGGL(k_quad_chain, dim3(h->G), dim3(256), Q.qscr ? 0 : 2 * lds_q, sq, Q);
     if (h->cfg.nproc > 1) {
         int rc = allreduce_dev(h, Q.qsend, Q.qall, h->QB, 0);
         if (rc) return rc;
-        hipLaunchKernelGGL(k_quad_tree, dim3(1), dim3(256), 0, sq, Q);
+        hipLaunchKernelGGL(k_quad_tree, dim3(1), dim3(256), h->sel.lds_qtree, sq, Q, h->sel.lds_qtree ? 1 : 0);
     }
     return TTX_OK;
 }
@@ -1149,9 +1158,10 @@
     p.fullpiv = FUN == FUN_HOST ? ChainPlan::FP_COLUMNS : P.fp_mfma ? ChainPlan::FP_MFMA : ChainPlan::FP_PLAIN;
     p.accept = kl(k_accept, "k_accept", dim3(2 * p.nfb + 2 * NM + 1, G), dim3(TTX_BLK), sizeof(double) * std::max<size_t>(RM + 2, (size_t)std::min<int>(RM, 64) * std::min<int>(RM, 64)));
     {
-        const size_t lds_s = s.lds_par + 16 + sizeof(short) * 256 * VS;
-        p.srows = lds_s <= TTX_LDS_WORK ? 1 : 0;
-        p.init_samples = kl(k_init_samples<FUN>, KFUN_(k_init_samples), dim3(G), dim3(256), p.srows ? lds_s : s.lds_par, p.srows != 0);
+        const bool own_rows = FUN != FUN_HOST && !(FUN == FUN_ISING && P.arith && P.ising_id != 1);
+        const InitSamplesPlan ip = init_samples_plan(s.lds_par, VS, h->d, (long)s.nn * s.snum, own_rows, s.init_wide);
+        p.srows = ip.rows;
+        p.init_samples = kl(k_init_samples<FUN>, KFUN_(k_init_samples), dim3(G), dim3(ip.threads), ip.lds, ip.rows != 0);
         p.init_fibers = kl(k_init_fibers<FUN>, KFUN_(k_init_fibers), dim3(h->NC, G), dim3(256), s.lds_par);
     }
     if (s.de_npair) p.tables = P.de_cut ? kl(k_de_ctables, "k_de_ctables", dim3(2 * RM, G), dim3(256), sizeof(double) * (size_t)(d + 2))
@@ -1219,7 +1229,8 @@
     LoopPlan L; ChainPlan plan;
     DevProb Pq;
     double val = 1.0, val_prev = 1.0;
-    int strike = 0; bool ready = false, fin_enqueued = false;
+    int strike = 0, sweeps = 0; bool ready = false, fin_enqueued = false;
+    double *sum_final = nullptr;
     explicit SweepRun(ttx_engine *h_) : h(h_), P(h_->P), st(h_->stream), d(h_->d), G(h_->G), nproc(h_->cfg.nproc), cluster(h_->cluster_nb()), fused(h_->sel.fused) {}
     double since() const { return std::chrono::duration<double>(clk::now() - t0).count(); }
     template <class... A>
@@ -1238,6 +1249,7 @@
         in.whole = cluster || fused; in.cluster = cluster != 0; in.profile = h->profile; in.pipeline_off = env_off("TTX_PIPELINE");
         in.W = h->W; in.nproc = nproc; in.has_quad = P.has_quad; in.host_pass = FUN == FUN_HOST;
         in.sweep_tail = h->sel.sweep_tail; in.sweep_tail_side = h->sel.sweep_tail_side; in.maxrank = h->cfg.maxrank;
+        in.head_direct = h->sel.head_direct; in.fin_early = h->sel.fin_early; in.fin_skip_exch = h->sel.fin_skip_exch;
         L = loop_plan(in);
         P.tail_side = L.side ? 1 : 0;
         h->recs.clear(); h->tapes.clear();
@@ -1253,12 +1265,14 @@
             if (int rc = EV(plan.init_samples, h->sel.snum, h->sel.nn, FUN == FUN_HOST ? 0 : plan.srows, 0)) return rc;
             if (int rc = EV(plan.init_fibers)) return rc;
             hipLaunchKernelGGL(k_init_factors, dim3(h->NC, G), dim3(256), lds_fpersist(P), st, P);
-            hipLaunchKernelGGL(k_init_final, dim3(G), dim3(256), 0, st, P);
+            hipLaunchKernelGGL(k_init_final, dim3(G), dim3(256), 0, st, P, h->sel.init_wave ? 1 : 0, L.head_direct ? h->h_sum_base : (double *)nullptr);
         }
         if (L.head) {
-            hipLaunchKernelGGL(k_collect, dim3(1), dim3(256), 0, st, P);
             h->h_sum = h->h_sum_base;
-            HIPCHECK(hipMemcpyAsync(h->h_sum, P.sumrecv, sizeof(double) * h->SB, hipMemcpyDeviceToHost, st));
+            if (!L.head_direct) {
+                hipLaunchKernelGGL(k_collect, dim3(1), dim3(256), 0, st, P);
+                HIPCHECK(hipMemcpyAsync(h->h_sum, P.sumrecv, sizeof(double) * h->SB, hipMemcpyDeviceToHost, st));
+            }
             HIPCHECK(hipEventRecord(h->ev_sum[0], st));
             if (int rc = launch_sweep_kernel(1)) return rc;
             HIPCHECK(hipEventSynchronize(h->ev_sum[0]));
@@ -1368,7 +1382,7 @@
     {
         {
             KScope ks(h, TTX_K_EXCHANGE, (h->W > 1 ? 4 : 2) + (nproc > 1 ? 1 : 0));
-            if (!cluster) hipLaunchKernelGGL(k_exch_pack, dim3(G), dim3(256), 0, st, P);
+            if (!cluster) hipLaunchKernelGGL(k_exch_pack, dim3(G), dim3(256), 0, st, P, 0);
             if (h->W > 1) {
                 hipLaunchKernelGGL(k_exch_localmax, dim3(1), dim3(64), 0, st, P);
                 if (int rc = xfer_neighbours(h)) return rc;
@@ -1389,7 +1403,7 @@
     {
         const int slot = it_ & 1;
         KScope ks(h, TTX_K_QUAD, nproc > 1 ? 3 : 2);
-        if (int rc = launch_quad(h, sq, L.pipe ? Pq : P, 0, P.quadw)) return rc;
+        if (int rc = launch_quad(h, sq, L.pipe ? Pq : P, 0, P.quadw, L.fin_early ? h->ev_qb[slot] : nullptr)) return rc;
         if (L.pipe) {
             HIPCHECK(hipMemcpyAsync(h->h_val + slot, &P.gs[0].val, sizeof(double), hipMemcpyDeviceToHost, sq));
             HIPCHECK(hipEventRecord(h->ev_val[slot], sq));
@@ -1409,16 +1423,27 @@
     {
         if (fin_enqueued) return TTX_OK;
         fin_enqueued = true;
-        if (after_val >= 0) HIPCHECK(hipStreamWaitEvent(st, h->ev_val[after_val], 0));
-        HIPCHECK(hipMemsetAsync(P.ctl, 0, sizeof(int) * 3, st));
-        KScope ks(h, TTX_K_OTHER, 2);
-        if (nproc > 1) {
-            hipLaunchKernelGGL(k_exch_pack, dim3(G), dim3(256), 0, st, P);
-            if (int rc = xfer_neighbours(h)) return rc;
-            hipLaunchKernelGGL(k_exch_apply, dim3(G), dim3(256), lds_fpersist(P), st, P);
+        const bool early = L.fin_early && after_val >= 0;
+        if (early) HIPCHECK(hipEventRecord(h->ev_fin[0], st));
+        if (after_val >= 0) HIPCHECK(hipStreamWaitEvent(st, early ? h->ev_qb[after_val] : h->ev_val[after_val], 0));
+        if (!early) HIPCHECK(hipMemsetAsync(P.ctl, 0, sizeof(int) * 3, st));
+        {
+            KScope ks(h, TTX_K_OTHER, 2);
+            if (L.final_exchange(sweeps)) {
+                hipLaunchKernelGGL(k_exch_pack, dim3(G), dim3(256), 0, st, P, 1);
+                if (int rc = xfer_neighbours(h)) return rc;
+                hipLaunchKernelGGL(k_exch_apply, dim3(G), dim3(256), lds_fpersist(P), st, P);
+            }
+            launch(st, plan.fin_luar, P, plan.fl);
+            launch(st, plan.fin_lual, P, plan.fl);
         }
-        launch(st, plan.fin_luar, P, plan.fl);
-        launch(st, plan.fin_lual, P, plan.fl);
+        if (!early) return TTX_OK;
+        const hipStream_t sq = h->qstream;
+        HIPCHECK(hipStreamWaitEvent(sq, h->ev_fin[0], 0));
+        HIPCHECK(hipMemsetAsync(P.ctl, 0, sizeof(int) * 3, sq));
+        sum_final = h->h_sum_base + (size_t)(after_val ^ 1) * h->SB;
+        if (int rc = readback_enqueue(h, sum_final, sq)) return rc;
+        HIPCHECK(hipEventRecord(h->ev_fin[1], sq));
         return TTX_OK;
     }
     void record(int it_, int dir)
@@ -1432,6 +1457,7 @@
     int process_sweep(int it_)
     {
         const int slot = it_ & 1;
+        sweeps = it_;
         if (L.pipe) {
             HIPCHECK(hipEventSynchronize(h->ev_sum[slot]));
             h->h_sum = h->h_sum_base + (size_t)slot * h->SB;
@@ -1473,7 +1499,9 @@
             }
         }
         if (int rc = enqueue_final(-1)) return rc;
-        if (int rc = readback(h)) return rc;
+        if (sum_final) h->h_sum = sum_final;
+        if (int rc = sum_final ? readback_wait(h) : readback(h)) return rc;
+        if (sum_final) HIPCHECK(hipEventSynchronize(h->ev_fin[1]));
         HIPCHECK(hipGetLastError());
 #ifdef TTX_STAMPS
         if (int rc = dump_stamps(h)) return rc;
diff --git a/ttcross_amd/csrc/ttx_kernels.h b/ttcross_amd/csrc/ttx_kernels.h
--- a/ttcross_amd/csrc/ttx_kernels.h
+++ b/ttcross_amd/csrc/ttx_kernels.h
@@ -709,11 +709,11 @@
 struct FixIdx { const int *ind; int self, selfval; __device__ __forceinline__ int operator()(int s) const { return s == self ? selfval : ind[s]; } };
 
 template <int FUN>
-__global__ __launch_bounds__(256) void k_init_samples(DevProb P, int snum, int nn, int ldsrows, int shift_hi)
+__global__ __launch_bounds__(512) void k_init_samples(DevProb P, int snum, int nn, int ldsrows, int shift_hi)
 {
     extern __shared__ __align__(16) double dyn[];
     double *par = dyn;
-    __shared__ double sha[4], shv[4]; __shared__ int shi[4];
+    __shared__ double sha[8], shv[8]; __shared__ int shi[8];
     const int g = blockIdx.x, tid = threadIdx.x;
     GroupState &gs = P.gs[g];
     for (int x = tid; x < P.npar; x += blockDim.x) par[x] = P.par[x];
@@ -745,10 +745,17 @@
             double a = fabs(f);
             if (a > ba || (a == ba && il < bi)) { ba = a; bv = f; bi = il; }
         }
-    else
+    else {
+    const int *nl = P.n + 1;
+    if (ldsrows == 2) {
+        int *nls = (int *)(((size_t)(rows + (size_t)blockDim.x * VSr) + 15) & ~(size_t)15);
+        for (int x = tid; x < m; x += blockDim.x) nls[x] = P.n[x + 1];
+        __syncthreads();
+        nl = nls;
+    }
     for (int il = tid; il < nn * snum; il += blockDim.x) {
         const int k = il % nn + 1, sft = il / nn;
-        for (int p = 1; p <= m; p++) row[p - 1] = (short)((k - 1 + sft * (p - 1)) % P.n[p] + 1);
+        for (int p = 1; p <= m; p++) row[p - 1] = (short)((k - 1 + sft * (p - 1)) % nl[p - 1] + 1);
         for (int x = m; x < VSr; x++) row[x] = 1;
         row[m - 1 + 0] = row[m - 1];
         const int self = row[m - 1];
@@ -757,6 +764,7 @@
         double f = eval_src3<FUN, true>(P, par, sx, (long)g * P.HS + il);
         double a = fabs(f);
         if (a > ba || (a == ba && il < bi)) { ba = a; bv = f; bi = il; }
+    }
     }
     if (HOST_PASS1(FUN, P)) return;
     block_argmax(ba, bv, bi, sha, shv, shi);
@@ -850,9 +858,15 @@
     }
 }
 
-__global__ __launch_bounds__(256) void k_init_final(DevProb P)
-{
-    __shared__ double dots[256];
+__device__ __forceinline__ double lane_value(double x, int k)
+{
+    const long long b = __double_as_longlong(x);
+    const int lo = __builtin_amdgcn_readlane((int)b, k), hi = __builtin_amdgcn_readlane((int)(b >> 32), k);
+    return __longlong_as_double(((long long)hi << 32) | (unsigned int)lo);
+}
+__global__ __launch_bounds__(256) void k_init_final(DevProb P, int wave, double *out)
+{
+    __shared__ double dots[256], divs[256];
     const int g = blockIdx.x, tid = threadIdx.x;
     GroupState &gs = P.gs[g];
     const bool lastgroup = (gs.last + 1 == P.d && gs.gglobal == P.nprocs - 1);
@@ -860,6 +874,21 @@
     double val = 1.0;
     if (P.has_quad) {
         for (int c0 = 0; c0 < ncore; c0 += 256) {
+            if (wave) {
+                const int lane = tid & 63, nw = blockDim.x >> 6, cend = min(ncore, c0 + 256);
+                for (int c = c0 + (tid >> 6); c < cend; c += nw) {
+                    const int p = gs.first + c, np_ = P.n[p];
+                    const double *A = core_ptr(P, P.arg, g, p, gs.first), *w = P.quadw + (size_t)p * P.NM;
+                    double t = 0.0;
+                    for (int b = 0; b < np_; b += 64) {
+                        const int j = b + lane, nb = min(64, np_ - b);
+                        const double pr = j < np_ ? A[(size_t)P.RM * j] * w[j] : 0.0;
+                        for (int k = 0; k < nb; k++) t = t + lane_value(pr, k);
+                    }
+                    if (lane == 0) dots[c - c0] = t;
+                }
+                if (c0 + tid < cend) { const int p = gs.first + c0 + tid; divs[tid] = p <= gs.last ? inv_ptr(P, g, p, gs.first)[0] : 0.0; }
+            } else {
             const int c = c0 + tid;
             if (c < ncore) {
                 const int p = gs.first + c;
@@ -868,17 +897,37 @@
                 for (int j = 0; j < P.n[p]; j++) t = t + A[(size_t)P.RM * j] * w[j];
                 dots[tid] = t;
             }
+            }
             __syncthreads();
             if (tid == 0)
                 for (int c2 = c0; c2 < min(ncore, c0 + 256); c2++) {
                     const int p = gs.first + c2;
-                    if (p <= gs.last) val = val * dots[c2 - c0] / inv_ptr(P, g, p, gs.first)[0];
+                    if (p <= gs.last) val = val * dots[c2 - c0] / (wave ? divs[c2 - c0] : inv_ptr(P, g, p, gs.first)[0]);
                     else val = val * dots[c2 - c0];
                 }
             __syncthreads();
         }
     }
     if (tid == 0) { gs.pivotmax_prev = gs.amax; gs.pivotmax = -1.0; gs.pivotmin = -1.0; gs.initval = val; }
+    if (!out) return;
+    const int m = P.d;
+    const int *r = P.r + (size_t)g * (m + 2), *tp = P.tape + (size_t)g * (m + 2) * 4;
+    for (int p = gs.first + tid; p <= gs.last; p += blockDim.x) {
+        double *e = out + SUM_HDR + P.nprocs + 5 * p;
+        e[0] = (double)r[p]; e[1] = (double)tp[4 * p]; e[2] = (double)tp[4 * p + 1]; e[3] = (double)tp[4 * p + 2]; e[4] = (double)tp[4 * p + 3];
+    }
+    if (g == 0)
+        for (int p = tid; p <= m; p += blockDim.x)
+            if (p < P.gs[0].first || p > P.gs[P.G - 1].last) { double *e = out + SUM_HDR + P.nprocs + 5 * p; for (int x = 0; x < 5; x++) e[x] = 0.0; }
+    if (tid != 0) return;
+    out[SUM_HDR + gs.gglobal] = val;
+    if (gs.gglobal == 0) { out[SUM_AMAX] = gs.amax; out[SUM_PMAX] = -1.0; out[SUM_PMIN] = -1.0; }
+    if (g != 0) return;
+    double nev = 0.0, by = 0.0, nr = 0.0;
+    for (int x = 0; x < P.G; x++) { const GroupState &o = P.gs[x]; nev += (double)o.neval; by += o.bytes_half; nr += (double)o.n_resid; }
+    out[SUM_NEVAL] = nev; out[SUM_BYTES] = by; out[SUM_NRESID] = nr;
+    out[SUM_VAL] = P.gs[0].val;
+    for (int x = SUM_VAL + 1; x < SUM_HDR; x++) out[x] = 0.0;
 }
 
 __global__ __launch_bounds__(256) void k_reset(DevProb P, size_t SB, size_t QB)
@@ -1917,7 +1966,7 @@
     }
 }
 
-__global__ __launch_bounds__(256) void k_exch_pack(DevProb P) { if (P.ctl[0]) return; exch_pack_group(P, blockIdx.x); }
+__global__ __launch_bounds__(256) void k_exch_pack(DevProb P, int force) { if (P.ctl[0] && !force) return; exch_pack_group(P, blockIdx.x); }
 __global__ __launch_bounds__(256) void k_exch_apply(DevProb P) { exch_apply_group(P, blockIdx.x); }
 
 __device__ __forceinline__ void exch_max_group(const DevProb &P, int g, int from_recv)
@@ -2202,7 +2251,7 @@
     }
 }
 
-__global__ __launch_bounds__(256) void k_quad_tree(DevProb P)
+__global__ __launch_bounds__(256) void k_quad_tree(DevProb P, int lds)
 {
     if (P.ctl[2]) return;
     const int tid = threadIdx.x, RM = P.RM, ng = P.nprocs;
@@ -2211,6 +2260,34 @@
     double *work = P.qwork;
     for (int g = tid; g < ng; g += blockDim.x) { mym[g] = (int)dims[2 * g]; myn[g] = (int)dims[2 * g + 1]; }
     __syncthreads();
+    if (lds) {
+        extern __shared__ double qsh[];
+        __shared__ int wh[256];
+        const size_t MS = (size_t)RM * RM, REG = (size_t)ng * MS;
+        for (int g = tid; g < ng; g += blockDim.x) wh[g] = 0;
+        for (int g = 0; g < ng; g++)
+            for (int x = tid; x < mym[g] * myn[g]; x += blockDim.x) qsh[(size_t)g * MS + (x % mym[g]) + RM * (x / mym[g])] = part[(size_t)g * MS + (x % mym[g]) + RM * (x / mym[g])];
+        __syncthreads();
+        for (int q = 1; q < ng; q *= 2) {
+            for (int me = 0; me + q < ng; me += 2 * q) {
+                const int her = me + q;
+                const double *Aa = qsh + (size_t)wh[me] * REG + (size_t)me * MS, *Bb = qsh + (size_t)wh[her] * REG + (size_t)her * MS;
+                double *dst = qsh + (size_t)(wh[me] ^ 1) * REG + (size_t)me * MS;
+                const int mm = mym[me], kk = myn[me], nn = myn[her];
+                for (int x = tid; x < mm * nn; x += blockDim.x) {
+                    int i = x % mm, j = x / mm;
+                    double c = 0.0;
+                    for (int l = 0; l < kk; l++) c = c + Bb[l + RM * j] * Aa[i + RM * l];
+                    dst[i + RM * j] = c;
+                }
+            }
+            __syncthreads();
+            if (tid == 0) for (int me = 0; me + q < ng; me += 2 * q) { myn[me] = myn[me + q]; wh[me] ^= 1; }
+            __syncthreads();
+        }
+        if (tid == 0) { const double v = qsh[(size_t)wh[0] * REG]; for (int g = 0; g < P.G; g++) P.gs[g].val = v; }
+        return;
+    }
     for (int g = 0; g < ng; g++)
         for (int x = tid; x < mym[g] * myn[g]; x += blockDim.x) work[(size_t)g * RM * RM + (x % mym[g]) + RM * (x / mym[g])] = part[(size_t)g * RM * RM + (x % mym[g]) + RM * (x / mym[g])];
     __syncthreads();
diff --git a/ttcross_amd/csrc/ttx_loop_plan.h b/ttcross_amd/csrc/ttx_loop_plan.h
--- a/ttcross_amd/csrc/ttx_loop_plan.h
+++ b/ttcross_amd/csrc/ttx_loop_plan.h
@@ -12,6 +12,9 @@
     bool sweep_tail = false;
     bool sweep_tail_side = false;
     int maxrank = 1;
+    bool head_direct = false;
+    bool fin_early = false;
+    bool fin_skip_exch = false;
 };
 
 struct LoopPlan {
@@ -20,6 +23,11 @@
     bool forkq = false;
     bool tail = false;
     bool side = false;
+    bool head_direct = false;
+    bool fin_early = false;
+    bool fin_skip_exch = false;
+    int nproc = 1;
+    bool final_exchange(int sweeps) const { return nproc > 1 && !(fin_skip_exch && sweeps >= 1); }
 };
 
 inline LoopPlan loop_plan(const LoopIn &in)
@@ -30,5 +38,9 @@
     p.forkq = p.pipe && in.has_quad && in.W == 1;
     p.tail = p.pipe && in.cluster && in.W == 1 && in.nproc > 1 && !in.host_pass && in.sweep_tail;
     p.side = p.tail && p.forkq && in.sweep_tail_side;
+    p.head_direct = p.head && in.head_direct;
+    p.fin_early = p.forkq && in.fin_early;
+    p.fin_skip_exch = in.W == 1 && in.fin_skip_exch;
+    p.nproc = in.nproc;
     return p;
 }
```
